# RLinf/RLinf

Measured on NVIDIA H100. Metric: env-steps/sec (rollout+update), higher is better.
Workload: dtype f32

## Files before the change

include/rlinf_b200.h:

```cpp
#ifndef RLINF_B200_H
#define RLINF_B200_H

#include <stdint.h>

#ifdef __cplusplus
extern "C" {
#endif

#define RB200_ABI_VERSION 2

#define RB200_OK 0
#define RB200_E_NULL (-1)
#define RB200_E_SHAPE (-2)
#define RB200_E_ARG (-3)
#define RB200_E_ALIGN (-4)
#define RB200_E_UNSUPPORTED (-5)

typedef void* rb200_stream_t;

int rb200_abi_version(void);
const char* rb200_strerror(int code);
int rb200_device_info(int* sm_count, int* cc_major, int* cc_minor);
uint64_t rb200_launch_count(void);

// ... 164 lines not shown
  float* loss;
  float* metrics;
  float* d_logprobs;
  float* d_entropy;
} rb200_token_loss_args;
int64_t rb200_token_loss_workspace_bytes(int64_t bsz, int64_t L);
int rb200_token_ppo_loss(const rb200_token_loss_args* args, rb200_stream_t stream);

enum {
  RB200_CM_VALUE_LOSS = 0,
  RB200_CM_VALUE_CLIP_RATIO = 1,
  RB200_CM_EV_COUNT = 2,
  RB200_CM_EV_RET_SUM = 3,
  RB200_CM_EV_RET_SQ_SUM = 4,
  RB200_CM_EV_ERR_SUM = 5,
  RB200_CM_EV_ERR_SQ_SUM = 6,
  RB200_CM_FINAL_VALUE_LOSS = 7,
  RB200_CM_NUM = 8
};
typedef struct rb200_token_critic_loss_args {
  int64_t bsz, L;
  const float* values;       int64_t values_stride;
  const float* returns;      int64_t returns_stride;
  const float* prev_values;  int64_t prev_values_stride;
  const uint8_t* loss_mask;  int64_t loss_mask_stride;
  double value_clip, huber_delta;
  void* workspace;
  int64_t workspace_bytes;
  float* loss;
  float* metrics;
  float* d_values;
} rb200_token_critic_loss_args;
int rb200_token_critic_loss(const rb200_token_critic_loss_args* args, rb200_stream_t stream);

enum {
  RB200_RR_SUM_PLEN = 0, RB200_RR_SUM_RLEN = 1, RB200_RR_SUM_REWARDS = 2, RB200_RR_SUM_END = 3,
  RB200_RR_SUM_ADV = 4, RB200_RR_NUM_SEQ = 5, RB200_RR_N_VALID = 6, RB200_RR_SUM_TRAJ_REWARDS = 7,
  RB200_RR_NUM_TRAJ = 8,
  RB200_RR_ADV_NEG_MIN = 9, RB200_RR_ADV_MAX = 10, RB200_RR_MAX_PLEN = 11, RB200_RR_MAX_RLEN = 12,
  RB200_RR_MAX_TOTAL = 13, RB200_RR_VAL_NEG_MIN = 14, RB200_RR_VAL_MAX = 15,
  RB200_RR_VALUES_MEAN = 16,
  RB200_RR_RLEN_SUM = 17, RB200_RR_RLEN_SQ_SUM = 18, RB200_RR_RLEN_MIN = 19, RB200_RR_RLEN_MAX = 20,
  RB200_RR_VERDICT = 21,
  RB200_RR_NUM = 24
};
enum { RB200_RV_EMPTY = 1, RB200_RV_BAD_TRAJ = 2 };
enum {
  RB200_RM_NUM_SEQ = 0, RB200_RM_PROMPT_LENGTH, RB200_RM_RESPONSE_LENGTH, RB200_RM_AVG_RESPONSE_LENGTH,
  RB200_RM_VAR_RESPONSE_LENGTH, RB200_RM_MAX_OF_RESPONSE_LENGTH, RB200_RM_MIN_OF_RESPONSE_LENGTH,
  RB200_RM_TOTAL_LENGTH, RB200_RM_REWARD_SCORES, RB200_RM_PROPERLY_ENDED, RB200_RM_ADV_MEAN, RB200_RM_ADV_MAX,
  RB200_RM_ADV_MIN, RB200_RM_VALUES_MEAN, RB200_RM_VALUES_MAX, RB200_RM_VALUES_MIN, RB200_RM_MAX_PROMPT_LENGTH,
  RB200_RM_MAX_RESPONSE_LENGTH, RB200_RM_MAX_TOTAL_LENGTH, RB200_RM_REWARD_SCORES_TRAJ, RB200_RM_REWARD_SCORES_TURN,
  RB200_RM_AVG_TURNS_PER_TRAJ, RB200_RM_VERDICT, RB200_RM_NUM_LENGTHS_MAX,
  RB200_RM_NUM = 24
};
typedef struct rb200_reasoning_record_args {
  int64_t bsz, L;
  const float* advantages;    int64_t advantages_stride;
  const uint8_t* mask;        int64_t mask_stride;
  const float* values;        int64_t values_stride;
  const int64_t* prompt_lengths;
  const int64_t* response_lengths;
  const float* rewards;
  const uint8_t* is_end;
  const int64_t* idx_to_traj;
  void* workspace;
  int64_t workspace_bytes;
  double* record;
} rb200_reasoning_record_args;
int64_t rb200_reasoning_record_workspace_bytes(int64_t bsz, int64_t L);
int rb200_reasoning_rollout_record(const rb200_reasoning_record_args* args, rb200_stream_t stream);
int rb200_reasoning_rollout_finish(const double* records, int32_t P, const float* values_world_sum,
                                   int32_t world_size, double* metrics, rb200_stream_t stream);

#define RB200_EPI_MAX_KEYS 24
#define RB200_EPI_WS_MIN 64
typedef struct rb200_mb_epilogue_args {
  int32_t n_avg, n_sum;
  int32_t final_slot, ratio_slot;
  const float* src[RB200_EPI_MAX_KEYS];
  const float* loss;
  const uint8_t* mask;  int64_t mask_stride;  int64_t bsz, L;
  const float* global_valid_token;
  int32_t dp, num_microbatches;
  int32_t has_early_stop, mb;
  double early_stop_imp_ratio;
  void* workspace;
  int64_t workspace_bytes;
  float* pack;
  float* scale;
  float* metrics;
  float* step_acc;
  int32_t n_mb, reserved;
} rb200_mb_epilogue_args;
int rb200_mask_count_f32(const uint8_t* mask, int64_t mask_stride, int64_t bsz, int64_t L, void* workspace,
                         int64_t workspace_bytes, float* out, rb200_stream_t stream);
int rb200_mb_epilogue_pack(const rb200_mb_epilogue_args* args, rb200_stream_t stream);
int rb200_mb_epilogue_apply(const rb200_mb_epilogue_args* args, rb200_stream_t stream);
int rb200_step_metrics_finish(const float* step_acc, int32_t n_mb, int32_t n_avg, int32_t n_sum, float* out,
                              rb200_stream_t stream);

int64_t rb200_value_head_workspace_bytes(int64_t n, int64_t H);
int rb200_value_head_fwd(const void* x, int64_t row_stride, const int64_t* rows, int64_t n, int64_t H, const void* w,
                         float* v, rb200_stream_t stream);
int rb200_value_head_bwd(const void* x, int64_t row_stride, const int64_t* rows, int64_t n, int64_t H, const float* g,
                         const void* w, const int64_t* inv_map, int64_t T, void* dx, void* dw, void* workspace,
                         int64_t workspace_bytes, rb200_stream_t stream);

int rb200_scale(float* x, int64_t n, float s, rb200_stream_t stream);
int rb200_scale_by(float* x, int64_t n, const float* s_dev, rb200_stream_t stream);

int rb200_grad_sqnorm(const float* grads, int64_t n, double* out_sq ,
                      rb200_stream_t stream);
int rb200_adamw_step(float* params, const float* grads, float* exp_avg, float* exp_avg_sq,
                     int64_t n, const int64_t* group_end_host, const double* group_lr_host,
                     int n_groups, double beta1, double beta2, double eps, double weight_decay,
                     float max_grad_norm, float grad_scale, const double* grad_sq ,
                     double* state , rb200_stream_t stream);
int rb200_adamw_step_dev(float* params, const float* grads, float* exp_avg, float* exp_avg_sq,
                         int64_t n, const int64_t* group_end_host, const double* group_lr_dev,
                         int n_groups, double beta1, double beta2, double eps, double weight_decay,
                         float max_grad_norm, float grad_scale, const double* grad_sq ,
                         double* state , rb200_stream_t stream);


typedef struct rb200_mlp_layout {
  int32_t obs_dim, act_dim , value_dim, hidden ;
  int64_t logstd;
  int64_t vw0, vb0, vw1, vb1, vw2, vb2, vw3;
  int64_t bw0, bb0, bw1, bb1, bw2, bb2;
  int64_t mw, mb;
  int64_t total;
} rb200_mlp_layout;

int rb200_mlp_layout_init(rb200_mlp_layout* L, int obs_dim, int act_dim, int value_dim, int hidden);

int64_t rb200_mlp_fwd_scratch_floats(const rb200_mlp_layout* L, int64_t n);

int64_t rb200_mlp_wsplit_floats(const rb200_mlp_layout* L);
int rb200_mlp_prepare_weights(const rb200_mlp_layout* L, const float* params, float* wsplit,
                              rb200_stream_t stream);

int rb200_mlp_forward(const rb200_mlp_layout* L, const float* params, const float* wsplit,
                      const float* states, const float* action, const int64_t* idx, int64_t n,
                      float* logprobs, float* entropy, float* values, float* acts, float* work,
                      const float* states_amax, rb200_stream_t stream);
int rb200_absmax(const float* x, int64_t rows, int cols, float* out, rb200_stream_t stream);

int rb200_mlp_backward(const rb200_mlp_layout* L, const float* params, const float* wsplit,
                       const float* states, const float* action, const int64_t* idx, int64_t n,
                       const float* d_logprobs, const float* d_entropy, const float* d_values,
                       const float* acts, float* work, float* grads, rb200_stream_t stream);

int rb200_mlp_sample(const rb200_mlp_layout* L, const float* params, const float* wsplit,
                     const float* states, const float* noise, uint64_t seed, uint64_t offset,
                     const uint64_t* counter_dev, int64_t n, float* action, float* logprobs, float* values,
                     float* work, rb200_stream_t stream);

int rb200_tc_gemm_h(const float* A, const float* B, float* C, int64_t M, int K, int mode, const float* amax,
                    float* work, rb200_stream_t stream);
int rb200_tc_wgrad_h(const float* Z, const float* H, float* dW, int64_t n, int IN, const float* amax,
                     rb200_stream_t stream);
int rb200_tc_dgrad_wgrad_h(const float* Z, const float* W, const float* H, float* dZprev, float* dW, float* colsum,
                           const float* amax_in, float* amax_out, int64_t n, int ngroups, float* work,
                           rb200_stream_t stream);

int rb200_debug_set_flags(int flags);

typedef struct rb200_rollout_args {
  float* states;
  float* actions;
  float* logprobs;
  float* values;
  float* rewards;
  uint8_t* terminations;
  uint8_t* truncations;
  uint8_t* dones;
  float* final_obs;
  float* final_values;
  const float* w_s;
  const float* w_a;
  int32_t* elapsed;
  const float* policy_noise;
  const float* env_noise;
  const uint64_t* counter_policy;
  const uint64_t* counter_env;
  float* episode_return;
  double* episode_acc;
  uint64_t seed_policy, seed_env, offset_policy;
  int32_t T, B;
  int32_t num_action_chunks;
  int32_t max_episode_steps, auto_reset;
  int32_t bootstrap_on_done;
  double gamma, p_term, noise_std, reward_noise_std;
} rb200_rollout_args;

int64_t rb200_rollout_fused_wt_floats(const rb200_mlp_layout* L);
int rb200_rollout_fused_supported(const rb200_mlp_layout* L, int B);
int rb200_rollout_fused_prepare(const rb200_mlp_layout* L, const float* params, float* wt, rb200_stream_t stream);
int rb200_rollout_fused(const rb200_mlp_layout* L, const float* params, const float* wt, const rb200_rollout_args* a,
                        rb200_stream_t stream);

int rb200_rollout_tc_supported(const rb200_mlp_layout* L, int num_action_chunks, int B);
int64_t rb200_rollout_tc_pack_bytes(const rb200_mlp_layout* L);
int rb200_rollout_tc_prepare(const rb200_mlp_layout* L, const float* params, const float* w_s, void* pack,
                             rb200_stream_t stream);
int rb200_rollout_tc(const rb200_mlp_layout* L, const float* params, const void* pack, const rb200_rollout_args* a,
                     rb200_stream_t stream);

int rb200_logits_logprob_entropy_fwd(const void* logits, int dtype, const int64_t* target, int64_t N, int64_t L,
                                     int64_t batch_stride, int64_t row_stride, int V, int v_lo, int v_hi,
                                     double inv_temperature, float* logprob, float* entropy, float* lse,
                                     rb200_stream_t stream);
int rb200_logits_logprob_entropy_bwd(const void* logits, int dtype, const int64_t* target, int64_t N, int64_t L,
                                     int64_t batch_stride, int64_t row_stride, int V, int v_lo, int v_hi,
                                     double inv_temperature, const float* lse, const float* entropy,
                                     const float* grad_logprob, const float* grad_entropy, void* dlogits,
                                     int64_t d_batch_stride, int64_t d_row_stride, rb200_stream_t stream);

int rb200_logits_topk_logprob_entropy_fwd(const void* logits, int dtype, const int64_t* target, int64_t N, int64_t L,
                                          int64_t batch_stride, int64_t row_stride, int V, int v_lo, int v_hi,
                                          double inv_temperature, int top_k, float* logprob, float* entropy, float* lse,
                                          float* threshold, rb200_stream_t stream);
int rb200_logits_topk_logprob_entropy_bwd(const void* logits, int dtype, const int64_t* target, int64_t N, int64_t L,
                                          int64_t batch_stride, int64_t row_stride, int V, int v_lo, int v_hi,
                                          double inv_temperature, const float* threshold, const float* lse,
                                          const float* entropy, const float* grad_logprob, const float* grad_entropy,
                                          void* dlogits, int64_t d_batch_stride, int64_t d_row_stride,
                                          rb200_stream_t stream);

int64_t rb200_lmhead_workspace_bytes(int64_t N, int64_t L, int H, int V, int v_lo, int v_hi, int64_t vocab_chunk);
int rb200_lmhead_logprob_entropy_fwd(const void* hidden, const void* weight, const int64_t* target, int64_t N, int64_t L,
                                     int64_t batch_stride, int64_t row_stride, int H, int V, int v_lo, int v_hi,
                                     double inv_temperature, float* logprob, float* entropy, float* lse,
                                     void* workspace, int64_t workspace_bytes, rb200_stream_t stream);
int rb200_lmhead_logprob_entropy_bwd(const void* hidden, const void* weight, const int64_t* target, int64_t N, int64_t L,
                                     int64_t batch_stride, int64_t row_stride, int H, int V, int v_lo, int v_hi,
                                     double inv_temperature, const float* lse, const float* entropy,
                                     const float* grad_logprob, const float* grad_entropy, void* d_hidden,
                                     void* d_weight, void* workspace, int64_t workspace_bytes, rb200_stream_t stream);

int64_t rb200_lmhead_topk_workspace_bytes(int64_t N, int64_t L, int H, int V, int v_lo, int v_hi, int64_t row_block,
                                          int64_t vocab_chunk);
int rb200_lmhead_topk_logprob_entropy_fwd(const void* hidden, const void* weight, const int64_t* target, int64_t N,
                                          int64_t L, int64_t batch_stride, int64_t row_stride, int H, int V, int v_lo,
                                          int v_hi, double inv_temperature, int top_k, float* logprob, float* entropy,
                                          float* lse, float* threshold, void* workspace, int64_t workspace_bytes,
                                          rb200_stream_t stream);
int rb200_lmhead_topk_logprob_entropy_bwd(const void* hidden, const void* weight, const int64_t* target, int64_t N,
                                          int64_t L, int64_t batch_stride, int64_t row_stride, int H, int V, int v_lo,
                                          int v_hi, double inv_temperature, const float* threshold, const float* lse,
                                          const float* entropy, const float* grad_logprob, const float* grad_entropy,
                                          void* d_hidden, void* d_weight, void* workspace, int64_t workspace_bytes,
                                          rb200_stream_t stream);

typedef struct rb200_action_bins {
  const double* bin_centers;
  const double* low;
  const double* high;
  const uint8_t* mask;
  int64_t vocab_size;
  int32_t n_bins;
  int32_t action_dim;
} rb200_action_bins;
int rb200_logits_sample_tokens(const void* logits, int dtype, int64_t N, int64_t L, int64_t batch_stride,
                               int64_t row_stride, int V, int v_lo, int v_hi, int do_sample, double inv_temperature,
                               int top_k, uint64_t seed, uint64_t offset, const rb200_action_bins* bins, int64_t* token,
                               float* logprob, double* action, rb200_stream_t stream);
int64_t rb200_lmhead_sample_workspace_bytes(int64_t N, int64_t L, int H, int V, int v_lo, int v_hi);
int rb200_lmhead_sample_tokens(const void* hidden, const void* weight, int64_t N, int64_t L, int64_t batch_stride,
                               int64_t row_stride, int H, int V, int v_lo, int v_hi, int do_sample,
                               double inv_temperature, int top_k, uint64_t seed, uint64_t offset,
                               const rb200_action_bins* bins, int64_t* token, float* logprob, double* action,
                               void* workspace, int64_t workspace_bytes, rb200_stream_t stream);

int64_t rb200_lmhead_vp_workspace_bytes(int64_t N, int64_t L, int H, int Vs, int64_t vocab_start, int v_lo, int v_hi,
                                        int64_t vocab_chunk);
int rb200_lmhead_vp_partials_fwd(const void* hidden, const void* weight_shard, const int64_t* target, int64_t N,
                                 int64_t L, int64_t batch_stride, int64_t row_stride, int H, int Vs,
                                 int64_t vocab_start, int v_lo, int v_hi, double inv_temperature, float* record,
                                 void* workspace, int64_t workspace_bytes, rb200_stream_t stream);
int rb200_lmhead_vp_logprob_entropy_bwd(const void* hidden, const void* weight_shard, const int64_t* target,
                                        int64_t N, int64_t L, int64_t batch_stride, int64_t row_stride, int H, int Vs,
                                        int64_t vocab_start, int v_lo, int v_hi, double inv_temperature,
                                        const float* lse, const float* entropy, const float* grad_logprob,
                                        const float* grad_entropy, float* d_hidden_partial, void* d_weight_shard,
                                        void* workspace, int64_t workspace_bytes, rb200_stream_t stream);
int rb200_logits_vp_partials_fwd(const void* logits, int dtype, const int64_t* target, int64_t N, int64_t L,
                                 int64_t batch_stride, int64_t row_stride, int Vs, int64_t vocab_start, int v_lo,
                                 int v_hi, double inv_temperature, float* record, rb200_stream_t stream);
int rb200_vp_combine(const float* records, int n_ranks, int64_t N, const int64_t* target, int vocab_shard, int v_lo,
                     int v_hi, float* logprob, float* entropy, float* lse, rb200_stream_t stream);

enum {
  RB200_RR_RESPONSE = 1,
  RB200_RR_PROMPT = 2,
  RB200_RR_BOUNDS = 4,
  RB200_RR_ORDER = 8,
  RB200_RR_MAX_PROMPT = 16,
  RB200_RR_CAPACITY = 32
};
int rb200_response_rows_plan(int layout, const int64_t* len0, const int64_t* len1, const int64_t* response_lengths,
                             int64_t bsz, int64_t S, int64_t L, int64_t T, int entropy_shift, const int64_t* tokens,
                             int64_t capacity, int64_t* rows, int64_t* targets, int64_t* cell_map,
                             int64_t* hidden_map, int64_t* cells, int64_t* status, rb200_stream_t stream);

enum {
  RB200_RR_SHARD = 64,
  RB200_RR_CP_ALIGN = 128
};
int rb200_response_rows_mp_plan(const int64_t* cu_seqlens_padded, const int64_t* seq_lengths,
                                const int64_t* response_lengths, const int64_t* responses, int64_t bsz, int64_t L,
                                int64_t T_c, int tp_size, int cp_size, int sequence_parallel, int tp_rank, int cp_rank,
                                int64_t capacity_c, int64_t capacity_k, int64_t* rows, int64_t* send, int64_t* unpad,
                                int64_t* slot_map, int64_t* targets, int64_t* cell_map, int64_t* cells,
                                int64_t* hidden_map, int64_t* status, rb200_stream_t stream);
int rb200_response_rows_mp_pack_grad(const float* dx, const int64_t* idx, void* out, int64_t n_out, int64_t H,
                                     rb200_stream_t stream);

int rb200_mlp_value(const rb200_mlp_layout* L, const float* params, const float* wsplit,
// ... 59 lines not shown
```

rlinf_b200/_lib.py:

```python
from __future__ import annotations

import ctypes as C
import os
from typing import Optional

import torch

_PKG_DIR = os.path.dirname(os.path.abspath(__file__))
LIB_PATH = os.path.join(_PKG_DIR, "librlinf_b200.so")

c_void_p, c_int, c_int64, c_float, c_double, c_uint64 = C.c_void_p, C.c_int, C.c_int64, C.c_float, C.c_double, C.c_uint64

NUM_METRICS = 24
LOGPROB_TYPES = {"token_level": 0, "action_level": 1, "chunk_level": 2}

M_KEYS = {
    0: "actor/policy_loss", 1: "actor/policy_loss_abs", 2: "actor/ratio", 3: "actor/ratio_abs",
    4: "actor/clipped_ratio", 5: "actor/dual_cliped_ratio", 6: "actor/approx_kl", 7: "actor/clip_fraction",
    8: "critic/value_loss", 9: "critic/value_clip_ratio",
    10: "__sum__/_critic_explained_variance/count",
    11: "__sum__/_critic_explained_variance/returns_sum",
    12: "__sum__/_critic_explained_variance/returns_sq_sum",
    13: "__sum__/_critic_explained_variance/errors_sum",
    14: "__sum__/_critic_explained_variance/errors_sq_sum",
# ... 32 lines not shown
class DppoScalarVersionArgs(C.Structure):
    _fields_ = [("base", PpoArgs), ("proximal_logprobs", c_void_p), ("version", c_double),
                ("current_version", c_double), ("has_behave_weight_threshold", C.c_int32),
                ("behave_weight_threshold", c_double)]


class RolloutArgs(C.Structure):
    _fields_ = [(n, c_void_p) for n in (
        "states", "actions", "logprobs", "values", "rewards", "terminations", "truncations", "dones", "final_obs",
        "final_values", "w_s", "w_a", "elapsed", "policy_noise", "env_noise", "counter_policy", "counter_env",
        "episode_return", "episode_acc")] + [
        ("seed_policy", c_uint64), ("seed_env", c_uint64), ("offset_policy", c_uint64),
        ("T", C.c_int32), ("B", C.c_int32), ("num_action_chunks", C.c_int32), ("max_episode_steps", C.c_int32),
        ("auto_reset", C.c_int32), ("bootstrap_on_done", C.c_int32),
        ("gamma", c_double), ("p_term", c_double), ("noise_std", c_double), ("reward_noise_std", c_double),
    ]


DM_KEYS = {
    0: "actor/policy_loss", 1: "actor/proximal_ratio", 2: "actor/clipped_proximal_ratio", 3: "actor/clip_fraction",
    4: "actor/dual_clip_fraction", 5: "actor/behav_clip_fraction", 6: "actor/proximal_approx_kl",
    7: "actor/behav_approx_kl", 8: "critic/value_loss", 9: "critic/value_clip_ratio",
    10: "__sum__/_critic_explained_variance/count", 11: "__sum__/_critic_explained_variance/returns_sum",
    12: "__sum__/_critic_explained_variance/returns_sq_sum", 13: "__sum__/_critic_explained_variance/errors_sum",
    14: "__sum__/_critic_explained_variance/errors_sq_sum",
}
DM_ENTROPY = 20


AGG_MODES = {"token-mean": 0, "seq-mean-token-sum": 1, "seq-mean-token-mean": 2}
TM_NUM = 16
TM_KEYS = {
    0: "actor/policy_loss", 1: "actor/policy_loss_abs", 2: "actor/ratio", 3: "actor/ratio_abs",
    4: "actor/clipped_ratio", 5: "actor/dual_cliped_ratio", 6: "actor/approx_kl", 7: "actor/clip_fraction",
    8: "actor/entropy_loss", 9: "actor/kl_loss", 10: "actor/final_loss", 11: "actor/rollout_train_kl",
}


class TokenLossArgs(C.Structure):
    _fields_ = [("bsz", c_int64), ("L", c_int64)] + [
        f for name in ("logprobs", "old_logprobs", "advantages", "loss_mask", "entropy", "ref_logprobs",
                       "rollout_logprobs", "recomputed_logprobs") for f in ((name, c_void_p), (name + "_stride", c_int64))
    ] + [(n, c_double) for n in ("clip_ratio_low", "clip_ratio_high", "clip_ratio_c", "clip_log_ratio_min",
                                  "clip_log_ratio_max", "entropy_bonus", "kl_beta", "importance_sampling_clip")] + [
        (n, C.c_int32) for n in ("has_clip_log_ratio_min", "has_clip_log_ratio_max", "agg", "kl_mode", "kl_order",
                                 "importance_sampling_fix", "fast_path_zero_loss_mask", "reserved")] + [
        ("workspace", c_void_p), ("workspace_bytes", c_int64),
        ("loss", c_void_p), ("metrics", c_void_p), ("d_logprobs", c_void_p), ("d_entropy", c_void_p),
    ]


CM_NUM = 8
CM_KEYS = {
    0: "critic/value_loss", 1: "critic/value_clip_ratio",
    2: "__sum__/_critic_explained_variance/count",
    3: "__sum__/_critic_explained_variance/returns_sum",
    4: "__sum__/_critic_explained_variance/returns_sq_sum",
    5: "__sum__/_critic_explained_variance/errors_sum",
    6: "__sum__/_critic_explained_variance/errors_sq_sum",
    7: "critic/final_value_loss",
}


class TokenCriticLossArgs(C.Structure):
    _fields_ = [("bsz", c_int64), ("L", c_int64)] + [
        f for name in ("values", "returns", "prev_values", "loss_mask")
        for f in ((name, c_void_p), (name + "_stride", c_int64))
    ] + [("value_clip", c_double), ("huber_delta", c_double), ("workspace", c_void_p), ("workspace_bytes", c_int64),
         ("loss", c_void_p), ("metrics", c_void_p), ("d_values", c_void_p)]


RR_NUM = 24
RM_NUM = 24
RM_SLOTS = {
    "total_num_sequence": 0, "prompt_length": 1, "response_length": 2, "average_response_length": 3,
    "variance_of_response_length": 4, "max_of_response_length": 5, "min_of_response_length": 6, "total_length": 7,
    "reward_scores": 8, "fraction_of_samples_properly_ended": 9, "advantages_mean": 10, "advantages_max": 11,
    "advantages_min": 12, "values_mean": 13, "values_max": 14, "values_min": 15, "max_prompt_length": 16,
    "max_response_length": 17, "max_total_length": 18, "reward_scores_traj": 19, "reward_scores_turn": 20,
    "avg_turns_per_traj": 21,
}
RM_VERDICT, RM_NUM_LENGTHS_MAX = 22, 23
RR_VALUES_MEAN = 16
RV_EMPTY, RV_BAD_TRAJ = 1, 2
EPI_MAX_KEYS = 24
EPI_WS_MIN = 64


class ReasoningRecordArgs(C.Structure):
    _fields_ = [("bsz", c_int64), ("L", c_int64)] + [
        f for name in ("advantages", "mask", "values") for f in ((name, c_void_p), (name + "_stride", c_int64))
    ] + [(n, c_void_p) for n in ("prompt_lengths", "response_lengths", "rewards", "is_end", "idx_to_traj",
                                 "workspace")] + [("workspace_bytes", c_int64), ("record", c_void_p)]


class MbEpilogueArgs(C.Structure):
    _fields_ = [(n, C.c_int32) for n in ("n_avg", "n_sum", "final_slot", "ratio_slot")] + [
        ("src", c_void_p * EPI_MAX_KEYS), ("loss", c_void_p), ("mask", c_void_p), ("mask_stride", c_int64),
        ("bsz", c_int64), ("L", c_int64), ("global_valid_token", c_void_p)] + [
        (n, C.c_int32) for n in ("dp", "num_microbatches", "has_early_stop", "mb")] + [
        ("early_stop_imp_ratio", c_double), ("workspace", c_void_p), ("workspace_bytes", c_int64)] + [
        (n, c_void_p) for n in ("pack", "scale", "metrics", "step_acc")] + [("n_mb", C.c_int32), ("reserved", C.c_int32)]


class ActionBins(C.Structure):
    _fields_ = [("bin_centers", c_void_p), ("low", c_void_p), ("high", c_void_p), ("mask", c_void_p),
                ("vocab_size", c_int64), ("n_bins", C.c_int32), ("action_dim", C.c_int32)]


class MlpLayout(C.Structure):
    _fields_ = [
        ("obs_dim", C.c_int32), ("act_dim", C.c_int32), ("value_dim", C.c_int32), ("hidden", C.c_int32),
        ("logstd", c_int64),
        ("vw0", c_int64), ("vb0", c_int64), ("vw1", c_int64), ("vb1", c_int64), ("vw2", c_int64), ("vb2", c_int64),
        ("vw3", c_int64),
        ("bw0", c_int64), ("bb0", c_int64), ("bw1", c_int64), ("bb1", c_int64), ("bw2", c_int64), ("bb2", c_int64),
        ("mw", c_int64), ("mb", c_int64), ("total", c_int64),
    ]


SIGNATURES = {
    "rb200_abi_version": (c_int, []),
    "rb200_strerror": (C.c_char_p, [c_int]),
    "rb200_device_info": (c_int, [C.POINTER(c_int)] * 3),
    "rb200_launch_count": (c_uint64, []),
    "rb200_loss_mask": (c_int, [c_void_p, c_void_p, c_void_p, c_int, c_int, c_int, c_void_p]),
    "rb200_gae": (c_int, [c_void_p] * 7 + [c_int, c_int, c_double, c_double, c_void_p]),
    "rb200_normalize": (c_int, [c_void_p, c_void_p, c_int64, c_float, c_void_p]),
    "rb200_grpo_scores": (c_int, [c_void_p, c_void_p, c_void_p, c_int, c_int, c_void_p]),
    "rb200_grpo_advantages": (c_int, [c_void_p, c_void_p, c_void_p, c_int, c_int, c_int, c_float, c_void_p]),
    "rb200_gather_rows": (c_int, [c_void_p, c_void_p, c_void_p, c_int64, c_int64, c_int64, c_void_p]),
    "rb200_ppo_loss": (c_int, [C.POINTER(PpoArgs), c_void_p]),
    "rb200_decoupled_ppo_loss": (c_int, [C.POINTER(DppoArgs), c_void_p]),
    "rb200_decoupled_ppo_loss_scalar_version": (c_int, [C.POINTER(DppoScalarVersionArgs), c_void_p]),
    "rb200_opd_loss": (c_int, [c_void_p] * 4 + [c_int64, c_int, c_int, c_double] + [c_void_p] * 5),
    "rb200_token_loss_workspace_bytes": (c_int64, [c_int64, c_int64]),
    "rb200_token_ppo_loss": (c_int, [C.POINTER(TokenLossArgs), c_void_p]),
    "rb200_scale": (c_int, [c_void_p, c_int64, c_float, c_void_p]),
    "rb200_scale_by": (c_int, [c_void_p, c_int64, c_void_p, c_void_p]),
    "rb200_grad_sqnorm": (c_int, [c_void_p, c_int64, c_void_p, c_void_p]),
    "rb200_adamw_step": (c_int, [c_void_p] * 4 + [c_int64, C.POINTER(c_int64), C.POINTER(c_double), c_int,
                                                  c_double, c_double, c_double, c_double, c_float, c_float,
                                                  c_void_p, c_void_p, c_void_p]),
    "rb200_adamw_step_dev": (c_int, [c_void_p] * 4 + [c_int64, C.POINTER(c_int64), c_void_p, c_int,
                                                      c_double, c_double, c_double, c_double, c_float, c_float,
                                                      c_void_p, c_void_p, c_void_p]),
    "rb200_mlp_layout_init": (c_int, [C.POINTER(MlpLayout), c_int, c_int, c_int, c_int]),
    "rb200_mlp_fwd_scratch_floats": (c_int64, [C.POINTER(MlpLayout), c_int64]),
    "rb200_mlp_wsplit_floats": (c_int64, [C.POINTER(MlpLayout)]),
    "rb200_mlp_prepare_weights": (c_int, [C.POINTER(MlpLayout), c_void_p, c_void_p, c_void_p]),
    "rb200_mlp_forward": (c_int, [C.POINTER(MlpLayout)] + [c_void_p] * 5 + [c_int64] + [c_void_p] * 7),
    "rb200_absmax": (c_int, [c_void_p, c_int64, c_int, c_void_p, c_void_p]),
    "rb200_mlp_backward": (c_int, [C.POINTER(MlpLayout)] + [c_void_p] * 5 + [c_int64] + [c_void_p] * 7),
    "rb200_mlp_sample": (c_int, [C.POINTER(MlpLayout)] + [c_void_p] * 4 + [c_uint64, c_uint64, c_void_p, c_int64] + [c_void_p] * 5),
    "rb200_tc_gemm_h": (c_int, [c_void_p, c_void_p, c_void_p, c_int64, c_int, c_int, c_void_p, c_void_p, c_void_p]),
    "rb200_tc_wgrad_h": (c_int, [c_void_p, c_void_p, c_void_p, c_int64, c_int, c_void_p, c_void_p]),
    "rb200_tc_dgrad_wgrad_h": (c_int, [c_void_p] * 8 + [c_int64, c_int, c_void_p, c_void_p]),
    "rb200_debug_set_flags": (c_int, [c_int]),
    "rb200_rollout_fused_wt_floats": (c_int64, [C.POINTER(MlpLayout)]),
    "rb200_rollout_fused_supported": (c_int, [C.POINTER(MlpLayout), c_int]),
    "rb200_rollout_fused_prepare": (c_int, [C.POINTER(MlpLayout), c_void_p, c_void_p, c_void_p]),
    "rb200_rollout_fused": (c_int, [C.POINTER(MlpLayout), c_void_p, c_void_p, C.POINTER(RolloutArgs), c_void_p]),
    "rb200_rollout_tc_supported": (c_int, [C.POINTER(MlpLayout), c_int, c_int]),
    "rb200_rollout_tc_pack_bytes": (c_int64, [C.POINTER(MlpLayout)]),
    "rb200_rollout_tc_prepare": (c_int, [C.POINTER(MlpLayout), c_void_p, c_void_p, c_void_p, c_void_p]),
    "rb200_rollout_tc": (c_int, [C.POINTER(MlpLayout), c_void_p, c_void_p, C.POINTER(RolloutArgs), c_void_p]),
    "rb200_logits_logprob_entropy_fwd": (c_int, [c_void_p, c_int, c_void_p, c_int64, c_int64, c_int64, c_int64, c_int,
                                                 c_int, c_int, c_double, c_void_p, c_void_p, c_void_p, c_void_p]),
    "rb200_logits_logprob_entropy_bwd": (c_int, [c_void_p, c_int, c_void_p, c_int64, c_int64, c_int64, c_int64, c_int,
                                                 c_int, c_int, c_double] + [c_void_p] * 5 + [c_int64, c_int64, c_void_p]),
    "rb200_logits_topk_logprob_entropy_fwd": (c_int, [c_void_p, c_int, c_void_p, c_int64, c_int64, c_int64, c_int64,
                                                      c_int, c_int, c_int, c_double, c_int] + [c_void_p] * 5),
    "rb200_logits_topk_logprob_entropy_bwd": (c_int, [c_void_p, c_int, c_void_p, c_int64, c_int64, c_int64, c_int64,
                                                      c_int, c_int, c_int, c_double] + [c_void_p] * 6
                                              + [c_int64, c_int64, c_void_p]),
    "rb200_lmhead_workspace_bytes": (c_int64, [c_int64, c_int64, c_int, c_int, c_int, c_int, c_int64]),
    "rb200_lmhead_logprob_entropy_fwd": (c_int, [c_void_p, c_void_p, c_void_p, c_int64, c_int64, c_int64, c_int64, c_int,
                                                 c_int, c_int, c_int, c_double] + [c_void_p] * 4 + [c_int64, c_void_p]),
    "rb200_lmhead_logprob_entropy_bwd": (c_int, [c_void_p, c_void_p, c_void_p, c_int64, c_int64, c_int64, c_int64, c_int,
                                                 c_int, c_int, c_int, c_double] + [c_void_p] * 7 + [c_int64, c_void_p]),
    "rb200_lmhead_topk_workspace_bytes": (c_int64, [c_int64, c_int64, c_int, c_int, c_int, c_int, c_int64, c_int64]),
    "rb200_lmhead_topk_logprob_entropy_fwd": (c_int, [c_void_p, c_void_p, c_void_p, c_int64, c_int64, c_int64, c_int64,
                                                      c_int, c_int, c_int, c_int, c_double, c_int] + [c_void_p] * 5
                                              + [c_int64, c_void_p]),
    "rb200_lmhead_topk_logprob_entropy_bwd": (c_int, [c_void_p, c_void_p, c_void_p, c_int64, c_int64, c_int64, c_int64,
                                                      c_int, c_int, c_int, c_int, c_double] + [c_void_p] * 8
                                              + [c_int64, c_void_p]),
    "rb200_logits_sample_tokens": (c_int, [c_void_p, c_int, c_int64, c_int64, c_int64, c_int64, c_int, c_int, c_int,
                                           c_int, c_double, c_int, c_uint64, c_uint64, C.POINTER(ActionBins)]
                                   + [c_void_p] * 4),
    "rb200_lmhead_sample_workspace_bytes": (c_int64, [c_int64, c_int64, c_int, c_int, c_int, c_int]),
    "rb200_lmhead_sample_tokens": (c_int, [c_void_p, c_void_p, c_int64, c_int64, c_int64, c_int64, c_int, c_int, c_int,
                                           c_int, c_int, c_double, c_int, c_uint64, c_uint64, C.POINTER(ActionBins)]
                                   + [c_void_p] * 4 + [c_int64, c_void_p]),
    "rb200_lmhead_vp_workspace_bytes": (c_int64, [c_int64, c_int64, c_int, c_int, c_int64, c_int, c_int, c_int64]),
    "rb200_lmhead_vp_partials_fwd": (c_int, [c_void_p, c_void_p, c_void_p, c_int64, c_int64, c_int64, c_int64, c_int,
                                             c_int, c_int64, c_int, c_int, c_double, c_void_p, c_void_p, c_int64,
                                             c_void_p]),
    "rb200_lmhead_vp_logprob_entropy_bwd": (c_int, [c_void_p, c_void_p, c_void_p, c_int64, c_int64, c_int64, c_int64,
                                                    c_int, c_int, c_int64, c_int, c_int, c_double] + [c_void_p] * 7
                                            + [c_int64, c_void_p]),
    "rb200_logits_vp_partials_fwd": (c_int, [c_void_p, c_int, c_void_p, c_int64, c_int64, c_int64, c_int64, c_int,
                                             c_int64, c_int, c_int, c_double, c_void_p, c_void_p]),
    "rb200_vp_combine": (c_int, [c_void_p, c_int, c_int64, c_void_p, c_int, c_int, c_int] + [c_void_p] * 4),
    "rb200_response_rows_plan": (c_int, [c_int, c_void_p, c_void_p, c_void_p, c_int64, c_int64, c_int64, c_int64,
                                         c_int, c_void_p, c_int64] + [c_void_p] * 6 + [c_void_p]),
    "rb200_response_rows_mp_plan": (c_int, [c_void_p] * 4 + [c_int64] * 3 + [c_int] * 5 + [c_int64] * 2
                                    + [c_void_p] * 9 + [c_void_p]),
    "rb200_response_rows_mp_pack_grad": (c_int, [c_void_p, c_void_p, c_void_p, c_int64, c_int64, c_void_p]),
    "rb200_token_critic_loss": (c_int, [C.POINTER(TokenCriticLossArgs), c_void_p]),
    "rb200_reasoning_record_workspace_bytes": (c_int64, [c_int64, c_int64]),
    "rb200_reasoning_rollout_record": (c_int, [C.POINTER(ReasoningRecordArgs), c_void_p]),
    "rb200_reasoning_rollout_finish": (c_int, [c_void_p, C.c_int32, c_void_p, C.c_int32, c_void_p, c_void_p]),
    "rb200_mask_count_f32": (c_int, [c_void_p, c_int64, c_int64, c_int64, c_void_p, c_int64, c_void_p, c_void_p]),
    "rb200_mb_epilogue_pack": (c_int, [C.POINTER(MbEpilogueArgs), c_void_p]),
    "rb200_mb_epilogue_apply": (c_int, [C.POINTER(MbEpilogueArgs), c_void_p]),
    "rb200_step_metrics_finish": (c_int, [c_void_p, C.c_int32, C.c_int32, C.c_int32, c_void_p, c_void_p]),
    "rb200_value_head_workspace_bytes": (c_int64, [c_int64, c_int64]),
    "rb200_value_head_fwd": (c_int, [c_void_p, c_int64, c_void_p, c_int64, c_int64, c_void_p, c_void_p, c_void_p]),
    "rb200_value_head_bwd": (c_int, [c_void_p, c_int64, c_void_p, c_int64, c_int64, c_void_p, c_void_p, c_void_p,
                                     c_int64, c_void_p, c_void_p, c_void_p, c_int64, c_void_p]),
    "rb200_mlp_value":(c_int, [C.POINTER(MlpLayout), c_void_p, c_void_p, c_void_p, c_int64, c_void_p, c_void_p, c_void_p]),
    "rb200_synth_env_step": (c_int, [c_void_p] * 13 + [c_int] * 5 + [c_float] * 3 + [c_uint64, c_void_p, c_void_p]),
    "rb200_synth_env_chunk_step": (c_int, [c_void_p] * 13 + [c_int] * 6 + [c_float] * 3 + [c_uint64, c_void_p, c_void_p]),
    "rb200_bootstrap_rewards_ld": (c_int, [c_void_p, c_int, c_void_p, c_int, c_void_p, c_int, c_int, c_double, c_void_p]),
    "rb200_bootstrap_rewards": (c_int, [c_void_p, c_void_p, c_void_p, c_int, c_int, c_double, c_void_p]),
    "rb200_reward_filter": (c_int, [c_void_p] * 4 + [c_int] * 4 + [c_float, c_float, c_void_p]),
    "rb200_kl_penalty": (c_int, [c_void_p] * 4 + [c_int64, c_int, c_void_p]),
    "rb200_masked_stats": (c_int, [c_void_p, c_void_p, c_int64, c_int64, c_void_p, c_void_p]),
    "rb200_counter_add": (c_int, [c_void_p, c_uint64, c_void_p]),
    "rb200_masked_moments": (c_int, [c_void_p, c_void_p, c_int64, c_void_p, c_void_p]),
    "rb200_masked_normalize": (c_int, [c_void_p, c_void_p, c_void_p, c_int64, c_void_p, c_int, c_double, c_int, c_void_p]),
    "rb200_raw_advantages": (c_int, [c_void_p, c_void_p, c_void_p, c_int, c_int, c_void_p, c_void_p]),
    "rb200_reinpp_returns": (c_int, [c_void_p] * 5 + [c_int, c_int, c_double, c_int, c_void_p, c_void_p]),
    "rb200_grpo_video_advantages": (c_int, [c_void_p] * 4 + [c_int, c_int, c_int, c_int, c_float, c_void_p]),
    "rb200_grpo_dynamic_turn_advantages": (c_int, [c_void_p] * 3 + [c_int, c_int, c_int, c_int, c_float, c_void_p]),
    "rb200_sub": (c_int, [c_void_p, c_void_p, c_void_p, c_int64, c_void_p]),
    "rb200_mlp_mean": (c_int, [C.POINTER(MlpLayout), c_void_p, c_void_p, c_void_p, c_int64] + [c_void_p] * 5),
    "rb200_episode_stats_step": (c_int, [c_void_p, c_void_p, c_int, c_int, c_int] + [c_void_p] * 6),
    "rb200_episode_stats_reduce": (c_int, [c_void_p, c_int, c_void_p, c_void_p]),
    "rb200_train_episode_stats_step": (c_int, [c_void_p, c_void_p] + [c_int] * 4 + [c_void_p] * 4),
}

_LIB: Optional[C.CDLL] = None


class Rb200Error(RuntimeError):
    pass


def load() -> C.CDLL:
    global _LIB
    if _LIB is not None:
        return _LIB
    if not os.path.exists(LIB_PATH):
        raise Rb200Error(
            f"{LIB_PATH} not found: build it with `python -m rlinf_b200.build` "
            "(nvcc, sm_90a). rlinf_b200 has no CPU or PyTorch fallback.")
    lib = C.CDLL(LIB_PATH)
    for name, (res, args) in SIGNATURES.items():
        fn = getattr(lib, name)
        fn.restype = res
        fn.argtypes = args
    _LIB = lib
    return lib


def check(code: int, what: str = "") -> None:
    if code == 0:
        return
    msg = load().rb200_strerror(code).decode()
    if code < 0:
        raise ValueError(f"rlinf_b200 {what}: {msg} (code {code})")
    raise Rb200Error(f"rlinf_b200 {what}: CUDA error {code}: {msg}")


def ptr(t: Optional[torch.Tensor]):
    if t is None:
        return None
    if not t.is_cuda:
        raise Rb200Error("rlinf_b200 kernels take CUDA tensors; move inputs with to_device() first")
    if not t.is_contiguous():
        raise Rb200Error("rlinf_b200 kernels take contiguous tensors")
    return c_void_p(t.data_ptr())


def stream_ptr(device=None):
    return c_void_p(torch.cuda.current_stream(device).cuda_stream)


def default_device() -> torch.device:
    if not torch.cuda.is_available():
        raise Rb200Error("rlinf_b200 needs a CUDA device (H100, sm_90a); there is no CPU fallback")
    return torch.device("cuda", torch.cuda.current_device())


def to_device(t: Optional[torch.Tensor], device=None, dtype=None) -> Optional[torch.Tensor]:
    if t is None:
        return None
    device = device or default_device()
    if t.device != device:
        t = t.to(device, non_blocking=True)
    if dtype is not None and t.dtype != dtype:
        t = t.to(dtype)
    return t.contiguous()


def as_u8(t: Optional[torch.Tensor]) -> Optional[torch.Tensor]:
    if t is None:
        return None
    if t.dtype == torch.bool:
# ... 5 lines not shown
```

rlinf_b200/actor.py:

```python
from __future__ import annotations

from typing import Optional

import numpy as np
import torch
import torch.distributed as dist

from . import _lib as L
from . import dist_utils as D
from . import ops
from .algorithms import calculate_adv_and_returns
from .config import wrap
from .lr_scheduler import LRSchedule
from .policy import FlatAdamW, MLPPolicy

EV_KEY = "critic/explained_variance"
_T_PLUS_ONE_KEYS = ("dones", "terminations", "truncations", "prev_values")


def process_nested_dict_for_adv(nested, rollout_epoch):
    out = {}
    for k, v in nested.items():
        if isinstance(v, dict):
            out[k] = process_nested_dict_for_adv(v, rollout_epoch)
        elif isinstance(v, torch.Tensor):
            x = v.reshape(rollout_epoch, -1, *v.shape[1:]).transpose(0, 1)
            out[k] = x.reshape(x.shape[0], -1, *x.shape[3:])
    return out


def process_nested_dict_for_train(nested, shuffle_id):
    out = {}
    for k, v in nested.items():
        if v is None:
            out[k] = None
        elif isinstance(v, dict):
            out[k] = process_nested_dict_for_train(v, shuffle_id)
        elif isinstance(v, torch.Tensor):
            if k in _T_PLUS_ONE_KEYS:
                v = v[:-1]
            flat = v.reshape(-1, *v.shape[2:])
            if any(s == 0 for s in flat.stride()) and flat.numel() > 1:
                flat = flat.contiguous()
            as_bool = flat.dtype == torch.bool
            src = flat.contiguous()
            res = ops.gather_rows(src.view(torch.uint8) if as_bool else src, shuffle_id)
            out[k] = res.view(torch.bool) if as_bool else res
    return out


class EmbodiedActor:
    def __init__(self, cfg, policy: Optional[MLPPolicy] = None, rank: Optional[int] = None,
                 world_size: Optional[int] = None, process_group=None):
        self.cfg = wrap(cfg)
        self.pg = process_group
        self._dist = dist.is_available() and dist.is_initialized()
        self._rank = rank if rank is not None else (dist.get_rank() if self._dist else 0)
        self._world_size = world_size if world_size is not None else (dist.get_world_size() if self._dist else 1)
        m = self.cfg.actor.model
        self.device = L.default_device()
        self.model = policy or MLPPolicy(m.obs_dim, m.action_dim, m.get("num_action_chunks", 1),
                                         add_value_head=m.get("add_value_head", True), device=self.device,
                                         seed=self.cfg.actor.seed)
        o = self.cfg.actor.optim
        self.optimizer = FlatAdamW(self.model, lr=o.lr, value_lr=o.get("value_lr", o.lr),
                                   betas=(o.get("adam_beta1", 0.9), o.get("adam_beta2", 0.999)),
                                   eps=o.get("adam_eps", 1e-8), weight_decay=o.get("weight_decay", 1e-2),
                                   clip_grad=o.get("clip_grad", 1.0))
        self.optimizer_steps = 0
        self.critic_warmup_steps = int(o.get("critic_warmup_steps", 0) or 0) if self.model.value_dim > 0 else 0
        self._with_critic = self.cfg.algorithm.adv_type == "gae"
        self._set_frozen_groups()
        self.lr_schedule = LRSchedule(o, base_lr=o.lr)
        self.optimizer.lr_scale = self.lr_schedule.multiplier()
        self.rollout_batch: dict = {}
        self._perm_cache: dict = {}
        self.version = 0
        self._graph_update = self.cfg.actor.get("cuda_graph_update", False)
        self._graph_multi_rank = bool(self.cfg.actor.get("cuda_graph_multi_rank", False))
        self._capture_nccl = bool(self.cfg.actor.get("cuda_graph_capture_nccl", True))
        self._static_batch: dict = {}
        self._step_graphs: dict = {}
        self._train_calls = 0
        self._states_amax = torch.zeros(4 + m.obs_dim if m.obs_dim <= 256 else 1, dtype=torch.float32,
                                        device=self.device) if m.obs_dim % 32 == 0 else None

    def recv_rollout_trajectories(self, batch: dict) -> None:
        def to_dev(d):
            return {k: (to_dev(v) if isinstance(v, dict) else L.to_device(v, self.device)) for k, v in d.items()
                    if v is not None}

        self.rollout_batch = self._process_received_rollout_batch(to_dev(batch))

    def _process_received_rollout_batch(self, rollout_batch: dict) -> dict:
        cfg = self.cfg
        rollout_epoch = cfg.env.train.get("rollout_epoch", 1)
        if rollout_epoch != 1:
            rollout_batch = process_nested_dict_for_adv(rollout_batch, rollout_epoch)
        if not cfg.env.train.auto_reset and not cfg.env.train.get("ignore_terminations", False):
            loss_mask, loss_mask_sum = ops.loss_mask(rollout_batch["dones"])
            if cfg.algorithm.reward_type == "chunk_level":
                loss_mask = loss_mask.any(dim=-1, keepdim=True)
                loss_mask_sum = loss_mask_sum[..., -1:]
            rollout_batch["loss_mask"] = loss_mask
            rollout_batch["loss_mask_sum"] = loss_mask_sum
        if cfg.algorithm.get("filter_rewards", False):
            rollout_batch["loss_mask"] = ops.reward_filter(
                rollout_batch["rewards"], rollout_batch.get("loss_mask", None), cfg.algorithm.group_size,
                cfg.algorithm.rewards_lower_bound, cfg.algorithm.rewards_upper_bound)
        return rollout_batch

    def compute_advantages_and_returns(self) -> dict:
        cfg, rb = self.cfg, self.rollout_batch
        kwargs = {
            "task_type": cfg.runner.task_type, "adv_type": cfg.algorithm.adv_type, "rewards": rb["rewards"],
            "dones": rb["dones"], "values": rb.get("prev_values", None), "prev_logprobs": rb.get("prev_logprobs", None),
            "teacher_logprobs": None, "num_action_chunks": cfg.actor.model.get("num_action_chunks", 1),
            "gamma": cfg.algorithm.get("gamma", 1), "gae_lambda": cfg.algorithm.get("gae_lambda", 1),
            "group_size": cfg.algorithm.get("group_size", 8), "reward_type": cfg.algorithm.reward_type,
            "loss_mask": rb.get("loss_mask", None), "loss_mask_sum": rb.get("loss_mask_sum", None),
            "advantage_mode": cfg.algorithm.get("advantage_mode", None),
        }
        rb.update(calculate_adv_and_returns(**kwargs))
        if not cfg.runner.get("rollout_metrics", True):
            return {}
        from .metric_utils import compute_rollout_metrics

        return compute_rollout_metrics(rb, self._world_size, self.pg)

    def _shuffle_id(self, n: int) -> torch.Tensor:
        key = (n, self.cfg.actor.seed + self._rank)
        if key not in self._perm_cache:
            g = torch.Generator()
            g.manual_seed(D.shuffle_seed(self.cfg.actor.seed, self._rank))
            self._perm_cache[key] = torch.randperm(n, generator=g).to(self.device)
        return self._perm_cache[key]

    def run_training(self) -> dict:
        cfg = self.cfg
        rb = self.rollout_batch
        rollout_size = rb["prev_logprobs"].shape[0] * rb["prev_logprobs"].shape[1]
        shuffle_id = self._shuffle_id(rollout_size)
        batch = process_nested_dict_for_train(rb, shuffle_id)
        self.rollout_batch = batch
        mbs = cfg.actor.micro_batch_size
        batch_size_per_rank, self.gradient_accumulation, n_global = D.per_rank_batch(
            cfg.actor.global_batch_size, self._world_size, mbs, rollout_size)
        update_epoch = cfg.algorithm.get("update_epoch", 1)
        n_steps = update_epoch * n_global
        n_micro = n_steps * self.gradient_accumulation
        metric_rows = torch.zeros(n_micro, L.NUM_METRICS, dtype=torch.float32, device=self.device)
        step_rows = torch.zeros(n_steps, 4, dtype=torch.float64, device=self.device)
        lr_rows = []
        mi = si = 0
        use_graph = self._graph_update
        if use_graph == "auto":
            use_graph = batch_size_per_rank <= 65536
        if self._world_size > 1 and not self._graph_multi_rank:
            use_graph = False
        graphed = bool(use_graph) and self._train_calls > 0
        self._train_calls += 1
        if graphed:
            batch = self._persist_batch(batch)
            self.rollout_batch = batch
        if self._states_amax is not None:
            ops.absmax(batch["forward_inputs"]["states"], out=self._states_amax)
        for _ in range(update_epoch):
            for gb in range(n_global):
                if graphed:
                    lr_rows.append(self._graphed_step(batch, gb, batch_size_per_rank, mbs,
                                                      metric_rows[mi: mi + self.gradient_accumulation], step_rows[si]))
                    mi += self.gradient_accumulation
                    si += 1
                    continue
                self.optimizer.zero_grad()
                for k in range(self.gradient_accumulation):
                    lo = gb * batch_size_per_rank + k * mbs
                    self.train_micro_batch(batch, lo, lo + mbs, metric_rows[mi])
                    mi += 1
                grad_norm_state, lr_list = self.optimizer_step()
                step_rows[si].copy_(grad_norm_state)
                lr_rows.append(lr_list)
                si += 1
        self.optimizer.lr_scale = self.lr_schedule.step()
        self.optimizer.zero_grad()
        return self._reduce_metrics(metric_rows, step_rows, lr_rows)

    def _persist_batch(self, batch: dict, prefix: str = "") -> dict:
        out = {}
        for k, v in batch.items():
            key = prefix + k
            if isinstance(v, dict):
                out[k] = self._persist_batch(v, key + "/")
            elif isinstance(v, torch.Tensor):
                buf = self._static_batch.get(key)
                if buf is None or buf.shape != v.shape or buf.dtype != v.dtype:
                    buf = torch.empty_like(v)
                    self._static_batch[key] = buf
                    self._step_graphs.clear()
                buf.copy_(v)
                out[k] = buf
            else:
                out[k] = v
        return out

    def _graphed_step(self, batch, gb, batch_size_per_rank, mbs, metric_out, state_out):
        warm = self.optimizer_steps < self.critic_warmup_steps
        accum = self.gradient_accumulation
        key = (gb, warm, accum, mbs, batch_size_per_rank, self._world_size)
        self.optimizer.sync_lr_table()
        entry = self._step_graphs.get(key)
        if entry is None:
            stage_m = torch.zeros(accum, L.NUM_METRICS, dtype=torch.float32, device=self.device)
            stage_s = torch.zeros(4, dtype=torch.float64, device=self.device)
            scale = 1.0 / self._world_size

            def fwd_bwd():
                self.optimizer.zero_grad()
                for k in range(accum):
                    lo = gb * batch_size_per_rank + k * mbs
                    self.train_micro_batch(batch, lo, lo + mbs, stage_m[k])

            def opt():
                self.optimizer.step(grad_scale=scale)
                stage_s.copy_(self.optimizer.state)

            graphs = None
            if self._world_size > 1 and self._capture_nccl:
                try:
                    torch.cuda.synchronize()
                    self.model.mark_params_changed()
                    g_all = torch.cuda.CUDAGraph()
                    with torch.cuda.graph(g_all):
                        fwd_bwd()
                        dist.all_reduce(self.model.flat_grads, op=dist.ReduceOp.SUM, group=self.pg)
                        opt()
                    graphs = (g_all, None)
                except Exception as e:
                    self._capture_nccl = False
                    self._capture_nccl_error = repr(e)
                    torch.cuda.synchronize()
            if graphs is None:
                torch.cuda.synchronize()
                self.model.mark_params_changed()
                g_a = torch.cuda.CUDAGraph()
                with torch.cuda.graph(g_a):
                    fwd_bwd()
                g_b = torch.cuda.CUDAGraph()
                with torch.cuda.graph(g_b, pool=g_a.pool()):
                    opt()
                graphs = (g_a, g_b)
            entry = (graphs, stage_m, stage_s)
            self._step_graphs[key] = entry
        (g_a, g_b), stage_m, stage_s = entry
        g_a.replay()
        self.optimizer_steps += 1
        if g_b is not None:
            D.allreduce_flat_grads(self.model.flat_grads, self._world_size, self.pg)
            g_b.replay()
        self.model.mark_params_changed()
        metric_out.copy_(stage_m)
        state_out.copy_(stage_s)
        return self._after_optimizer_step()

    def train_micro_batch(self, batch, lo, hi, metric_out) -> None:
        cfg = self.cfg
        fi = batch["forward_inputs"]
        with_critic = self._with_critic
        ent_bonus = float(cfg.algorithm.get("entropy_bonus", 0) or 0)
        warm = self.optimizer_steps < self.critic_warmup_steps
        out = self.model.forward_train(fi["states"][lo:hi], fi["action"][lo:hi], compute_entropy=ent_bonus > 0,
                                       compute_values=with_critic, states_amax=self._states_amax)
        A = cfg.actor.model.get("action_dim", 7)
        Cc = out["logprobs"].shape[1] // A
        U = 1 if cfg.algorithm.logprob_type == "chunk_level" else Cc
        n = hi - lo

        def unit(key):
            t = batch.get(key)
            return None if t is None else t[lo:hi].reshape(n, U)

        loss, metrics, d_lp, d_v, d_e = ops.ppo_loss(
            logprobs=out["logprobs"], values=out.get("values") if with_critic else None,
            entropy=out.get("entropy"), old_logprobs=batch["prev_logprobs"][lo:hi].reshape(n, Cc * A),
            advantages=unit("advantages"), returns=unit("returns") if with_critic else None,
            prev_values=unit("prev_values") if with_critic else None, loss_mask=unit("loss_mask"),
            loss_mask_sum=unit("loss_mask_sum"), C_chunks=Cc, A_dim=A, logprob_type=cfg.algorithm.logprob_type,
            clip_ratio_low=cfg.algorithm.clip_ratio_low, clip_ratio_high=cfg.algorithm.clip_ratio_high,
            value_clip=cfg.algorithm.get("value_clip", None), huber_delta=cfg.algorithm.get("huber_delta", None),
            max_episode_steps=cfg.env.train.max_episode_steps if batch.get("loss_mask_sum") is not None else None,
            critic_warmup=warm, entropy_bonus=ent_bonus, loss_scale=1.0 / self.gradient_accumulation)
        metric_out.copy_(metrics)
        self.model.backward(d_lp, d_v if with_critic else None, d_e)

    def _set_frozen_groups(self):
        frozen = set()
        if self.critic_warmup_steps > 0:
            frozen.add("actor")
        if not self._with_critic:
            frozen.add("critic")
        self.optimizer.frozen = frozen

    def _after_optimizer_step(self):
        if self.critic_warmup_steps > 0:
            lr_list = [0.0 for _ in self.optimizer.lr_list()]
            if self.optimizer_steps >= self.critic_warmup_steps:
                self.critic_warmup_steps = 0
                self._set_frozen_groups()
                self.optimizer.reset_state(carry_grads=True)
                self.lr_schedule = LRSchedule(self.cfg.actor.optim, base_lr=self.cfg.actor.optim.lr)
                self.optimizer.lr_scale = self.lr_schedule.multiplier()
            return lr_list
        return self.optimizer.lr_list()

    def state_dict(self) -> dict:
        return {"optimizer": self.optimizer.state_dict(), "optimizer_steps": int(self.optimizer_steps),
                "critic_warmup_steps": int(self.critic_warmup_steps),
                "lr_last_epoch": int(self.lr_schedule.last_epoch), "lr_scale": float(self.optimizer.lr_scale)}

    def load_state_dict(self, sd: dict) -> None:
        self.optimizer.load_state_dict(sd["optimizer"])
        self.optimizer_steps = int(sd["optimizer_steps"])
        self.critic_warmup_steps = int(sd["critic_warmup_steps"])
        self._set_frozen_groups()
        self.lr_schedule.last_epoch = int(sd["lr_last_epoch"])
        self.optimizer.lr_scale = float(sd["lr_scale"])
        self.model.mark_params_changed()

    def optimizer_step(self):
        self.optimizer_steps += 1
        scale = D.allreduce_flat_grads(self.model.flat_grads, self._world_size, self.pg)
        self.optimizer.step(grad_scale=scale)
        state = self.optimizer.state.clone()
        return state, self._after_optimizer_step()

    def _reduce_metrics(self, metric_rows, step_rows, lr_rows) -> dict:
        with_critic = self.cfg.algorithm.adv_type == "gae"
        mean_vec = metric_rows.mean(dim=0)
        ev_sum = metric_rows[:, 10:15].sum(dim=0)
        grad_norm = step_rows[:, 1].mean().to(torch.float32)
        packed = D.reduce_metric_pack(mean_vec, ev_sum, grad_norm, self._world_size, self.pg)
        host = packed.tolist()
        out = {}
        slots = L.ACTOR_SLOTS + ((8, 9) if with_critic else ()) + (15, 16)
        for s in slots:
            out[L.M_KEYS[s]] = host[s]
        out["actor/grad_norm"] = host[-1]
        out["actor/lr"] = float(np.mean([r[0] for r in lr_rows]))
        second = [r[1] for r in lr_rows if len(r) > 1]
        if second:
            out["critic/lr"] = float(np.mean(second))
        if with_critic:
            cnt, rs, rss, es, ess = host[L.NUM_METRICS: L.NUM_METRICS + 5]
            ev = float("nan")
            if cnt >= 2:
                rc = rss - rs * rs / cnt
                ec = ess - es * es / cnt
                if rc == rc and rc != 0 and ec == ec:
                    ev = 1 - ec / rc
            out[EV_KEY] = ev
        return out

    def sync_model_to_rollout(self, rollout_params: Optional[torch.Tensor] = None, src: int = 0):
        if rollout_params is not None and rollout_params.data_ptr() != self.model.flat_params.data_ptr():
            rollout_params.copy_(self.model.flat_params)
        if self.cfg.runner.get("broadcast_params", True):
            from .weight_sync import broadcast_flat

            self.rollout_version = broadcast_flat(self.model, self.version, src, self.pg)
        self.model.mark_params_changed()
```

rlinf_b200/csrc/mlp.cu:

```cuda
#include <curand_kernel.h>

#include "common.cuh"
#include "sgemm.cuh"
#include "tc_gemm.cuh"

namespace {

using namespace rb::gemm;

__global__ void __launch_bounds__(256) absmax_kernel(const float4* __restrict__ x, int64_t n4, int cols4, int cols,
                                                     float* __restrict__ out) {
  __shared__ unsigned int s_col[256];
  __shared__ unsigned int s_all;
  for (int c = threadIdx.x; c < 256; c += blockDim.x) s_col[c] = 0u;
  if (threadIdx.x == 0) s_all = 0u;
  __syncthreads();
  float4 m = make_float4(0.f, 0.f, 0.f, 0.f);
  for (int64_t i = (int64_t)blockIdx.x * blockDim.x + threadIdx.x; i < n4; i += (int64_t)gridDim.x * blockDim.x) {
    const float4 v = __ldg(x + i);
    m.x = fmaxf(m.x, fabsf(v.x)); m.y = fmaxf(m.y, fabsf(v.y)); m.z = fmaxf(m.z, fabsf(v.z)); m.w = fmaxf(m.w, fabsf(v.w));
  }
  atomicMax(&s_all, __float_as_uint(fmaxf(fmaxf(m.x, m.y), fmaxf(m.z, m.w))));
  if (cols) {
    const int c0 = 4 * (threadIdx.x % cols4);
    atomicMax(&s_col[c0], __float_as_uint(m.x)); atomicMax(&s_col[c0 + 1], __float_as_uint(m.y));
    atomicMax(&s_col[c0 + 2], __float_as_uint(m.z)); atomicMax(&s_col[c0 + 3], __float_as_uint(m.w));
  }
  __syncthreads();
  if (threadIdx.x == 0 && s_all) atomicMax(reinterpret_cast<unsigned int*>(out), s_all);
  for (int c = threadIdx.x; c < cols; c += blockDim.x)
    if (s_col[c]) atomicMax(reinterpret_cast<unsigned int*>(out + 4 + c), s_col[c]);
}

constexpr int kH = 256;
constexpr int kMaxAct = 32;
constexpr int kMaxVal = 8;
constexpr float kHalfLog2Pi = 0.91893853320467274178f;

struct HeadFwdArgs {
  const float* h3;
  const float* g3;
  const float* mw;
  const float* mb;
  const float* logstd;
  const float* vw3;
  const float* action;
  const int64_t* idx;
  const float* noise;
  uint64_t seed, offset;
  const uint64_t* counter;
  int sample_mode;
  float* mean_out;
  float* action_out;
  float* logprobs;
  float* entropy;
  float* values;
  int64_t n;
  int act, vdim;
};

__global__ void __launch_bounds__(256) head_fwd_kernel(HeadFwdArgs p) {
  extern __shared__ float sm[];
  float* s_mw = sm;
  float* s_vw = sm + p.act * kH;
  for (int i = threadIdx.x; i < p.act * kH; i += blockDim.x) s_mw[i] = p.mw[i];
  if (p.g3 && p.values)
    for (int i = threadIdx.x; i < p.vdim * kH; i += blockDim.x) s_vw[i] = p.vw3[i];
  __syncthreads();
  const int lane = threadIdx.x & 31, warp = threadIdx.x >> 5, nwarp = blockDim.x >> 5;
  const bool want_v = p.g3 && p.values;
  const int64_t row_stride = (int64_t)gridDim.x * nwarp;
  float4 nh0 = make_float4(0.f, 0.f, 0.f, 0.f), nh1 = nh0, ng0 = nh0, ng1 = nh0;
  auto fetch = [&](int64_t r) {
    if (r < p.n) {
      nh0 = __ldg(reinterpret_cast<const float4*>(p.h3 + r * kH + lane * 4));
      nh1 = __ldg(reinterpret_cast<const float4*>(p.h3 + r * kH + 128 + lane * 4));
      if (want_v) {
        ng0 = __ldg(reinterpret_cast<const float4*>(p.g3 + r * kH + lane * 4));
        ng1 = __ldg(reinterpret_cast<const float4*>(p.g3 + r * kH + 128 + lane * 4));
      }
    }
  };
  fetch((int64_t)blockIdx.x * nwarp + warp);
  for (int64_t row = (int64_t)blockIdx.x * nwarp + warp; row < p.n; row += row_stride) {
    const float4 h0 = nh0, h1 = nh1, pg0 = ng0, pg1 = ng1;
    fetch(row + row_stride);
    float my_mean = 0.f;
    for (int a = 0; a < p.act; ++a) {
      const float4 w0 = *reinterpret_cast<const float4*>(s_mw + a * kH + lane * 4);
      const float4 w1 = *reinterpret_cast<const float4*>(s_mw + a * kH + 128 + lane * 4);
      float s = h0.x * w0.x + h0.y * w0.y + h0.z * w0.z + h0.w * w0.w + h1.x * w1.x + h1.y * w1.y + h1.z * w1.z +
                h1.w * w1.w;
      s = rb::warp_sum(s);
      if (lane == a) my_mean = s + p.mb[a];
    }
    if (lane < p.act) {
      const float ls = p.logstd[lane];
      const float sd = expf(ls);
      float x;
      if (p.sample_mode == 2) {
        x = my_mean;
        p.action_out[row * p.act + lane] = x;
      } else if (p.sample_mode) {
        float z;
        if (p.noise) {
          z = p.noise[row * p.act + lane];
        } else {
          curandStatePhilox4_32_10_t st;
          curand_init(p.seed, (unsigned long long)(row * p.act + lane), p.offset + 4ull * (p.counter ? p.counter[0] : 0ull), &st);
          z = curand_normal(&st);
        }
        x = my_mean + sd * z;
        p.action_out[row * p.act + lane] = x;
      } else {
        const int64_t src = p.idx ? p.idx[row] : row;
        x = p.action[src * p.act + lane];
      }
      const float d = x - my_mean;
      const float var = sd * sd;
      if (p.logprobs) p.logprobs[row * p.act + lane] = -(d * d) / (2.0f * var) - logf(sd) - kHalfLog2Pi;
      if (p.entropy) p.entropy[row * p.act + lane] = 0.5f + kHalfLog2Pi + logf(sd);
      if (p.mean_out) p.mean_out[row * p.act + lane] = my_mean;
    }
    if (want_v) {
      const float4 g0 = pg0, g1 = pg1;
      for (int c = 0; c < p.vdim; ++c) {
        const float4 w0 = *reinterpret_cast<const float4*>(s_vw + c * kH + lane * 4);
        const float4 w1 = *reinterpret_cast<const float4*>(s_vw + c * kH + 128 + lane * 4);
        float s = g0.x * w0.x + g0.y * w0.y + g0.z * w0.z + g0.w * w0.w + g1.x * w1.x + g1.y * w1.y + g1.z * w1.z +
                  g1.w * w1.w;
        s = rb::warp_sum(s);
        if (lane == 0) p.values[row * p.vdim + c] = s;
      }
    }
  }
}

struct HeadBwdArgs {
  const float* h3;
  const float* g3;
  const float* mean;
  const float* mw;
  const float* logstd;
  const float* vw3;
  const float* action;
  const int64_t* idx;
  const float* d_logprobs;
  const float* d_entropy;
  const float* d_values;
  float* dz3;
  float* dy3;
  float* g_mw;
  float* g_mb;
  float* g_logstd;
  float* g_vw3;
  float* g_b2;
  float* g_vb2;
  float* amax_dz3;
  float* amax_dy3;
  float* part;
  int64_t n;
  int act, vdim;
};

template <bool REG>
__global__ void __launch_bounds__(256) head_bwd_kernel(HeadBwdArgs p) {
  extern __shared__ float sm[];
  const int lane = threadIdx.x & 31, warp = threadIdx.x >> 5, nwarp = blockDim.x >> 5;
  const int acc_len = (p.act + p.vdim) * kH + 64 + 2 * kH;
  float* s_mw = sm;
  float* s_vw = s_mw + p.act * kH;
  float* acc0 = s_vw + p.vdim * kH;
  float* a_mw = acc0 + warp * acc_len;
  float* a_vw = a_mw + p.act * kH;
  float* a_mb = a_vw + p.vdim * kH;
  float* a_ls = a_mb + 32;
  float* a_b2 = a_ls + 32;
  float* a_vb2 = a_b2 + kH;
  const bool has_v = p.d_values != nullptr;
  for (int i = threadIdx.x; i < p.act * kH; i += blockDim.x) s_mw[i] = p.mw[i];
  for (int i = threadIdx.x; i < p.vdim * kH; i += blockDim.x) s_vw[i] = has_v ? p.vw3[i] : 0.f;
  for (int i = threadIdx.x; i < nwarp * acc_len; i += blockDim.x) acc0[i] = 0.f;
  __syncthreads();
  float cb[8] = {0.f, 0.f, 0.f, 0.f, 0.f, 0.f, 0.f, 0.f}, cv[8] = {0.f, 0.f, 0.f, 0.f, 0.f, 0.f, 0.f, 0.f};
  float mz = 0.f, my = 0.f;
  float rm[REG ? 8 : 1][8], rv[REG ? 2 : 1][8];
#pragma unroll
  for (int a = 0; a < (REG ? 8 : 1); ++a)
#pragma unroll
    for (int j = 0; j < 8; ++j) rm[a][j] = 0.f;
#pragma unroll
  for (int c = 0; c < (REG ? 2 : 1); ++c)
#pragma unroll
    for (int j = 0; j < 8; ++j) rv[c][j] = 0.f;
  struct RowIn {
    float4 h0, h1, g0, g1;
    float x, mu, dlp, den, dv0, dv1;
  };
  auto load_row = [&](int64_t row) -> RowIn {
    RowIn r;
    r.h0 = r.h1 = r.g0 = r.g1 = make_float4(0.f, 0.f, 0.f, 0.f);
    r.x = r.mu = r.dlp = r.den = r.dv0 = r.dv1 = 0.f;
    if (row < p.n) {
      r.h0 = __ldg(reinterpret_cast<const float4*>(p.h3 + row * kH + lane * 4));
      r.h1 = __ldg(reinterpret_cast<const float4*>(p.h3 + row * kH + 128 + lane * 4));
      if (has_v) {
        r.g0 = __ldg(reinterpret_cast<const float4*>(p.g3 + row * kH + lane * 4));
        r.g1 = __ldg(reinterpret_cast<const float4*>(p.g3 + row * kH + 128 + lane * 4));
        if (REG) {
          r.dv0 = __ldg(p.d_values + row * p.vdim);
          if (p.vdim > 1) r.dv1 = __ldg(p.d_values + row * p.vdim + 1);
        }
      }
      if (lane < p.act) {
        const int64_t src = p.idx ? p.idx[row] : row;
        r.x = __ldg(p.action + src * p.act + lane);
        r.mu = __ldg(p.mean + row * p.act + lane);
        r.dlp = __ldg(p.d_logprobs + row * p.act + lane);
        if (p.d_entropy) r.den = __ldg(p.d_entropy + row * p.act + lane);
      }
    }
    return r;
  };
  const int64_t row_stride = (int64_t)gridDim.x * nwarp;
  const int64_t row_first = (int64_t)blockIdx.x * nwarp + warp;
  const float sd_l = lane < p.act ? expf(p.logstd[lane]) : 1.f;
  const float var_l = sd_l * sd_l;
  RowIn nxt0 = load_row(row_first), nxt1 = load_row(row_first + row_stride);
  for (int64_t row = row_first; row < p.n; row += row_stride) {
    const RowIn cur = nxt0;
    nxt0 = nxt1;
    nxt1 = load_row(row + 2 * row_stride);
    const float4 h0 = cur.h0, h1 = cur.h1;
    float dmu = 0.f;
    if (lane < p.act) {
      const float d = cur.x - cur.mu;
      dmu = cur.dlp * d / var_l;
      const float dls = cur.dlp * (d * d / var_l - 1.0f) + cur.den;
      atomicAdd(&a_mb[lane], dmu);
      atomicAdd(&a_ls[lane], dls);
    }
    float4 dh0 = make_float4(0.f, 0.f, 0.f, 0.f), dh1 = dh0;
#pragma unroll
    for (int a = 0; a < (REG ? 8 : kMaxAct); ++a) {
      if (a >= p.act) break;
      const float g = __shfl_sync(0xffffffffu, dmu, a);
      const float4 w0 = *reinterpret_cast<const float4*>(s_mw + a * kH + lane * 4);
      const float4 w1 = *reinterpret_cast<const float4*>(s_mw + a * kH + 128 + lane * 4);
      dh0.x += g * w0.x; dh0.y += g * w0.y; dh0.z += g * w0.z; dh0.w += g * w0.w;
      dh1.x += g * w1.x; dh1.y += g * w1.y; dh1.z += g * w1.z; dh1.w += g * w1.w;
      if (REG) {
        const int ar = a < 8 ? a : 0;
        rm[ar][0] += g * h0.x; rm[ar][1] += g * h0.y; rm[ar][2] += g * h0.z; rm[ar][3] += g * h0.w;
        rm[ar][4] += g * h1.x; rm[ar][5] += g * h1.y; rm[ar][6] += g * h1.z; rm[ar][7] += g * h1.w;
        continue;
      }
      float* am = a_mw + a * kH;
      atomicAdd(&am[lane * 4 + 0], g * h0.x); atomicAdd(&am[lane * 4 + 1], g * h0.y);
      atomicAdd(&am[lane * 4 + 2], g * h0.z); atomicAdd(&am[lane * 4 + 3], g * h0.w);
      atomicAdd(&am[128 + lane * 4 + 0], g * h1.x); atomicAdd(&am[128 + lane * 4 + 1], g * h1.y);
      atomicAdd(&am[128 + lane * 4 + 2], g * h1.z); atomicAdd(&am[128 + lane * 4 + 3], g * h1.w);
    }
    float4 o0, o1;
    o0.x = dh0.x * (1.f - h0.x * h0.x); o0.y = dh0.y * (1.f - h0.y * h0.y);
    o0.z = dh0.z * (1.f - h0.z * h0.z); o0.w = dh0.w * (1.f - h0.w * h0.w);
    o1.x = dh1.x * (1.f - h1.x * h1.x); o1.y = dh1.y * (1.f - h1.y * h1.y);
    o1.z = dh1.z * (1.f - h1.z * h1.z); o1.w = dh1.w * (1.f - h1.w * h1.w);
    *reinterpret_cast<float4*>(p.dz3 + row * kH + lane * 4) = o0;
    *reinterpret_cast<float4*>(p.dz3 + row * kH + 128 + lane * 4) = o1;
    cb[0] += o0.x; cb[1] += o0.y; cb[2] += o0.z; cb[3] += o0.w;
    cb[4] += o1.x; cb[5] += o1.y; cb[6] += o1.z; cb[7] += o1.w;
    mz = fmaxf(mz, fmaxf(fmaxf(fmaxf(fabsf(o0.x), fabsf(o0.y)), fmaxf(fabsf(o0.z), fabsf(o0.w))),
                         fmaxf(fmaxf(fabsf(o1.x), fabsf(o1.y)), fmaxf(fabsf(o1.z), fabsf(o1.w)))));

    if (has_v) {
      const float4 g0 = cur.g0, g1 = cur.g1;
      float4 dg0 = make_float4(0.f, 0.f, 0.f, 0.f), dg1 = dg0;
#pragma unroll
      for (int c = 0; c < (REG ? 2 : kMaxVal); ++c) {
        if (c >= p.vdim) break;
        const float g = REG ? (c == 0 ? cur.dv0 : cur.dv1) : p.d_values[row * p.vdim + c];
        const float4 w0 = *reinterpret_cast<const float4*>(s_vw + c * kH + lane * 4);
        const float4 w1 = *reinterpret_cast<const float4*>(s_vw + c * kH + 128 + lane * 4);
        dg0.x += g * w0.x; dg0.y += g * w0.y; dg0.z += g * w0.z; dg0.w += g * w0.w;
        dg1.x += g * w1.x; dg1.y += g * w1.y; dg1.z += g * w1.z; dg1.w += g * w1.w;
        if (REG) {
          const int cr = c < 2 ? c : 0;
          rv[cr][0] += g * g0.x; rv[cr][1] += g * g0.y; rv[cr][2] += g * g0.z; rv[cr][3] += g * g0.w;
          rv[cr][4] += g * g1.x; rv[cr][5] += g * g1.y; rv[cr][6] += g * g1.z; rv[cr][7] += g * g1.w;
          continue;
        }
        float* av = a_vw + c * kH;
        atomicAdd(&av[lane * 4 + 0], g * g0.x); atomicAdd(&av[lane * 4 + 1], g * g0.y);
        atomicAdd(&av[lane * 4 + 2], g * g0.z); atomicAdd(&av[lane * 4 + 3], g * g0.w);
        atomicAdd(&av[128 + lane * 4 + 0], g * g1.x); atomicAdd(&av[128 + lane * 4 + 1], g * g1.y);
        atomicAdd(&av[128 + lane * 4 + 2], g * g1.z); atomicAdd(&av[128 + lane * 4 + 3], g * g1.w);
      }
      float4 q0, q1;
      q0.x = dg0.x * (1.f - g0.x * g0.x); q0.y = dg0.y * (1.f - g0.y * g0.y);
      q0.z = dg0.z * (1.f - g0.z * g0.z); q0.w = dg0.w * (1.f - g0.w * g0.w);
      q1.x = dg1.x * (1.f - g1.x * g1.x); q1.y = dg1.y * (1.f - g1.y * g1.y);
      q1.z = dg1.z * (1.f - g1.z * g1.z); q1.w = dg1.w * (1.f - g1.w * g1.w);
      *reinterpret_cast<float4*>(p.dy3 + row * kH + lane * 4) = q0;
      *reinterpret_cast<float4*>(p.dy3 + row * kH + 128 + lane * 4) = q1;
      cv[0] += q0.x; cv[1] += q0.y; cv[2] += q0.z; cv[3] += q0.w;
      cv[4] += q1.x; cv[5] += q1.y; cv[6] += q1.z; cv[7] += q1.w;
      my = fmaxf(my, fmaxf(fmaxf(fmaxf(fabsf(q0.x), fabsf(q0.y)), fmaxf(fabsf(q0.z), fabsf(q0.w))),
                           fmaxf(fmaxf(fabsf(q1.x), fabsf(q1.y)), fmaxf(fabsf(q1.z), fabsf(q1.w)))));
    }
  }
  if (p.amax_dz3 != nullptr) {
#pragma unroll
    for (int o = 16; o > 0; o >>= 1) {
      mz = fmaxf(mz, __shfl_xor_sync(0xffffffffu, mz, o));
      my = fmaxf(my, __shfl_xor_sync(0xffffffffu, my, o));
    }
    if (lane == 0) {
      if (mz > 0.f) atomicMax(reinterpret_cast<unsigned int*>(p.amax_dz3), __float_as_uint(mz));
      if (has_v && my > 0.f && p.amax_dy3) atomicMax(reinterpret_cast<unsigned int*>(p.amax_dy3), __float_as_uint(my));
    }
  }
#pragma unroll
  for (int j = 0; j < 4; ++j) {
    atomicAdd(&a_b2[lane * 4 + j], cb[j]);
    atomicAdd(&a_b2[128 + lane * 4 + j], cb[4 + j]);
    if (has_v) {
      atomicAdd(&a_vb2[lane * 4 + j], cv[j]);
      atomicAdd(&a_vb2[128 + lane * 4 + j], cv[4 + j]);
    }
  }
  if (REG) {
#pragma unroll
    for (int a = 0; a < 8; ++a) {
      if (a >= p.act) break;
      float* am = a_mw + a * kH;
#pragma unroll
      for (int j = 0; j < 4; ++j) {
        atomicAdd(&am[lane * 4 + j], rm[a][j]);
        atomicAdd(&am[128 + lane * 4 + j], rm[a][4 + j]);
      }
    }
    if (has_v) {
#pragma unroll
      for (int c = 0; c < 2; ++c) {
        if (c >= p.vdim) break;
        float* av = a_vw + c * kH;
#pragma unroll
        for (int j = 0; j < 4; ++j) {
          atomicAdd(&av[lane * 4 + j], rv[c][j]);
          atomicAdd(&av[128 + lane * 4 + j], rv[c][4 + j]);
        }
      }
    }
  }
  __syncthreads();
  for (int i = threadIdx.x; i < acc_len; i += blockDim.x) {
    float s = 0.f;
    for (int w = 0; w < nwarp; ++w) s += acc0[w * acc_len + i];
    p.part[(size_t)blockIdx.x * acc_len + i] = s;
  }
}

int head_grid(int64_t n) {
  int64_t blocks = (n + 7) / 8;
  const int64_t cap = (int64_t)rb::sm_count() * 4;
  if (blocks > cap) blocks = cap;
  return (int)(blocks < 1 ? 1 : blocks);
}

struct TowerW {
  const float *w0, *b0, *w1, *b1, *w2, *b2;
};
int layer_forward(const float* in, const int64_t* idx, int64_t n, int in_dim, const float* w, const float* b,
                  float* out, cudaStream_t st) {
  GemmArgs g{};
  g.M = n; g.N = kH; g.ldc = kH; g.k_per_split = 1 << 30;
  g.A = in; g.lda = in_dim; g.a_rows = idx; g.B = w; g.ldb = in_dim; g.K = in_dim; g.bias = b; g.C = out;
  return launch_gemm<A_KCONTIG, B_KCONTIG, EPI_BIAS_TANH>(g, 1, st);
}


struct TowerWH {
  const float *w0f, *w1f, *w2f;
  const float *w1d, *w2d;
};

struct TowerIO {
  TowerW w;
  TowerWH wh;
  float *H1, *H2, *H3;
  float *g_w0, *g_b0, *g_w1, *g_b1, *g_w2, *g_b2;
  const float* dZ3;
  float *tA, *tB;
  float* amax;
};

bool layer0_on_tc(const int64_t* idx, int in_dim) { return idx == nullptr && in_dim % rb::tc::BK == 0; }

float* x_amax_slot(const rb200_mlp_layout* L, float* buf, int64_t n) { return buf + 6 * n * kH + n * L->act_dim; }
int64_t x_amax_floats(int cols) { return cols <= 256 ? 4 + cols : 1; }

int publish_absmax(const float* X, int64_t rows, int cols, float* out, cudaStream_t st) {
  if (reinterpret_cast<uintptr_t>(X) & 15) return RB200_E_ALIGN;
  if (cols % 4 != 0) return RB200_E_SHAPE;
  cudaError_t ce = cudaMemsetAsync(out, 0, sizeof(float) * x_amax_floats(cols), st);
  if (ce != cudaSuccess) return (int)ce;
  const int cols4 = cols / 4, col_out = cols <= 256 ? cols : 0;
  const int threads = col_out ? cols4 * (256 / cols4) : 256;
  const int64_t n4 = rows * cols4;
  int64_t blocks = (n4 + threads - 1) / threads;
  const int64_t cap = (int64_t)rb::sm_count() * 4;
  if (blocks > cap) blocks = cap;
  absmax_kernel<<<(int)(blocks < 1 ? 1 : blocks), threads, 0, st>>>(reinterpret_cast<const float4*>(X), n4,
                                                                    col_out ? cols4 : 1, col_out, out);
  rb::count_launch();
  ce = cudaPeekAtLastError();
  return ce == cudaSuccess ? 0 : (int)ce;
}

int towers_forward_h(const float* X, const int64_t* idx, int64_t n, int in_dim, TowerIO* t, int nt, float* x_amax,
                     const float* x_amax_in, cudaStream_t st) {
  int e;
  const bool l0_tc = layer0_on_tc(idx, in_dim);
  rb::tch::GemmLaunch g[2];
  auto gemm = [&](int K) {
    return K <= rb::tc::BN ? rb::tch::forward(g, nt, n, K, rb::tc::EPI_BIAS_TANH, st)
                           : rb::tch::launch(g, nt, n, K, rb::tc::EPI_BIAS_TANH, 0, st);
  };
  if (l0_tc) {
    if (x_amax_in) {
      cudaError_t ce = cudaMemcpyAsync(x_amax, x_amax_in, sizeof(float) * x_amax_floats(in_dim), cudaMemcpyDeviceToDevice, st);
      if (ce != cudaSuccess) return (int)ce;
    } else if ((e = publish_absmax(X, n, in_dim, x_amax, st))) {
      return e;
    }
    for (int i = 0; i < nt; ++i) g[i] = rb::tch::GemmLaunch{X, t[i].wh.w0f, t[i].H1, t[i].w.b0, nullptr, nullptr, nullptr, nullptr, x_amax};
    if ((e = gemm(in_dim))) return e;
  } else {
    for (int i = 0; i < nt; ++i)
      if ((e = layer_forward(X, idx, n, in_dim, t[i].w.w0, t[i].w.b0, t[i].H1, st))) return e;
  }
  for (int i = 0; i < nt; ++i) g[i] = rb::tch::GemmLaunch{t[i].H1, t[i].wh.w1f, t[i].H2, t[i].w.b1, nullptr, nullptr, nullptr, nullptr};
  if ((e = gemm(kH))) return e;
  for (int i = 0; i < nt; ++i) g[i] = rb::tch::GemmLaunch{t[i].H2, t[i].wh.w2f, t[i].H3, t[i].w.b2, nullptr, nullptr, nullptr, nullptr};
  return gemm(kH);
}

int simt_wgrad_chunks(int64_t n, int64_t* rows_per_chunk) {
  int64_t chunks = (n + 255) / 256;
  const int64_t cap = rb::sm_count() / 2 > 1 ? rb::sm_count() / 2 : 1;
  if (chunks > cap) chunks = cap;
  const int64_t rows = (n + chunks - 1) / chunks;
  *rows_per_chunk = rows;
  return (int)((n + rows - 1) / rows);
}

int towers_backward_h(const float* X, const int64_t* idx, int64_t n, int in_dim, TowerIO* t, int nt,
                      const float* x_amax, cudaStream_t st) {
  int e;
  rb::tch::WgradLaunch w[2];
  rb::tch::BackwardLaunch b[2];
  for (int i = 0; i < nt; ++i)
    b[i] = rb::tch::BackwardLaunch{t[i].dZ3, t[i].wh.w2d, t[i].H2, t[i].tA, t[i].g_w2, t[i].g_b1, t[i].amax, t[i].amax + 1,
                                   t[i].tB};
  if ((e = rb::tch::dgrad_wgrad(b, nt, n, st))) return e;
  for (int i = 0; i < nt; ++i)
    b[i] = rb::tch::BackwardLaunch{t[i].tA, t[i].wh.w1d, t[i].H1, t[i].tB, t[i].g_w1, t[i].g_b0, t[i].amax + 1, t[i].amax + 2,
                                   const_cast<float*>(t[i].dZ3)};
  if ((e = rb::tch::dgrad_wgrad(b, nt, n, st))) return e;
  if (layer0_on_tc(idx, in_dim) && in_dim <= 256) {
    for (int i = 0; i < nt; ++i) w[i] = rb::tch::WgradLaunch{t[i].tB, X, t[i].g_w0, t[i].amax + 2, x_amax + 4};
    return rb::tch::wgrad(w, nt, n, in_dim, st);
  }
  int64_t rows = 0;
  const int chunks = simt_wgrad_chunks(n, &rows);
  const int64_t slab = (int64_t)kH * in_dim;
  float* part = rb::partials_scratch(chunks * slab);
  if (!part) return RB200_E_UNSUPPORTED;
  for (int i = 0; i < nt; ++i) {
    GemmArgs a{};
    a.A = t[i].tB; a.lda = kH; a.B = X; a.ldb = in_dim; a.b_rows = idx; a.C = part; a.c_split_stride = slab;
    a.ldc = in_dim; a.M = kH; a.N = in_dim; a.K = n; a.k_per_split = rows;
    if ((e = launch_gemm<A_MCONTIG, B_NCONTIG, EPI_STORE>(a, chunks, st))) return e;
    rb::tch::SlotSums ss{};
    ss.count = 1;
    ss.nslab = chunks;
    ss.stride = slab;
    ss.part[0] = part;
    ss.out[0] = t[i].g_w0;
    ss.len[0] = (int)slab;
    if ((e = rb::tch::sum_slots(ss, st))) return e;
  }
  return 0;
}

}

extern "C" int rb200_mlp_layout_init(rb200_mlp_layout* L, int obs_dim, int act_dim, int value_dim, int hidden) {
  if (!L) return RB200_E_NULL;
  if (obs_dim <= 0 || act_dim <= 0 || value_dim < 0) return RB200_E_SHAPE;
  if (hidden != kH || act_dim > kMaxAct || value_dim > kMaxVal) return RB200_E_UNSUPPORTED;
  L->obs_dim = obs_dim; L->act_dim = act_dim; L->value_dim = value_dim; L->hidden = hidden;
  int64_t o = 0;
  auto take = [&](int64_t n) { o = (o + 3) & ~int64_t(3); const int64_t at = o; o += n; return at; };
  L->logstd = take(act_dim);
  L->vw0 = take((int64_t)hidden * obs_dim); L->vb0 = take(hidden);
  L->vw1 = take((int64_t)hidden * hidden); L->vb1 = take(hidden);
  L->vw2 = take((int64_t)hidden * hidden); L->vb2 = take(hidden);
  L->vw3 = take((int64_t)value_dim * hidden);
  L->bw0 = take((int64_t)hidden * obs_dim); L->bb0 = take(hidden);
  L->bw1 = take((int64_t)hidden * hidden); L->bb1 = take(hidden);
  L->bw2 = take((int64_t)hidden * hidden); L->bb2 = take(hidden);
  L->mw = take((int64_t)act_dim * hidden); L->mb = take(act_dim);
  L->total = (o + 3) & ~int64_t(3);
  const int64_t sms = rb::sm_count(), head = 4 * sms * ((act_dim + value_dim) * hidden + 64 + 2 * hidden);
  const int64_t wg = sms / 2 * hidden * (obs_dim > hidden ? obs_dim : hidden) + sms * hidden;
  if (!rb::partials_scratch(head > wg ? head : wg)) (void)cudaGetLastError();
  return RB200_OK;
}

static inline int64_t act_floats(int64_t n) { return n * kH; }

extern "C" int64_t rb200_mlp_fwd_scratch_floats(const rb200_mlp_layout* L, int64_t n) {
  if (!L || n <= 0) return 0;
  return 6 * act_floats(n) + n * L->act_dim + 64 + 256;
}

static inline int64_t wsplit_tower_floats(int obs) { return (int64_t)kH * obs + 4ll * kH * kH; }

extern "C" int64_t rb200_mlp_wsplit_floats(const rb200_mlp_layout* L) {
  if (!L) return 0;
  return 2 * wsplit_tower_floats(L->obs_dim);
}

static int check_layout(const rb200_mlp_layout* L) {
  if (!L) return RB200_E_NULL;
  if (L->hidden != kH || L->act_dim <= 0 || L->act_dim > kMaxAct || L->value_dim < 0 || L->value_dim > kMaxVal)
    return RB200_E_UNSUPPORTED;
  return RB200_OK;
}

namespace {
TowerW tower_w(const rb200_mlp_layout* L, const float* P, bool value) {
  TowerW w;
  if (value) {
    w.w0 = P + L->vw0; w.b0 = P + L->vb0; w.w1 = P + L->vw1; w.b1 = P + L->vb1; w.w2 = P + L->vw2; w.b2 = P + L->vb2;
  } else {
    w.w0 = P + L->bw0; w.b0 = P + L->bb0; w.w1 = P + L->bw1; w.b1 = P + L->bb1; w.w2 = P + L->bw2; w.b2 = P + L->bb2;
  }
  return w;
}
TowerWH tower_wh(const rb200_mlp_layout* L, const float* ws, bool value) {
  const int64_t n0 = (int64_t)kH * L->obs_dim, nn = (int64_t)kH * kH;
  const float* b = ws + (value ? 0 : wsplit_tower_floats(L->obs_dim));
  TowerWH t;
  t.w0f = b;
  t.w1f = b + n0;
  t.w2f = b + n0 + nn;
  t.w1d = b + n0 + 2 * nn;
  t.w2d = b + n0 + 3 * nn;
  return t;
}

TowerIO tower_io(const rb200_mlp_layout* L, const float* P, const float* wsplit, bool value, float* h, int64_t n) {
  TowerIO t{};
  t.w = tower_w(L, P, value);
  t.wh = tower_wh(L, wsplit, value);
  t.H1 = h;
  t.H2 = h + act_floats(n);
  t.H3 = h + 2 * act_floats(n);
  return t;
}

int forward_towers(const rb200_mlp_layout* L, const float* P, const float* wsplit, const float* states,
                   const int64_t* idx, int64_t n, bool policy, bool value, float* buf, const float* x_amax_in,
                   cudaStream_t st) {
  TowerIO t[2];
  int nt = 0;
  if (policy) t[nt++] = tower_io(L, P, wsplit, false, buf, n);
  if (value) t[nt++] = tower_io(L, P, wsplit, true, buf + 3 * act_floats(n), n);
  return towers_forward_h(states, idx, n, L->obs_dim, t, nt, x_amax_slot(L, buf, n), x_amax_in, st);
}

int head_forward(const rb200_mlp_layout* L, const float* P, const float* buf, int64_t n, float* values, HeadFwdArgs h,
                 cudaStream_t st) {
  h.h3 = buf + 2 * act_floats(n); h.g3 = values ? buf + 5 * act_floats(n) : nullptr;
  h.mw = P + L->mw; h.mb = P + L->mb; h.logstd = P + L->logstd; h.vw3 = P + L->vw3;
  h.values = values; h.n = n; h.act = L->act_dim; h.vdim = L->value_dim;
  const size_t smem = sizeof(float) * (size_t)(L->act_dim + (values ? L->value_dim : 0)) * kH;
  head_fwd_kernel<<<head_grid(n), 256, smem, st>>>(h);
  rb::count_launch();
  RB_RETURN_LAUNCH();
}
}

extern "C" int rb200_mlp_prepare_weights(const rb200_mlp_layout* L, const float* params, float* wsplit,
                                         rb200_stream_t stream) {
  int e = check_layout(L);
  if (e) return e;
  if (!params || !wsplit) return RB200_E_NULL;
  rb::tch::SplitSpec sp[6];
  int cnt = 0;
  for (int v = 0; v < 2; ++v) {
    if (v == 0 && L->value_dim == 0) continue;
    const TowerW w = tower_w(L, params, v == 0);
    const TowerWH t = tower_wh(L, wsplit, v == 0);
    const int64_t n0 = (int64_t)kH * L->obs_dim, nn = (int64_t)kH * kH;
    if (L->obs_dim % rb::tc::BK == 0)
      sp[cnt++] = rb::tch::SplitSpec{w.w0, const_cast<float*>(t.w0f), nullptr, n0};
    sp[cnt++] = rb::tch::SplitSpec{w.w1, const_cast<float*>(t.w1f), const_cast<float*>(t.w1d), nn};
    sp[cnt++] = rb::tch::SplitSpec{w.w2, const_cast<float*>(t.w2f), const_cast<float*>(t.w2d), nn};
  }
  return rb::tch::split_weights(sp, cnt, rb::as_stream(stream));
}

extern "C" int rb200_mlp_forward(const rb200_mlp_layout* L, const float* params, const float* wsplit,
                                 const float* states, const float* action, const int64_t* idx, int64_t n,
                                 float* logprobs, float* entropy, float* values, float* acts, float* work,
                                 const float* states_amax, rb200_stream_t stream) {
  int e = check_layout(L);
  if (e) return e;
  if (!params || !wsplit || !states || !action || !logprobs || !acts || !work) return RB200_E_NULL;
  if (n <= 0) return RB200_E_SHAPE;
  if (values && L->value_dim == 0) return RB200_E_SHAPE;
  cudaStream_t st = rb::as_stream(stream);
  if ((e = forward_towers(L, params, wsplit, states, idx, n, true, values != nullptr, acts, states_amax, st))) return e;
  HeadFwdArgs h{};
  h.action = action; h.idx = idx; h.sample_mode = 0; h.mean_out = acts + 6 * act_floats(n); h.logprobs = logprobs;
  h.entropy = entropy;
  return head_forward(L, params, acts, n, values, h, st);
}

extern "C" int rb200_mlp_backward(const rb200_mlp_layout* L, const float* params, const float* wsplit,
                                  const float* states, const float* action, const int64_t* idx, int64_t n,
                                  const float* d_logprobs, const float* d_entropy, const float* d_values,
                                  const float* acts, float* work, float* grads, rb200_stream_t stream) {
  int e = check_layout(L);
  if (e) return e;
  if (!params || !wsplit || !states || !action || !d_logprobs || !acts || !work || !grads) return RB200_E_NULL;
  if (n <= 0) return RB200_E_SHAPE;
  cudaStream_t st = rb::as_stream(stream);
  const int64_t PF = act_floats(n);
  const float *H3 = acts + 2 * PF, *G3 = acts + 5 * PF, *mean = acts + 6 * PF;
  float *dZ3 = work, *tA = dZ3 + PF, *tB = tA + PF, *dY3 = tB + PF, *uA = dY3 + PF, *uB = uA + PF;
  const float* P = params;
  float* G = grads;
  HeadBwdArgs h{};
  h.h3 = H3; h.g3 = G3; h.mean = mean; h.mw = P + L->mw;
  h.logstd = P + L->logstd; h.vw3 = P + L->vw3; h.action = action; h.idx = idx; h.d_logprobs = d_logprobs;
  h.d_entropy = d_entropy; h.d_values = d_values; h.dz3 = dZ3; h.dy3 = dY3;
  h.g_mw = G + L->mw; h.g_mb = G + L->mb; h.g_logstd = G + L->logstd; h.g_vw3 = G + L->vw3;
  h.g_b2 = G + L->bb2; h.g_vb2 = G + L->vb2;
  h.n = n; h.act = L->act_dim; h.vdim = L->value_dim;
  float* amax = work + 6 * PF;
  {
    cudaError_t ce = cudaMemsetAsync(amax, 0, 8 * sizeof(float), st);
    if (ce != cudaSuccess) return (int)ce;
  }
  h.amax_dz3 = amax;
  h.amax_dy3 = amax + 3;
  const int acc_len = (L->act_dim + L->value_dim) * kH + 64 + 2 * kH, w_len = (L->act_dim + L->value_dim) * kH;
  int nw = (232448 / 4 - w_len) / acc_len;
  nw = nw > 8 ? 8 : nw;
  const size_t smem = sizeof(float) * ((size_t)w_len + (size_t)nw * acc_len);
  const bool reg = L->act_dim <= 8 && L->value_dim <= 2;
  const int grid = head_grid(n);
  if (!(h.part = rb::partials_scratch((int64_t)grid * acc_len))) return RB200_E_UNSUPPORTED;
  {
    cudaError_t ce = cudaFuncSetAttribute(head_bwd_kernel<false>, cudaFuncAttributeMaxDynamicSharedMemorySize, (int)smem);
    if (ce == cudaSuccess)
      ce = cudaFuncSetAttribute(head_bwd_kernel<true>, cudaFuncAttributeMaxDynamicSharedMemorySize, (int)smem);
    if (ce != cudaSuccess) return (int)ce;
  }
  if (reg)
    head_bwd_kernel<true><<<grid, 32 * nw, smem, st>>>(h);
  else
    head_bwd_kernel<false><<<grid, 32 * nw, smem, st>>>(h);
  rb::count_launch();
  {
    cudaError_t ce = cudaPeekAtLastError();
    if (ce != cudaSuccess) return (int)ce;
  }
  {
    rb::tch::SlotSums ss{};
    ss.nslab = grid;
    ss.stride = acc_len;
    const int A = L->act_dim, V = L->value_dim;
    auto seg = [&](int off, float* out, int len) {
      ss.part[ss.count] = h.part + off; ss.out[ss.count] = out; ss.len[ss.count++] = len;
    };
    seg(0, h.g_mw, A * kH);
    seg((A + V) * kH, h.g_mb, A);
    seg((A + V) * kH + 32, h.g_logstd, A);
    seg((A + V) * kH + 64, h.g_b2, kH);
    if (d_values) {
      seg(A * kH, h.g_vw3, V * kH);
      seg((A + V) * kH + 64 + kH, h.g_vb2, kH);
    }
    if ((e = rb::tch::sum_slots(ss, st))) return e;
  }
  float* act_buf = const_cast<float*>(acts);
  TowerIO t[2] = {tower_io(L, P, wsplit, false, act_buf, n), tower_io(L, P, wsplit, true, act_buf + 3 * PF, n)};
  t[0].dZ3 = dZ3; t[0].tA = tA; t[0].tB = tB; t[0].amax = amax;
  t[0].g_w0 = G + L->bw0; t[0].g_b0 = G + L->bb0; t[0].g_w1 = G + L->bw1; t[0].g_b1 = G + L->bb1;
  t[0].g_w2 = G + L->bw2; t[0].g_b2 = G + L->bb2;
  t[1].dZ3 = dY3; t[1].tA = uA; t[1].tB = uB; t[1].amax = amax + 3;
  t[1].g_w0 = G + L->vw0; t[1].g_b0 = G + L->vb0; t[1].g_w1 = G + L->vw1; t[1].g_b1 = G + L->vb1;
  t[1].g_w2 = G + L->vw2; t[1].g_b2 = G + L->vb2;
  return towers_backward_h(states, idx, n, L->obs_dim, t, d_values ? 2 : 1, x_amax_slot(L, act_buf, n), st);
}

extern "C" int rb200_mlp_sample(const rb200_mlp_layout* L, const float* params, const float* wsplit,
                                const float* states, const float* noise, uint64_t seed, uint64_t offset,
                                const uint64_t* counter_dev, int64_t n, float* action, float* logprobs, float* values,
                                float* work, rb200_stream_t stream) {
  int e = check_layout(L);
  if (e) return e;
  if (!params || !wsplit || !states || !action || !logprobs || !work) return RB200_E_NULL;
  if (n <= 0) return RB200_E_SHAPE;
  cudaStream_t st = rb::as_stream(stream);
  if ((e = forward_towers(L, params, wsplit, states, nullptr, n, true, values != nullptr, work, nullptr, st))) return e;
  HeadFwdArgs h{};
  h.noise = noise; h.seed = seed; h.offset = offset; h.counter = counter_dev; h.sample_mode = 1; h.action_out = action;
  h.logprobs = logprobs;
  return head_forward(L, params, work, n, values, h, st);
}

namespace rb {
int mlp_mean_forward(const rb200_mlp_layout* L, const float* params, const float* wsplit, const float* states,
                     int64_t n, float* action, float* logprobs, float* values, float* work, cudaStream_t st) {
  int e = check_layout(L);
  if (e) return e;
  if ((e = forward_towers(L, params, wsplit, states, nullptr, n, true, values != nullptr, work, nullptr, st))) return e;
  HeadFwdArgs h{};
  h.sample_mode = 2; h.action_out = action; h.logprobs = logprobs;
  return head_forward(L, params, work, n, values, h, st);
}
}

extern "C" int rb200_absmax(const float* x, int64_t rows, int cols, float* out, rb200_stream_t stream) {
  if (!x || !out) return RB200_E_NULL;
  if (rows <= 0 || cols <= 0 || cols % 4 != 0) return RB200_E_SHAPE;
  return publish_absmax(x, rows, cols, out, rb::as_stream(stream));
}

namespace {
__global__ void __launch_bounds__(256) value_head_kernel(const float* __restrict__ g3, const float* __restrict__ vw3, float* __restrict__ values,
                                                         int64_t n, int vdim) {
  const int lane = threadIdx.x & 31, warp = threadIdx.x >> 5, nwarp = blockDim.x >> 5;
  for (int64_t row = (int64_t)blockIdx.x * nwarp + warp; row < n; row += (int64_t)gridDim.x * nwarp) {
    const float4 g0 = *reinterpret_cast<const float4*>(g3 + row * kH + lane * 4);
    const float4 g1 = *reinterpret_cast<const float4*>(g3 + row * kH + 128 + lane * 4);
    for (int c = 0; c < vdim; ++c) {
      const float4 w0 = *reinterpret_cast<const float4*>(vw3 + c * kH + lane * 4);
      const float4 w1 = *reinterpret_cast<const float4*>(vw3 + c * kH + 128 + lane * 4);
      float s = g0.x * w0.x + g0.y * w0.y + g0.z * w0.z + g0.w * w0.w + g1.x * w1.x + g1.y * w1.y + g1.z * w1.z +
                g1.w * w1.w;
      s = rb::warp_sum(s);
      if (lane == 0) values[row * vdim + c] = s;
    }
  }
}
}

extern "C" int rb200_mlp_value(const rb200_mlp_layout* L, const float* params, const float* wsplit,
                               const float* states, int64_t n, float* values, float* work, rb200_stream_t stream) {
  int e = check_layout(L);
  if (e) return e;
  if (!params || !wsplit || !states || !values || !work) return RB200_E_NULL;
  if (n <= 0 || L->value_dim <= 0) return RB200_E_SHAPE;
  cudaStream_t st = rb::as_stream(stream);
  if ((e = forward_towers(L, params, wsplit, states, nullptr, n, false, true, work, nullptr, st))) return e;
  value_head_kernel<<<head_grid(n), 256, 0, st>>>(work + 5 * act_floats(n), params + L->vw3, values, n, L->value_dim);
  rb::count_launch();
  RB_RETURN_LAUNCH();
}
```

rlinf_b200/csrc/tc_gemm_h.cu:

```cuda
#include <cuda_fp16.h>

#include "common.cuh"
#include "tc_gemm.cuh"
#include "tc_half.cuh"
#include "tma.cuh"
#include "wgmma.cuh"

namespace rb {
namespace tch {

using rb::tc::BK;
using rb::tc::BM;
using rb::tc::BN;

constexpr int kStages = 4;
constexpr int kA32 = BM * BK * 4;
constexpr int kB16 = BN * BK * 2;
constexpr int kWBytes = 2 * kB16;
constexpr int kStageBytes = kA32 + kWBytes;
constexpr int kRingBytes = kStages * kStageBytes;
constexpr int kThreads = 384;
constexpr int kProducerRegs = 40, kConsumerRegs = 232;
static_assert(128 * kProducerRegs + 256 * kConsumerRegs <= 65536, "register file");

// ... 390 lines not shown
  }
}

int encode_f32_sw128(CUtensorMap* out, const float* base, uint64_t rows, uint64_t cols, uint32_t box_rows);

int launch(const GemmLaunch* L, int ngroups, int64_t M, int K, int epi, int b_mn, cudaStream_t st) {
  if (ngroups < 1 || ngroups > 2 || K % BK != 0 || K <= 0 || M <= 0) return RB200_E_SHAPE;
  GemmParams P{};
  P.M = M; P.K = K; P.epi = epi; P.ngroups = ngroups;
  for (int g = 0; g < ngroups; ++g) {
    const GemmLaunch& l = L[g];
    const uintptr_t al = reinterpret_cast<uintptr_t>(l.a) | reinterpret_cast<uintptr_t>(l.b_hi) |
                         reinterpret_cast<uintptr_t>(l.c) | reinterpret_cast<uintptr_t>(l.h);
    if (al & 15) return RB200_E_ALIGN;
    if (encode_f32_sw128(&P.a[g], l.a, (uint64_t)M, (uint64_t)K, BM)) return RB200_E_UNSUPPORTED;
    P.wpack[g] = reinterpret_cast<const uint8_t*>(l.b_hi);
    P.g[g] = Group{l.bias, l.h, l.colsum, l.amax_in, l.amax_x, l.amax_out, l.c};
  }
  static bool attr_done = false;
  constexpr int kSmem = kRingBytes + 1024 + (int)sizeof(Barriers);
  static_assert(kSmem <= 232448, "tc_h_gemm_kernel shared memory");
  if (!attr_done) {
    cudaError_t ce = cudaFuncSetAttribute(tc_h_gemm_kernel<0>, cudaFuncAttributeMaxDynamicSharedMemorySize, kSmem);
    if (ce == cudaSuccess) ce = cudaFuncSetAttribute(tc_h_gemm_kernel<1>, cudaFuncAttributeMaxDynamicSharedMemorySize, kSmem);
    if (ce != cudaSuccess) return (int)ce;
    attr_done = true;
  }
  const int64_t n_tiles = (M + BM - 1) / BM;
  int per_group = rb::sm_count() / ngroups;
  if (per_group > n_tiles) per_group = (int)n_tiles;
  if (per_group < 1) per_group = 1;
  rb::tch::SlotSums ss{};
  ss.nslab = per_group;
  ss.stride = (int64_t)ngroups * BN;
  if (epi == rb::tc::EPI_TANHGRAD)
    for (int g = 0; g < ngroups; ++g)
      if (L[g].colsum) {
        if (!P.part && !(P.part = rb::partials_scratch((int64_t)per_group * ngroups * BN))) return RB200_E_UNSUPPORTED;
        ss.part[ss.count] = P.part + g * BN;
        ss.out[ss.count] = L[g].colsum;
        ss.len[ss.count++] = BN;
      }
  if (b_mn) tc_h_gemm_kernel<1><<<per_group * ngroups, kThreads, kSmem, st>>>(P);
  else tc_h_gemm_kernel<0><<<per_group * ngroups, kThreads, kSmem, st>>>(P);
  rb::count_launch();
  cudaError_t ce = cudaPeekAtLastError();
  if (ce != cudaSuccess) return (int)ce;
  return ss.count ? rb::tch::sum_slots(ss, st) : 0;
}

int wgrad(const WgradLaunch* L, int ngroups, int64_t n, int IN, cudaStream_t st) {
  if (ngroups < 1 || ngroups > 2 || n <= 0 || IN <= 0 || IN > 256 || IN % 32 != 0) return RB200_E_SHAPE;
  WgradParams P{};
  P.n = n; P.IN = IN; P.ngroups = ngroups;
  for (int g = 0; g < ngroups; ++g) {
    const uintptr_t al = reinterpret_cast<uintptr_t>(L[g].z) | reinterpret_cast<uintptr_t>(L[g].h) |
                         reinterpret_cast<uintptr_t>(L[g].dW);
    if (al & 15) return RB200_E_ALIGN;
    int e = encode_f32_sw128(&P.z[g], L[g].z, (uint64_t)n, 256, 32);
    if (!e) e = encode_f32_sw128(&P.h[g], L[g].h, (uint64_t)n, (uint64_t)IN, 32);
    if (e) return RB200_E_UNSUPPORTED;
    P.dW[g] = L[g].dW;
    P.amax_z[g] = L[g].amax_z;
    P.amax_h[g] = L[g].amax_h;
  }
  static bool attr_done = false;
  constexpr int kSmem = kWgRingBytes + 1024 + (int)sizeof(WgBarriers);
  static_assert(kSmem <= 232448, "tc_h_wgrad_kernel shared memory");
  if (!attr_done) {
    cudaError_t ce = cudaFuncSetAttribute(tc_h_wgrad_kernel<128>, cudaFuncAttributeMaxDynamicSharedMemorySize, kSmem);
    if (ce == cudaSuccess) ce = cudaFuncSetAttribute(tc_h_wgrad_kernel<256>, cudaFuncAttributeMaxDynamicSharedMemorySize, kSmem);
    if (ce != cudaSuccess) return (int)ce;
    attr_done = true;
  }
  const int n_kb = (int)((n + BK - 1) / BK);
  int chunks = rb::sm_count() / (2 * ngroups);
  if (chunks < 1) chunks = 1;
  if (chunks > n_kb) chunks = n_kb;
  P.kb_per_chunk = (n_kb + chunks - 1) / chunks;
  chunks = (n_kb + P.kb_per_chunk - 1) / P.kb_per_chunk;
  const int64_t slab = 256 * (int64_t)IN;
  if (!(P.part = rb::partials_scratch(chunks * ngroups * slab))) return RB200_E_UNSUPPORTED;
  const dim3 grid(ngroups * 2 * chunks);
  if (IN <= 128) tc_h_wgrad_kernel<128><<<grid, kThreads, kSmem, st>>>(P);
  else tc_h_wgrad_kernel<256><<<grid, kThreads, kSmem, st>>>(P);
  rb::count_launch();
  cudaError_t ce = cudaPeekAtLastError();
  if (ce != cudaSuccess) return (int)ce;
  rb::tch::SlotSums ss{};
  ss.count = ngroups;
  ss.nslab = chunks;
  ss.stride = ngroups * slab;
  for (int g = 0; g < ngroups; ++g) {
    ss.part[g] = P.part + g * slab;
    ss.out[g] = L[g].dW;
    ss.len[g] = (int)slab;
  }
  return rb::tch::sum_slots(ss, st);
}

__global__ void __launch_bounds__(256) sum_slots_kernel(const SlotSums s) {
  const int q = blockIdx.y;
  for (int i = blockIdx.x * blockDim.x + threadIdx.x; i < s.len[q]; i += gridDim.x * blockDim.x) {
    float acc = 0.f;
    for (int k = 0; k < s.nslab; ++k) acc += s.part[q][k * s.stride + i];
    s.out[q][i] += acc;
  }
}

int sum_slots(const SlotSums& s, cudaStream_t st) {
  if (s.count < 1 || s.count > 8 || s.nslab < 1) return RB200_E_SHAPE;
  int len = 0;
  for (int q = 0; q < s.count; ++q) len = s.len[q] > len ? s.len[q] : len;
  int blocks = (len + 255) / 256;
  if (blocks > 4 * rb::sm_count()) blocks = 4 * rb::sm_count();
  sum_slots_kernel<<<dim3(blocks, s.count), 256, 0, st>>>(s);
  rb::count_launch();
  cudaError_t ce = cudaPeekAtLastError();
  return ce == cudaSuccess ? 0 : (int)ce;
}

int split_weights(const SplitSpec* specs, int count, cudaStream_t st) {
  if (count < 1 || count > 8) return RB200_E_SHAPE;
  SplitJobs jobs{};
  jobs.count = count;
  int64_t total = 0;
  for (int i = 0; i < count; ++i) {
    const int64_t K = specs[i].n / BN;
    if (K * BN != specs[i].n || K % BK != 0 || (specs[i].lo != nullptr && K != BN)) return RB200_E_SHAPE;
    jobs.j[i] = SplitJob{specs[i].src, reinterpret_cast<uint8_t*>(specs[i].hi), reinterpret_cast<uint8_t*>(specs[i].lo), (int)K};
    total = specs[i].n / 8 > total ? specs[i].n / 8 : total;
  }
  int64_t blocks = (total + 255) / 256;
  const int64_t cap = (int64_t)rb::sm_count() * 4;
  if (blocks > cap) blocks = cap;
  split_half_kernel<<<(int)blocks, 256, 0, st>>>(jobs);
  rb::count_launch();
  cudaError_t ce = cudaPeekAtLastError();
  return ce == cudaSuccess ? 0 : (int)ce;
}

}

namespace tc {
int g_debug_flags = 0;

}
}

extern "C" int rb200_debug_set_flags(int flags) {
  rb::tc::g_debug_flags = flags;
  return RB200_OK;
}

extern "C" int rb200_tc_gemm_h(const float* A, const float* B, float* C, int64_t M, int K, int mode, const float* amax,
                               float* work, rb200_stream_t stream) {
  if (!A || !B || !C || !work) return RB200_E_NULL;
  if (M <= 0 || K <= 0 || K % rb::tc::BK != 0 || mode < 0 || mode > 2) return RB200_E_SHAPE;
  cudaStream_t st = rb::as_stream(stream);
  const int64_t nb = (int64_t)rb::tc::BN * K;
  const bool dgrad = mode == 1;
  if (dgrad && K != rb::tc::BN) return RB200_E_SHAPE;
  rb::tch::SplitSpec sp{B, work, dgrad ? work + nb : nullptr, nb};
  int e = rb::tch::split_weights(&sp, 1, st);
  if (e) return e;
  rb::tch::GemmLaunch l{};
  l.a = A; l.b_hi = dgrad ? sp.lo : sp.hi; l.c = C; l.amax_in = amax;
  if (mode == 0 && K <= rb::tc::BN) return rb::tch::forward(&l, 1, M, K, rb::tc::EPI_STORE, st);
  return rb::tch::launch(&l, 1, M, K, rb::tc::EPI_STORE, dgrad ? 1 : 0, st);
}

extern "C" int rb200_tc_wgrad_h(const float* Z, const float* H, float* dW, int64_t n, int IN, const float* amax,
                                rb200_stream_t stream) {
  if (!Z || !H || !dW) return RB200_E_NULL;
  rb::tch::WgradLaunch l{Z, H, dW, amax};
  return rb::tch::wgrad(&l, 1, n, IN, rb::as_stream(stream));
}
```

rlinf_b200/ops.py:

```python
from __future__ import annotations

import ctypes as C
import operator
from typing import Optional

import torch

from . import _lib as L


def loss_mask(dones: torch.Tensor):
    lib = L.load()
    if dones.dim() != 3:
        raise ValueError(f"dones must be [n_chunk_steps+1, bsz, num_action_chunks], got {tuple(dones.shape)}")
    d = L.as_u8(L.to_device(dones))
    ncp1, B, Cc = d.shape
    mask = torch.empty((ncp1 - 1, B, Cc), dtype=torch.uint8, device=d.device)
    msum = torch.empty((B,), dtype=torch.int64, device=d.device)
    L.check(lib.rb200_loss_mask(L.ptr(d), L.ptr(mask), L.ptr(msum), ncp1 - 1, B, Cc, L.stream_ptr()), "loss_mask")
    return mask.view(torch.bool), msum.view(1, B, 1).expand(ncp1 - 1, B, Cc)


def gae(rewards, values, dones, gamma, gae_lambda, loss_mask=None, want_stats=False):
    lib = L.load()
    r = L.to_device(rewards, dtype=torch.float32)
    dev = r.device
    v = L.to_device(values, dev, torch.float32)
    d = L.as_u8(L.to_device(dones, dev))
    m = L.as_u8(L.to_device(loss_mask, dev))
    T, B = r.shape
    if d.shape != (T + 1, B):
        raise ValueError(f"dones must be [T+1,B]=({T + 1},{B}), got {tuple(d.shape)}")
    if v is not None and v.shape != (T + 1, B):
        raise ValueError(f"values must be [T+1,B]=({T + 1},{B}), got {tuple(v.shape)}")
    if m is not None and m.shape != (T, B):
        raise ValueError(f"loss_mask must be [T,B]=({T},{B}), got {tuple(m.shape)}")
    adv = torch.empty_like(r)
    ret = torch.empty_like(r)
    stats = torch.empty(6, dtype=torch.float64, device=dev) if want_stats else None
    L.check(lib.rb200_gae(L.ptr(r), L.ptr(v), L.ptr(d), L.ptr(m), L.ptr(adv), L.ptr(ret), L.ptr(stats), T, B,
                          float(gamma), float(gae_lambda), L.stream_ptr()), "gae")
    return adv, ret, stats


def normalize_(x: torch.Tensor, stats: torch.Tensor, eps: float = 1e-5) -> torch.Tensor:
    lib = L.load()
    L.check(lib.rb200_normalize(L.ptr(x), L.ptr(stats), x.numel(), float(eps), L.stream_ptr()), "normalize")
    return x


def grpo_scores(rewards, dones) -> torch.Tensor:
    lib = L.load()
    r = L.to_device(rewards, dtype=torch.float32)
    d = L.as_u8(L.to_device(dones, r.device))
    T, B = r.shape
    s = torch.empty((B,), dtype=torch.float32, device=r.device)
    L.check(lib.rb200_grpo_scores(L.ptr(r), L.ptr(d), L.ptr(s), T, B, L.stream_ptr()), "grpo_scores")
    return s


def grpo_advantages(scores, loss_mask, T, group_size, eps=1e-6) -> torch.Tensor:
    lib = L.load()
    s = L.to_device(scores, dtype=torch.float32).reshape(-1)
    m = L.as_u8(L.to_device(loss_mask, s.device))
    B = s.numel()
    adv = torch.empty((T, B), dtype=torch.float32, device=s.device)
    L.check(lib.rb200_grpo_advantages(L.ptr(s), L.ptr(m), L.ptr(adv), T, B, int(group_size), float(eps),
                                      L.stream_ptr()), "grpo_advantages")
    return adv


def absmax(x: torch.Tensor, out: Optional[torch.Tensor] = None) -> torch.Tensor:
    lib = L.load()
    rows, cols = x.shape[0], x[0].numel()
    out = out if out is not None else torch.empty(4 + cols if cols <= 256 else 1, dtype=torch.float32, device=x.device)
    L.check(lib.rb200_absmax(L.ptr(x), rows, cols, L.ptr(out), L.stream_ptr()), "absmax")
    return out


def gather_rows(src: torch.Tensor, idx: torch.Tensor) -> torch.Tensor:
    lib = L.load()
    s = L.to_device(src)
    i = L.to_device(idx, s.device, torch.int64)
    n_src = s.shape[0]
    row_bytes = s[0].numel() * s.element_size() if n_src > 0 else 0
    out = torch.empty((i.numel(), *s.shape[1:]), dtype=s.dtype, device=s.device)
    if i.numel() == 0 or row_bytes == 0:
        return out
    L.check(lib.rb200_gather_rows(L.ptr(s), L.ptr(i), L.ptr(out), i.numel(), n_src, row_bytes, L.stream_ptr()),
            "gather_rows")
    return out


def ppo_loss(*, logprobs, old_logprobs, advantages, C_chunks, A_dim, logprob_type, values=None, returns=None,
             prev_values=None, loss_mask=None, loss_mask_sum=None, mask_sum_row_mod=0, idx=None, entropy=None,
             adv_stats=None, adv_norm_eps=1e-5, clip_ratio_low=0.2, clip_ratio_high=0.2, clip_ratio_c=None,
             clip_log_ratio_min=None, clip_log_ratio_max=None, value_clip=0.0, huber_delta=0.0,
             max_episode_steps=None, critic_warmup=False, entropy_bonus=0.0, loss_scale=1.0, want_grads=True,
             _decoupled=None):
    lib = L.load()
    dev = logprobs.device
    bsz = logprobs.shape[0]
    with_critic = values is not None
    lp = logprobs.contiguous()
    a = L.PpoArgs()
    a.bsz, a.C, a.A = bsz, int(C_chunks), int(A_dim)
    a.logprob_type = L.LOGPROB_TYPES[logprob_type] if isinstance(logprob_type, str) else int(logprob_type)
    a.with_critic = 1 if with_critic else 0
    keep = [lp]

    def P(t, dtype=None):
        if t is None:
            return None
        t = L.to_device(t, dev, dtype)
        keep.append(t)
        return L.ptr(t)

    a.logprobs = L.ptr(lp)
    a.values = P(values, torch.float32)
    a.entropy = P(entropy, torch.float32)
    a.idx = P(idx, torch.int64)
    a.old_logprobs = P(old_logprobs, torch.float32)
    a.advantages = P(advantages, torch.float32)
    a.returns = P(returns, torch.float32)
    a.prev_values = P(prev_values, torch.float32)
    a.loss_mask = P(L.as_u8(loss_mask) if loss_mask is not None else None)
    a.loss_mask_sum = P(loss_mask_sum, torch.int64)
    a.mask_sum_row_mod = int(mask_sum_row_mod)
    a.adv_stats = P(adv_stats, torch.float64)
    a.adv_norm_eps = float(adv_norm_eps)
    a.clip_ratio_low, a.clip_ratio_high = float(clip_ratio_low), float(clip_ratio_high)
    a.clip_ratio_c = float(clip_ratio_c) if clip_ratio_c is not None else 0.0
    if clip_ratio_c is not None and not clip_ratio_c > 1.0:
        raise AssertionError("clip_ratio_c must be greater than 1.0")
    a.has_clip_log_ratio_min = int(clip_log_ratio_min is not None)
    a.has_clip_log_ratio_max = int(clip_log_ratio_max is not None)
    a.clip_log_ratio_min = float(clip_log_ratio_min or 0.0)
    a.clip_log_ratio_max = float(clip_log_ratio_max or 0.0)
    a.value_clip = float(value_clip or 0.0)
    a.huber_delta = float(huber_delta or 0.0)
    a.max_episode_steps = int(max_episode_steps) if max_episode_steps else 0
    a.critic_warmup = int(bool(critic_warmup))
    a.entropy_bonus = float(entropy_bonus)
    a.loss_scale = float(loss_scale)
    ws = _loss_workspace(dev)
    loss = torch.empty(1, dtype=torch.float32, device=dev)
    metrics = torch.empty(L.NUM_METRICS, dtype=torch.float32, device=dev)
    d_lp = torch.empty_like(lp) if want_grads else None
    d_v = torch.empty((values.numel(),), dtype=torch.float32, device=dev).view(values.shape) if (want_grads and with_critic) else None
    d_e = torch.empty_like(keep[0]) if (want_grads and entropy is not None) else None
    a.workspace, a.loss, a.metrics = L.ptr(ws), L.ptr(loss), L.ptr(metrics)
    a.d_logprobs, a.d_values, a.d_entropy = L.ptr(d_lp), L.ptr(d_v), L.ptr(d_e)
    if _decoupled is not None and _decoupled.get("version") is not None:
        if _decoupled.get("versions") is not None or _decoupled.get("current_version") is None:
            raise ValueError("a scalar `version` needs `current_version` and excludes the `versions` tensor")
        d = L.DppoScalarVersionArgs()
        d.base = a
        d.proximal_logprobs = P(_decoupled.get("proximal_logprobs"), torch.float32)
        d.version, d.current_version = float(_decoupled["version"]), float(_decoupled["current_version"])
        thr = _decoupled.get("behave_weight_threshold")
        d.has_behave_weight_threshold, d.behave_weight_threshold = int(thr is not None), float(thr or 0.0)
        L.check(lib.rb200_decoupled_ppo_loss_scalar_version(C.byref(d), L.stream_ptr()), "decoupled_ppo_loss")
        return loss, metrics, d_lp, d_v, d_e
    if _decoupled is not None:
        d = L.DppoArgs()
        d.base = a
        d.proximal_logprobs = P(_decoupled.get("proximal_logprobs"), torch.float32)
        d.versions = P(_decoupled.get("versions"), torch.float32)
        cv, thr = _decoupled.get("current_version"), _decoupled.get("behave_weight_threshold")
        d.has_current_version, d.current_version = int(cv is not None), float(cv or 0.0)
        d.has_behave_weight_threshold, d.behave_weight_threshold = int(thr is not None), float(thr or 0.0)
        L.check(lib.rb200_decoupled_ppo_loss(C.byref(d), L.stream_ptr()), "decoupled_ppo_loss")
        return loss, metrics, d_lp, d_v, d_e
    L.check(lib.rb200_ppo_loss(C.byref(a), L.stream_ptr()), "ppo_loss")
    return loss, metrics, d_lp, d_v, d_e


def opd_loss(*, logprobs, advantages, loss_mask, loss_mask_sum, max_episode_steps=None, loss_scale=1.0, want_grads=True):
    lib = L.load()
    lp = logprobs.contiguous()
    dev = lp.device
    n_units, g = lp.shape
    adv = L.to_device(advantages, dev, torch.float32).reshape(n_units, g)
    m = L.as_u8(L.to_device(loss_mask, dev)).reshape(n_units).contiguous()
    ms = L.to_device(loss_mask_sum, dev, torch.int64).reshape(n_units).contiguous()
    loss = torch.empty(1, dtype=torch.float32, device=dev)
    metrics = torch.empty(L.NUM_METRICS, dtype=torch.float32, device=dev)
    d_lp = torch.empty_like(lp) if want_grads else None
    L.check(lib.rb200_opd_loss(L.ptr(lp), L.ptr(adv), L.ptr(m), L.ptr(ms), n_units, g, int(max_episode_steps or 0),
                               float(loss_scale), L.ptr(_loss_workspace(dev)), L.ptr(loss), L.ptr(metrics), L.ptr(d_lp),
                               L.stream_ptr()), "opd_loss")
    return loss, metrics, d_lp


_WS: dict = {}


def _loss_workspace(dev) -> torch.Tensor:
    key = dev.index
    ws = _WS.get(key)
    if ws is None:
        ws = torch.zeros(32, dtype=torch.float64, device=dev)
        _WS[key] = ws
    return ws


def scale_(x: torch.Tensor, s: float) -> torch.Tensor:
    lib = L.load()
    L.check(lib.rb200_scale(L.ptr(x), x.numel(), float(s), L.stream_ptr()), "scale")
    return x


def scale_by_(x: torch.Tensor, s_dev: torch.Tensor) -> torch.Tensor:
    lib = L.load()
    s = s_dev.reshape(1).to(torch.float32)
    L.check(lib.rb200_scale_by(L.ptr(x), x.numel(), L.ptr(s), L.stream_ptr()), "scale_by")
    return x


def reward_filter(rewards, loss_mask, group_size, lower, upper):
    lib = L.load()
    r = L.to_device(rewards, dtype=torch.float32)
    m = L.as_u8(L.to_device(loss_mask, r.device))
    nc, B, Cc = r.shape
    if B % group_size != 0:
        raise AssertionError(f"batch {B} not divisible by group_size {group_size}")
    out = torch.empty((nc, B, Cc if m is not None else 1), dtype=torch.uint8, device=r.device)
    keep = torch.empty((B,), dtype=torch.uint8, device=r.device)
    L.check(lib.rb200_reward_filter(L.ptr(r), L.ptr(m), L.ptr(out), L.ptr(keep), nc, B, Cc, int(group_size),
                                    float(lower), float(upper), L.stream_ptr()), "reward_filter")
    return out.view(torch.bool)


_KL_MODES = {"kl": 0, "k1": 0, "abs": 1, "mse": 2, "k2": 2, "low_var_kl": 3, "k3": 3}


def kl_penalty_raw(logprob, ref_logprob, kind, want_grad=False):
    lib = L.load()
    if kind not in _KL_MODES:
        raise NotImplementedError(kind)
    a = L.to_device(logprob, dtype=torch.float32)
    b = L.to_device(ref_logprob, a.device, torch.float32)
    out = torch.empty_like(a)
    g = torch.empty_like(a) if want_grad else None
    L.check(lib.rb200_kl_penalty(L.ptr(a), L.ptr(b), L.ptr(out), L.ptr(g), a.numel(), _KL_MODES[kind],
                                 L.stream_ptr()), "kl_penalty")
    return out, g


_KL_ORDERS = {"megatron": 0, "fsdp": 1}


def _rows(t, name, shape, dev, dtype=torch.float32):
    if t is None:
        return None, 0
    if tuple(t.shape) != shape:
        raise ValueError(f"token_policy_loss: {name} has shape {tuple(t.shape)}, expected {shape} (that of logprobs)")
    if t.dtype != dtype:
        raise ValueError(f"token_policy_loss: {name} must be {dtype}, got {t.dtype}")
    if t.device != dev:
        raise ValueError(f"token_policy_loss: {name} is on {t.device}, logprobs on {dev}")
    if t.stride(1) != 1 or t.stride(0) < shape[1]:
        t = t.contiguous()
    return t, t.stride(0)


def _token_loss_cfg(logprobs, old_logprobs, advantages, loss_mask, entropy, ref_logprobs, rollout_logprobs,
                    recomputed_logprobs, loss_agg, clip_ratio_low, clip_ratio_high, clip_ratio_c, clip_log_ratio_min,
                    clip_log_ratio_max, entropy_bonus, kl_beta, kl_penalty, kl_order, importance_sampling_fix,
                    importance_sampling_clip, fast_path_zero_loss_mask):
    for name, t in (("logprobs", logprobs), ("old_logprobs", old_logprobs), ("advantages", advantages)):
        assert t.dtype == torch.float32, f"{name} must be float32 to keep numerical stability"
    if logprobs.dim() != 2:
        raise ValueError(f"token_policy_loss: logprobs must be [bsz, L], got {tuple(logprobs.shape)}")
    if loss_agg not in L.AGG_MODES:
        raise ValueError(f"Unsupported loss aggregation method: {loss_agg}; supported: {sorted(L.AGG_MODES)}")
    if clip_ratio_c is not None:
        assert clip_ratio_c > 1.0, "clip_ratio_c must be greater than 1.0"
    if kl_penalty == "full":
        raise NotImplementedError("kl_penalty 'full' needs the whole vocabulary's log-probs (utils.py:60-62)")
    if kl_penalty not in _KL_MODES:
        raise ValueError(f"unknown kl_penalty {kl_penalty!r}; supported: {sorted(_KL_MODES)}")
    if kl_order not in _KL_ORDERS:
        raise ValueError(f"kl_order must be one of {sorted(_KL_ORDERS)}, got {kl_order!r}")
    if importance_sampling_fix:
        if rollout_logprobs is None or recomputed_logprobs is None:
            raise ValueError("importance_sampling_fix requires both rollout_logprobs and recomputed_logprobs")
        if importance_sampling_clip is None:
            raise ValueError("importance_sampling_fix requires importance_sampling_clip")
    shape, dev = tuple(logprobs.shape), logprobs.device
    if loss_mask is None or tuple(loss_mask.shape) != shape:
        raise ValueError(f"token_policy_loss: loss_mask has shape {None if loss_mask is None else tuple(loss_mask.shape)}"
                         f", expected {shape} (that of logprobs)")
    if loss_mask.dtype not in (torch.bool, torch.uint8):
        raise ValueError(f"token_policy_loss: loss_mask must be bool or uint8, got {loss_mask.dtype}")
    if 0 in shape:
        raise ValueError(f"token_policy_loss: empty logprobs {shape}")
    named = dict(logprobs=logprobs, old_logprobs=old_logprobs, advantages=advantages,
                 loss_mask=loss_mask.view(torch.uint8) if loss_mask.dtype == torch.bool else loss_mask,
                 entropy=entropy, ref_logprobs=ref_logprobs, rollout_logprobs=rollout_logprobs,
                 recomputed_logprobs=recomputed_logprobs)
    ins = {k: _rows(t, k, shape, dev, torch.uint8 if k == "loss_mask" else torch.float32) for k, t in named.items()}
    hp = dict(clip_ratio_low=float(clip_ratio_low), clip_ratio_high=float(clip_ratio_high),
              clip_ratio_c=float(clip_ratio_c) if clip_ratio_c is not None else 0.0,
              has_clip_log_ratio_min=int(clip_log_ratio_min is not None),
              has_clip_log_ratio_max=int(clip_log_ratio_max is not None),
              clip_log_ratio_min=float(clip_log_ratio_min or 0.0), clip_log_ratio_max=float(clip_log_ratio_max or 0.0),
              entropy_bonus=float(entropy_bonus or 0.0), kl_beta=float(kl_beta or 0.0),
              importance_sampling_clip=float(importance_sampling_clip or 0.0), agg=L.AGG_MODES[loss_agg],
              kl_mode=_KL_MODES[kl_penalty], kl_order=_KL_ORDERS[kl_order],
              importance_sampling_fix=int(bool(importance_sampling_fix)),
              fast_path_zero_loss_mask=int(bool(fast_path_zero_loss_mask)))
    return ins, hp


def _token_loss_launch(lp, ent, ins, hp, want_d_lp, want_d_ent):
    if not lp.is_cuda:
        raise L.Rb200Error("token_policy_loss takes CUDA tensors; there is no CPU path")
    lib = L.load()
    dev = lp.device
    bsz, Ln = lp.shape
    a = L.TokenLossArgs()
    a.bsz, a.L = bsz, Ln
    keep = []
    for name, (t, stride) in ins.items():
        if name == "logprobs":
            t, stride = lp, lp.stride(0)
        elif name == "entropy":
# ... 1301 lines not shown
```

rlinf_b200/policy.py:

```python
from __future__ import annotations

import ctypes as C
import math
from typing import Optional

import torch

from . import _lib as L

HIDDEN = 256


class MLPPolicy:
    def __init__(self, obs_dim: int, action_dim: int, num_action_chunks: int = 1, add_value_head: bool = True,
                 value_granularity: str = "action_level", device=None, seed: Optional[int] = None):
        self.obs_dim, self.action_dim, self.num_action_chunks = int(obs_dim), int(action_dim), int(num_action_chunks)
        self.act_dim = self.action_dim * self.num_action_chunks
        self.value_dim = 0 if not add_value_head else (1 if value_granularity == "chunk_level" else self.num_action_chunks)
        self.device = device or L.default_device()
        lib = L.load()
        self.layout = L.MlpLayout()
        L.check(lib.rb200_mlp_layout_init(C.byref(self.layout), self.obs_dim, self.act_dim, self.value_dim, HIDDEN),
                "mlp_layout_init")
        n = self.layout.total
        self._param_store = torch.zeros(n + 4, dtype=torch.float32, device=self.device)
        self.flat_params = self._param_store[:n]
        self.flat_grads = torch.zeros(n, dtype=torch.float32, device=self.device)
        self._spec = self._build_spec()
        self._scratch: dict[tuple, torch.Tensor] = {}
        self.wsplit = torch.zeros(int(lib.rb200_mlp_wsplit_floats(C.byref(self.layout))), dtype=torch.float32,
                                  device=self.device)
        self._wsplit_fresh = False
        self.reset_parameters(seed)

    def _build_spec(self):
        Lo, H, O, A, V = self.layout, HIDDEN, self.obs_dim, self.act_dim, self.value_dim
        spec = [("actor_logstd", Lo.logstd, (1, A)),
                ("value_head.mlp.0.weight", Lo.vw0, (H, O)), ("value_head.mlp.0.bias", Lo.vb0, (H,)),
                ("value_head.mlp.2.weight", Lo.vw1, (H, H)), ("value_head.mlp.2.bias", Lo.vb1, (H,)),
                ("value_head.mlp.4.weight", Lo.vw2, (H, H)), ("value_head.mlp.4.bias", Lo.vb2, (H,)),
                ("value_head.mlp.6.weight", Lo.vw3, (V, H)),
                ("backbone.0.weight", Lo.bw0, (H, O)), ("backbone.0.bias", Lo.bb0, (H,)),
                ("backbone.2.weight", Lo.bw1, (H, H)), ("backbone.2.bias", Lo.bb1, (H,)),
                ("backbone.4.weight", Lo.bw2, (H, H)), ("backbone.4.bias", Lo.bb2, (H,)),
                ("actor_mean.weight", Lo.mw, (A, H)), ("actor_mean.bias", Lo.mb, (A,))]
        if V == 0:
            spec = [s for s in spec if not s[0].startswith("value_head")]
        return spec

    def named_parameters(self):
        for name, off, shape in self._spec:
            yield name, self.flat_params[off: off + math.prod(shape)].view(shape)

    def named_grads(self):
        for name, off, shape in self._spec:
            yield name, self.flat_grads[off: off + math.prod(shape)].view(shape)

    def state_dict(self):
        return {k: v.clone() for k, v in self.named_parameters()}

    def sync_buffer(self) -> torch.Tensor:
        return self._param_store[: self.flat_params.numel() + 1]

    def mark_params_changed(self):
        self._wsplit_fresh = False

    def _ws(self):
        if not self._wsplit_fresh:
            L.check(L.load().rb200_mlp_prepare_weights(C.byref(self.layout), L.ptr(self.flat_params),
                                                       L.ptr(self.wsplit), L.stream_ptr()), "mlp_prepare_weights")
            self._wsplit_fresh = True
        return L.ptr(self.wsplit)

    def load_state_dict(self, sd: dict, strict: bool = False):
        views = dict(self.named_parameters())
        if strict:
            unexpected = [k for k in sd if k not in views]
            shapes = [f"{k}: {tuple(sd[k].shape)} vs {tuple(v.shape)}" for k, v in views.items()
                      if k in sd and tuple(sd[k].shape) != tuple(v.shape)]
            if unexpected or shapes:
                raise ValueError(f"state dict does not match the policy: unexpected keys {unexpected}, "
                                 f"shape mismatches {shapes}")
        missing = [k for k in views if k not in sd]
        if missing:
            raise KeyError(f"missing parameters: {missing}")
        for k, v in views.items():
            v.copy_(sd[k].to(self.device, torch.float32).reshape(v.shape))
        self.mark_params_changed()

    def lr_group_ends(self):
        segs = []
        for name, off, shape in self._spec:
            kind = "critic" if "value_head" in name else "actor"
            end = off + math.prod(shape)
            if segs and segs[-1][0] == kind:
                segs[-1][1] = end
            else:
                segs.append([kind, end])
        segs[-1][1] = int(self.layout.total)
        return segs

    def reset_parameters(self, seed: Optional[int] = None):
        g = torch.Generator().manual_seed(0 if seed is None else int(seed))
        for name, p in self.named_parameters():
            if name == "actor_logstd":
                p.fill_(-0.5)
            elif name.endswith("bias"):
                p.zero_()
            elif name == "value_head.mlp.6.weight":
                p.copy_(torch.randn(p.shape, generator=g) * 0.02)
            elif name.startswith("value_head"):
                p.copy_(torch.randn(p.shape, generator=g) * ((5.0 / 3.0) / math.sqrt(p.shape[0])))
            else:
                w = torch.empty(p.shape)
                gain = 0.01 * math.sqrt(2) if name.startswith("actor_mean") else math.sqrt(2)
                torch.nn.init.orthogonal_(w, gain=gain, generator=g)
                p.copy_(w)
        self.mark_params_changed()

    def _buf(self, key, numel):
        t = self._scratch.get(key)
        if t is None or t.numel() < numel:
            t = torch.empty(numel, dtype=torch.float32, device=self.device)
            self._scratch[key] = t
        return t

    def forward_train(self, states, action, idx=None, n=None, compute_entropy=True, compute_values=True,
                      states_amax=None):
        lib = L.load()
        n = int(n if n is not None else (idx.numel() if idx is not None else states.shape[0]))
        nscr = lib.rb200_mlp_fwd_scratch_floats(C.byref(self.layout), n)
        acts = self._buf("acts", nscr)
        work = self._buf("work", nscr)
        logp = torch.empty((n, self.act_dim), dtype=torch.float32, device=self.device)
        ent = torch.empty_like(logp) if compute_entropy else None
        vals = torch.empty((n, self.value_dim), dtype=torch.float32, device=self.device) if (
            compute_values and self.value_dim > 0) else None
        L.check(lib.rb200_mlp_forward(C.byref(self.layout), L.ptr(self.flat_params), self._ws(), L.ptr(states),
                                      L.ptr(action), L.ptr(idx), n, L.ptr(logp), L.ptr(ent), L.ptr(vals), L.ptr(acts),
                                      L.ptr(work), L.ptr(states_amax), L.stream_ptr()), "mlp_forward")
        self._last = (states, action, idx, n, acts)
        out = {"logprobs": logp}
        if ent is not None:
            out["entropy"] = ent
        if vals is not None:
            out["values"] = vals
        return out

    def backward(self, d_logprobs, d_values=None, d_entropy=None):
        lib = L.load()
        states, action, idx, n, acts = self._last
        work = self._buf("work", acts.numel())
        L.check(lib.rb200_mlp_backward(C.byref(self.layout), L.ptr(self.flat_params), self._ws(), L.ptr(states),
                                       L.ptr(action), L.ptr(idx), n, L.ptr(d_logprobs), L.ptr(d_entropy), L.ptr(d_values),
                                       L.ptr(acts), L.ptr(work), L.ptr(self.flat_grads), L.stream_ptr()),
                "mlp_backward")

    def sample(self, states, noise=None, seed=0, offset=0, calculate_values=True, counter=None, out=None):
        lib = L.load()
        n = states.shape[0]
        work = self._buf("sample", lib.rb200_mlp_fwd_scratch_floats(C.byref(self.layout), n))
        if out is not None:
            action, logp, vals = out
        else:
            action = torch.empty((n, self.act_dim), dtype=torch.float32, device=self.device)
            logp = torch.empty_like(action)
            vals = torch.empty((n, self.value_dim), dtype=torch.float32, device=self.device) if (
                calculate_values and self.value_dim > 0) else None
        L.check(lib.rb200_mlp_sample(C.byref(self.layout), L.ptr(self.flat_params), self._ws(), L.ptr(states), L.ptr(noise),
                                     int(seed), int(offset), L.ptr(counter), n, L.ptr(action), L.ptr(logp),
                                     L.ptr(vals), L.ptr(work), L.stream_ptr()), "mlp_sample")
        return action, logp, vals

    def value(self, states, out=None):
        lib = L.load()
        n = states.shape[0]
        work = self._buf("value", lib.rb200_mlp_fwd_scratch_floats(C.byref(self.layout), n))
        vals = out if out is not None else torch.empty((n, self.value_dim), dtype=torch.float32, device=self.device)
        L.check(lib.rb200_mlp_value(C.byref(self.layout), L.ptr(self.flat_params), self._ws(), L.ptr(states), n, L.ptr(vals),
                                    L.ptr(work), L.stream_ptr()), "mlp_value")
        return vals

    def mean(self, states, calculate_logprobs=True, calculate_values=True, out=None, work_key="mean"):
        lib = L.load()
        n = states.shape[0]
        work = self._buf(work_key, lib.rb200_mlp_fwd_scratch_floats(C.byref(self.layout), n))
        action = out if out is not None else torch.empty((n, self.act_dim), dtype=torch.float32, device=self.device)
        logp = torch.empty_like(action) if calculate_logprobs else None
        vals = torch.empty((n, self.value_dim), dtype=torch.float32, device=self.device) if (
            calculate_values and self.value_dim > 0) else None
        L.check(lib.rb200_mlp_mean(C.byref(self.layout), L.ptr(self.flat_params), self._ws(), L.ptr(states), n,
                                   L.ptr(action), L.ptr(logp), L.ptr(vals), L.ptr(work), L.stream_ptr()), "mlp_mean")
        return action, logp, vals

    def predict_action_batch(self, env_obs, calculate_values=True, noise=None, seed=0, offset=0, mode="train",
                             **kwargs):
        states = env_obs["states"]
        if mode == "train":
            action, logp, vals = self.sample(states, noise=noise, seed=seed, offset=offset,
                                             calculate_values=calculate_values)
        elif mode == "eval":
            action, logp, vals = self.mean(states, calculate_values=calculate_values)
        else:
            raise NotImplementedError(f"mode={mode!r}")
        if vals is None:
            vals = torch.zeros((states.shape[0], 1), dtype=torch.float32, device=self.device)
        result = {"prev_logprobs": logp, "prev_values": vals,
                  "forward_inputs": {"action": action, "model_action": action, "states": states}}
        return action.reshape(-1, self.num_action_chunks, self.action_dim), result


class FlatAdamW:

    def __init__(self, policy: MLPPolicy, lr=3e-4, value_lr=3e-4, betas=(0.9, 0.999), eps=1e-8, weight_decay=1e-2,
                 clip_grad=0.5):
        self.policy = policy
        self.lr, self.value_lr, self.betas, self.eps, self.weight_decay = lr, value_lr, betas, eps, weight_decay
        self.clip_grad = float(clip_grad)
        n = policy.flat_params.numel()
        dev = policy.device
        self.exp_avg = torch.zeros(n, dtype=torch.float32, device=dev)
        self.exp_avg_sq = torch.zeros(n, dtype=torch.float32, device=dev)
        self.grad_sq = torch.zeros(1, dtype=torch.float64, device=dev)
        self.state = torch.zeros(4, dtype=torch.float64, device=dev)
        segs = policy.lr_group_ends()
        self._ends = (C.c_int64 * len(segs))(*[e for _, e in segs])
        self._kinds = [k for k, _ in segs]
        self.lr_scale = 1.0
        self.frozen: set = set()
        self._lr_dev = torch.zeros(8, dtype=torch.float64, device=dev)
        self._lr_key = None

    def zero_grad(self):
        self.policy.flat_grads.zero_()

    def _segment_lrs(self):
        return [-1.0 if k in self.frozen else (self.value_lr if k == "critic" else self.lr) * self.lr_scale
                for k in self._kinds]

    def sync_lr_table(self):
        lrs = self._segment_lrs()
        key = tuple(lrs)
        if key != self._lr_key:
            host = torch.zeros(8, dtype=torch.float64)
            host[: len(lrs)] = torch.tensor(lrs, dtype=torch.float64)
            self._lr_dev.copy_(host)
            self._lr_key = key

    def step(self, grad_scale: float = 1.0):
        lib = L.load()
        p = self.policy
        n = p.flat_params.numel()
        st = L.stream_ptr()
        if not torch.cuda.is_current_stream_capturing():
            self.sync_lr_table()
        L.check(lib.rb200_grad_sqnorm(L.ptr(p.flat_grads), n, L.ptr(self.grad_sq), st), "grad_sqnorm")
        L.check(lib.rb200_adamw_step_dev(L.ptr(p.flat_params), L.ptr(p.flat_grads), L.ptr(self.exp_avg),
                                         L.ptr(self.exp_avg_sq), n, self._ends, L.ptr(self._lr_dev), len(self._kinds),
                                         self.betas[0], self.betas[1], self.eps, self.weight_decay, self.clip_grad,
                                         float(grad_scale), L.ptr(self.grad_sq), L.ptr(self.state), st), "adamw_step")
        self._last_grad_scale = float(grad_scale)
        p.mark_params_changed()

    def state_dict(self) -> dict:
        return {"exp_avg": self.exp_avg, "exp_avg_sq": self.exp_avg_sq, "state": self.state,
                "last_grad_scale": float(getattr(self, "_last_grad_scale", 1.0))}

    def load_state_dict(self, sd: dict):
        self.exp_avg.copy_(sd["exp_avg"])
        self.exp_avg_sq.copy_(sd["exp_avg_sq"])
        self.state.copy_(sd["state"])
        self._last_grad_scale = float(sd["last_grad_scale"])

    def reset_state(self, carry_grads: bool = False):
        self.state[0].zero_()
        if not carry_grads:
            self.exp_avg.zero_()
            self.exp_avg_sq.zero_()
            return
        gmul = self.state[2].to(torch.float32) * getattr(self, "_last_grad_scale", 1.0)
        g = self.policy.flat_grads * gmul
        g = torch.where(self.state[3] != 0, torch.zeros_like(g), g)
        torch.mul(g, 1.0 - self.betas[0], out=self.exp_avg)
        torch.mul(g * g, 1.0 - self.betas[1], out=self.exp_avg_sq)

    def last_grad_norm(self) -> torch.Tensor:
        return self.state[1]

    def lr_list(self):
        lrs = []
        if "actor" not in self.frozen:
            lrs.append(self.lr * self.lr_scale)
        if "critic" in self._kinds and "critic" not in self.frozen:
            lrs.append(self.value_lr * self.lr_scale)
        return lrs
```

Measured before the change: 6.615 million.

## Fuse policy/value heads with PPO loss and head backward into one kernel

```diff
diff --git a/include/rlinf_b200.h b/include/rlinf_b200.h
--- a/include/rlinf_b200.h
+++ b/include/rlinf_b200.h
@@ -340,6 +340,10 @@
                        const float* d_logprobs, const float* d_entropy, const float* d_values,
                        const float* acts, float* work, float* grads, rb200_stream_t stream);
 
+int rb200_mlp_ppo_train(const rb200_mlp_layout* L, const float* params, const float* wsplit, const float* states,
+                        const float* action, int64_t n, const rb200_ppo_args* args, const float* states_amax,
+                        float* acts, float* work, float* grads, rb200_stream_t stream);
+
 int rb200_mlp_sample(const rb200_mlp_layout* L, const float* params, const float* wsplit,
                      const float* states, const float* noise, uint64_t seed, uint64_t offset,
                      const uint64_t* counter_dev, int64_t n, float* action, float* logprobs, float* values,
@@ -354,6 +358,7 @@
                            rb200_stream_t stream);
 
 int rb200_debug_set_flags(int flags);
+int rb200_debug_get_flags(void);
 
 typedef struct rb200_rollout_args {
   float* states;
diff --git a/rlinf_b200/_lib.py b/rlinf_b200/_lib.py
--- a/rlinf_b200/_lib.py
+++ b/rlinf_b200/_lib.py
@@ -208,11 +208,14 @@
     "rb200_mlp_forward": (c_int, [C.POINTER(MlpLayout)] + [c_void_p] * 5 + [c_int64] + [c_void_p] * 7),
     "rb200_absmax": (c_int, [c_void_p, c_int64, c_int, c_void_p, c_void_p]),
     "rb200_mlp_backward": (c_int, [C.POINTER(MlpLayout)] + [c_void_p] * 5 + [c_int64] + [c_void_p] * 7),
+    "rb200_mlp_ppo_train": (c_int, [C.POINTER(MlpLayout)] + [c_void_p] * 4 + [c_int64, C.POINTER(PpoArgs)] +
+                            [c_void_p] * 5),
     "rb200_mlp_sample": (c_int, [C.POINTER(MlpLayout)] + [c_void_p] * 4 + [c_uint64, c_uint64, c_void_p, c_int64] + [c_void_p] * 5),
     "rb200_tc_gemm_h": (c_int, [c_void_p, c_void_p, c_void_p, c_int64, c_int, c_int, c_void_p, c_void_p, c_void_p]),
     "rb200_tc_wgrad_h": (c_int, [c_void_p, c_void_p, c_void_p, c_int64, c_int, c_void_p, c_void_p]),
     "rb200_tc_dgrad_wgrad_h": (c_int, [c_void_p] * 8 + [c_int64, c_int, c_void_p, c_void_p]),
     "rb200_debug_set_flags": (c_int, [c_int]),
+    "rb200_debug_get_flags": (c_int, []),
     "rb200_rollout_fused_wt_floats": (c_int64, [C.POINTER(MlpLayout)]),
     "rb200_rollout_fused_supported": (c_int, [C.POINTER(MlpLayout), c_int]),
     "rb200_rollout_fused_prepare": (c_int, [C.POINTER(MlpLayout), c_void_p, c_void_p, c_void_p]),
diff --git a/rlinf_b200/actor.py b/rlinf_b200/actor.py
--- a/rlinf_b200/actor.py
+++ b/rlinf_b200/actor.py
@@ -70,6 +70,7 @@
         self.optimizer_steps = 0
         self.critic_warmup_steps = int(o.get("critic_warmup_steps", 0) or 0) if self.model.value_dim > 0 else 0
         self._with_critic = self.cfg.algorithm.adv_type == "gae"
+        self._heads_ppo = ops.heads_ppo_supported(self.cfg, self.model.layout)
         self._set_frozen_groups()
         self.lr_schedule = LRSchedule(o, base_lr=o.lr)
         self.optimizer.lr_scale = self.lr_schedule.multiplier()
@@ -269,12 +270,29 @@
         with_critic = self._with_critic
         ent_bonus = float(cfg.algorithm.get("entropy_bonus", 0) or 0)
         warm = self.optimizer_steps < self.critic_warmup_steps
+        n = hi - lo
+        if self._heads_ppo and not (L.load().rb200_debug_get_flags() & ops.HEADS_PPO_OFF):
+            def rows(key):
+                t = batch.get(key)
+                return None if t is None else t[lo:hi].reshape(n)
+
+            _, metrics = self.model.ppo_train(
+                fi["states"][lo:hi], fi["action"][lo:hi], states_amax=self._states_amax, with_critic=with_critic,
+                old_logprobs=batch["prev_logprobs"][lo:hi].reshape(n, -1), advantages=rows("advantages"),
+                returns=rows("returns") if with_critic else None,
+                prev_values=rows("prev_values") if with_critic else None, loss_mask=rows("loss_mask"),
+                loss_mask_sum=rows("loss_mask_sum"), logprob_type=cfg.algorithm.logprob_type,
+                clip_ratio_low=cfg.algorithm.clip_ratio_low, clip_ratio_high=cfg.algorithm.clip_ratio_high,
+                value_clip=cfg.algorithm.get("value_clip", None), huber_delta=cfg.algorithm.get("huber_delta", None),
+                max_episode_steps=cfg.env.train.max_episode_steps if batch.get("loss_mask_sum") is not None else None,
+                critic_warmup=warm, entropy_bonus=ent_bonus, loss_scale=1.0 / self.gradient_accumulation)
+            metric_out.copy_(metrics)
+            return
         out = self.model.forward_train(fi["states"][lo:hi], fi["action"][lo:hi], compute_entropy=ent_bonus > 0,
                                        compute_values=with_critic, states_amax=self._states_amax)
         A = cfg.actor.model.get("action_dim", 7)
         Cc = out["logprobs"].shape[1] // A
         U = 1 if cfg.algorithm.logprob_type == "chunk_level" else Cc
-        n = hi - lo
 
         def unit(key):
             t = batch.get(key)
diff --git a/rlinf_b200/csrc/heads.cuh b/rlinf_b200/csrc/heads.cuh
--- /dev/null
+++ b/rlinf_b200/csrc/heads.cuh
@@ -0,0 +1,64 @@
+#pragma once
+#include "common.cuh"
+
+namespace rb {
+namespace heads {
+
+constexpr int kH = 256;
+constexpr int kMaxAct = 32;
+constexpr int kMaxVal = 8;
+constexpr float kHalfLog2Pi = 0.91893853320467274178f;
+
+__device__ __forceinline__ float row_dot(const float4& h0, const float4& h1, const float* w, int lane) {
+  const float4 w0 = *reinterpret_cast<const float4*>(w + lane * 4);
+  const float4 w1 = *reinterpret_cast<const float4*>(w + 128 + lane * 4);
+  const float s = h0.x * w0.x + h0.y * w0.y + h0.z * w0.z + h0.w * w0.w + h1.x * w1.x + h1.y * w1.y + h1.z * w1.z +
+                  h1.w * w1.w;
+  return rb::warp_sum(s);
+}
+
+__device__ __forceinline__ float normal_logprob(float d, float sd) {
+  const float var = sd * sd;
+  return -(d * d) / (2.0f * var) - logf(sd) - kHalfLog2Pi;
+}
+__device__ __forceinline__ float normal_entropy(float sd) { return 0.5f + kHalfLog2Pi + logf(sd); }
+
+struct HeadBwdArgs {
+  const float* h3;
+  const float* g3;
+  const float* mean;
+  const float* mw;
+  const float* logstd;
+  const float* vw3;
+  const float* action;
+  const int64_t* idx;
+  const float* d_logprobs;
+  const float* d_entropy;
+  const float* d_values;
+  float* dz3;
+  float* dy3;
+  float* g_mw;
+  float* g_mb;
+  float* g_logstd;
+  float* g_vw3;
+  float* g_b2;
+  float* g_vb2;
+  float* amax_dz3;
+  float* amax_dy3;
+  float* part;
+  int64_t n;
+  int act, vdim;
+};
+
+int head_grid(int64_t n);
+
+}
+
+int mlp_train_forward(const rb200_mlp_layout* L, const float* params, const float* wsplit, const float* states, int64_t n,
+                      bool values, float* acts, const float* states_amax, cudaStream_t st);
+void head_bwd_shape(const rb200_mlp_layout* L, int* warps, size_t* smem, int* acc_len);
+int head_bwd_finish(const rb200_mlp_layout* L, const float* params, const float* wsplit, const float* states,
+                    const int64_t* idx, int64_t n, const float* part, int grid, bool values, const float* acts,
+                    float* work, float* grads, cudaStream_t st);
+
+}
diff --git a/rlinf_b200/csrc/heads_ppo.cu b/rlinf_b200/csrc/heads_ppo.cu
--- /dev/null
+++ b/rlinf_b200/csrc/heads_ppo.cu
@@ -0,0 +1,517 @@
+#include "common.cuh"
+#include "critic_unit.cuh"
+#include "heads.cuh"
+#include "ppo_unit.cuh"
+#include "tc_gemm.cuh"
+
+namespace {
+
+using rb::heads::HeadBwdArgs;
+using rb::heads::kH;
+
+enum SumSlot {
+  S_CNT = 0,
+  S_L,
+  S_LABS,
+  S_RATIO,
+  S_RABS,
+  S_CLIPPED,
+  S_DUAL,
+  S_KL,
+  S_CLIPFRAC,
+  S_VL,
+  S_VCLIP,
+  S_EV_N,
+  S_EV_R,
+  S_EV_R2,
+  S_EV_E,
+  S_EV_E2,
+  S_ENT,
+  S_NUM
+};
+
+struct Hyper {
+  float clip_lo_bound, clip_hi_bound;
+  float dual_c;
+  int has_lr_min, has_lr_max;
+  float lr_min, lr_max;
+  float value_clip, huber_delta, half_huber_delta;
+  float max_episode_steps;
+  int critic_warmup;
+  float entropy_bonus, loss_scale;
+  float adv_eps;
+};
+
+struct RowPassArgs {
+  HeadBwdArgs p;
+  const float* mb;
+  const float* old_logprobs;
+  const float* advantages;
+  const float* returns;
+  const float* prev_values;
+  const uint8_t* loss_mask;
+  const int64_t* loss_mask_sum;
+  int64_t mask_sum_row_mod;
+  const double* adv_stats;
+  Hyper h;
+  int critic;
+  int token;
+  int entropy;
+  double* sums;
+  float* loss;
+  float* metrics;
+};
+
+__global__ void __launch_bounds__(256) mask_count_kernel(const uint8_t* __restrict__ mask, int64_t n,
+                                                         double* __restrict__ sums) {
+  __shared__ double red[32];
+  double v[1] = {0.0};
+  for (int64_t i = (int64_t)blockIdx.x * blockDim.x + threadIdx.x; i < n; i += (int64_t)gridDim.x * blockDim.x)
+    v[0] += mask[i] ? 1.0 : 0.0;
+  rb::block_sum<1>(v, red);
+  if (threadIdx.x == 0 && v[0] != 0.0) atomicAdd(&sums[S_CNT], v[0]);
+}
+
+__device__ void finalize(const RowPassArgs& q, const double* sums) {
+  const Hyper& h = q.h;
+  const double n_units = (double)q.p.n;
+  const double n_elems = n_units * (q.token ? q.p.act : 1);
+  const bool has_mask = q.loss_mask != nullptr;
+  const bool ratio_agg = has_mask && q.loss_mask_sum != nullptr && h.max_episode_steps > 0.0f;
+  const double mcnt = has_mask ? sums[S_CNT] : 0.0;
+  const bool all_masked = has_mask && mcnt == 0.0;
+  const double cnt = has_mask ? (mcnt > 0.0 ? mcnt : 1.0) : n_elems;
+  const double d_loss = ratio_agg ? n_elems : (has_mask ? (all_masked ? 1.0 : mcnt) : n_elems);
+  const double d_metric = has_mask ? (all_masked ? 1.0 : mcnt * (q.token ? q.p.act : 1)) : n_elems;
+  const double d_unit = ratio_agg ? n_units : (has_mask ? (all_masked ? 1.0 : mcnt) : n_units);
+  const double d_ent = has_mask ? (all_masked ? 1.0 : mcnt) : n_units;
+
+  float* M = q.metrics;
+  for (int k = 0; k < RB200_NUM_METRICS; ++k) M[k] = 0.0f;
+  double policy_loss = sums[S_L] / d_loss;
+  if (h.critic_warmup) policy_loss = 0.0;
+  M[RB200_M_POLICY_LOSS] = (float)policy_loss;
+  M[RB200_M_POLICY_LOSS_ABS] = (float)(sums[S_LABS] / d_loss);
+  M[RB200_M_RATIO] = (float)(sums[S_RATIO] / d_metric);
+  M[RB200_M_RATIO_ABS] = (float)(sums[S_RABS] / d_metric);
+  M[RB200_M_CLIPPED_RATIO] = (float)(sums[S_CLIPPED] / d_metric);
+  M[RB200_M_DUAL_CLIPPED_RATIO] = (float)(sums[S_DUAL] / d_metric);
+  M[RB200_M_APPROX_KL] = (float)(-sums[S_KL] / cnt);
+  M[RB200_M_CLIP_FRACTION] = (float)(sums[S_CLIPFRAC] / cnt);
+  M[RB200_M_TOKEN_NUM] = (float)(has_mask ? mcnt : n_elems);
+  double total = policy_loss;
+  if (q.critic) {
+    const double vl = sums[S_VL] / d_unit;
+    M[RB200_M_VALUE_LOSS] = (float)vl;
+    M[RB200_M_VALUE_CLIP_RATIO] = (float)(sums[S_VCLIP] / n_units);
+    M[RB200_M_EV_COUNT] = (float)sums[S_EV_N];
+    M[RB200_M_EV_RET_SUM] = (float)sums[S_EV_R];
+    M[RB200_M_EV_RET_SQ_SUM] = (float)sums[S_EV_R2];
+    M[RB200_M_EV_ERR_SUM] = (float)sums[S_EV_E];
+    M[RB200_M_EV_ERR_SQ_SUM] = (float)sums[S_EV_E2];
+    total += vl;
+  }
+  if (q.entropy && h.entropy_bonus > 0.0f && !h.critic_warmup) {
+    const double ent = sums[S_ENT] / d_ent;
+    M[RB200_M_ENTROPY] = (float)ent;
+    total -= (double)h.entropy_bonus * ent;
+  }
+  total *= (double)h.loss_scale;
+  M[RB200_M_TOTAL_LOSS] = (float)total;
+  if (q.loss) q.loss[0] = (float)total;
+}
+
+template <int ACT, bool CRITIC, bool TOKEN>
+__global__ void __launch_bounds__(256) heads_ppo_kernel(RowPassArgs q) {
+  extern __shared__ float sm[];
+  __shared__ double red[S_NUM * 32];
+  const HeadBwdArgs& p = q.p;
+  const int act = ACT ? ACT : p.act;
+  const Hyper& h = q.h;
+  const int lane = threadIdx.x & 31, warp = threadIdx.x >> 5, nwarp = blockDim.x >> 5;
+  const int acc_len = (act + p.vdim) * kH + 64 + 2 * kH;
+  float* s_mw = sm;
+  float* s_vw = s_mw + act * kH;
+  float* acc0 = s_vw + p.vdim * kH;
+  float* a_mw = acc0 + warp * acc_len;
+  float* a_vw = a_mw + act * kH;
+  float* a_mb = a_vw + p.vdim * kH;
+  float* a_ls = a_mb + 32;
+  float* a_b2 = a_ls + 32;
+  float* a_vb2 = a_b2 + kH;
+  constexpr bool has_v = CRITIC;
+  for (int i = threadIdx.x; i < act * kH; i += blockDim.x) s_mw[i] = p.mw[i];
+  for (int i = threadIdx.x; i < p.vdim * kH; i += blockDim.x) s_vw[i] = has_v ? p.vw3[i] : 0.f;
+  for (int i = threadIdx.x; i < nwarp * acc_len; i += blockDim.x) acc0[i] = 0.f;
+  __syncthreads();
+
+  const bool has_mask = q.loss_mask != nullptr;
+  const bool ratio_agg = has_mask && q.loss_mask_sum != nullptr && h.max_episode_steps > 0.0f;
+  const double n_units = (double)p.n;
+  const double n_elems = n_units * (TOKEN ? act : 1);
+  const double mask_cnt = has_mask ? q.sums[S_CNT] : 0.0;
+  float coef_actor, coef_unit;
+  if (ratio_agg) {
+    coef_actor = (float)(1.0 / n_elems);
+    coef_unit = (float)(1.0 / n_units);
+  } else if (has_mask) {
+    const double d = mask_cnt > 0.0 ? mask_cnt : 1.0;
+    coef_actor = (float)(1.0 / d);
+    coef_unit = coef_actor;
+  } else {
+    coef_actor = (float)(1.0 / n_elems);
+    coef_unit = (float)(1.0 / n_units);
+  }
+  bool norm_adv = false;
+  float adv_mean = 0.0f, adv_den = 1.0f;
+  if (q.adv_stats != nullptr && q.adv_stats[0] > 0.0) {
+    const double cnt = q.adv_stats[0];
+    const double mean_d = q.adv_stats[1] / cnt;
+    const double var_d = (q.adv_stats[2] - q.adv_stats[1] * mean_d) / (cnt - 1.0);
+    adv_mean = (float)mean_d;
+    adv_den = __fadd_rn((float)sqrt(var_d > 0.0 || !(var_d == var_d) ? var_d : 0.0), h.adv_eps);
+    norm_adv = true;
+  }
+  const float scale = h.loss_scale;
+  const float sd_l = lane < act ? expf(p.logstd[lane]) : 1.f;
+  const float var_l = sd_l * sd_l;
+  const float mb_l = lane < act ? q.mb[lane] : 0.f;
+  float ent_sum = 0.0f;
+  if (q.entropy) {
+    const float e_l = rb::heads::normal_entropy(sd_l);
+    for (int k = 0; k < act; ++k) ent_sum = __fadd_rn(ent_sum, __shfl_sync(0xffffffffu, e_l, k));
+  }
+  const bool want_den = q.entropy && h.entropy_bonus > 0.0f && !h.critic_warmup;
+
+  float acc[S_NUM];
+#pragma unroll
+  for (int k = 0; k < S_NUM; ++k) acc[k] = 0.0f;
+  float cb[8] = {0.f, 0.f, 0.f, 0.f, 0.f, 0.f, 0.f, 0.f}, cv[8] = {0.f, 0.f, 0.f, 0.f, 0.f, 0.f, 0.f, 0.f};
+  float mz = 0.f, my = 0.f;
+  float rm[8][8], rv[8];
+#pragma unroll
+  for (int a = 0; a < 8; ++a)
+#pragma unroll
+    for (int j = 0; j < 8; ++j) rm[a][j] = 0.f;
+#pragma unroll
+  for (int j = 0; j < 8; ++j) rv[j] = 0.f;
+
+  struct RowIn {
+    float4 h0, h1, g0, g1;
+    float x, olp, adv, rt, pv, msum;
+    bool m;
+  };
+  auto load_row = [&](int64_t row) -> RowIn {
+    RowIn r;
+    r.h0 = r.h1 = r.g0 = r.g1 = make_float4(0.f, 0.f, 0.f, 0.f);
+    r.x = r.olp = r.adv = r.rt = r.pv = r.msum = 0.f;
+    r.m = true;
+    if (row < p.n) {
+      r.h0 = __ldg(reinterpret_cast<const float4*>(p.h3 + row * kH + lane * 4));
+      r.h1 = __ldg(reinterpret_cast<const float4*>(p.h3 + row * kH + 128 + lane * 4));
+      if (has_v) {
+        r.g0 = __ldg(reinterpret_cast<const float4*>(p.g3 + row * kH + lane * 4));
+        r.g1 = __ldg(reinterpret_cast<const float4*>(p.g3 + row * kH + 128 + lane * 4));
+        r.rt = __ldg(q.returns + row);
+        r.pv = __ldg(q.prev_values + row);
+      }
+      if (lane < act) {
+        r.x = __ldg(p.action + row * act + lane);
+        r.olp = __ldg(q.old_logprobs + row * act + lane);
+      }
+      r.adv = __ldg(q.advantages + row);
+      if (has_mask) r.m = q.loss_mask[row] != 0;
+      if (ratio_agg) r.msum = (float)q.loss_mask_sum[q.mask_sum_row_mod > 0 ? row % q.mask_sum_row_mod : row];
+    }
+    return r;
+  };
+  const int64_t row_stride = (int64_t)gridDim.x * nwarp;
+  const int64_t row_first = (int64_t)blockIdx.x * nwarp + warp;
+  RowIn nxt0 = load_row(row_first), nxt1 = load_row(row_first + row_stride);
+  for (int64_t row = row_first; row < p.n; row += row_stride) {
+    const RowIn cur = nxt0;
+    nxt0 = nxt1;
+    nxt1 = load_row(row + 2 * row_stride);
+    const float4 h0 = cur.h0, h1 = cur.h1;
+
+    float mu = 0.f;
+#pragma unroll
+    for (int a = 0; a < 8; ++a) {
+      const float s = rb::heads::row_dot(h0, h1, s_mw + (a < act ? a : 0) * kH, lane);
+      if (lane == a) mu = s + mb_l;
+    }
+    const float v = rb::heads::row_dot(cur.g0, cur.g1, s_vw, lane);
+    const float lp = lane < act ? rb::heads::normal_logprob(cur.x - mu, sd_l) : 0.f;
+
+    const bool m = cur.m;
+    const float mf = m ? 1.0f : 0.0f;
+    float adv = cur.adv;
+    if (norm_adv) adv = __fdiv_rn(__fsub_rn(adv, adv_mean), adv_den);
+    float w = 1.0f;
+    if (ratio_agg) w = __fdiv_rn(cur.msum, h.max_episode_steps);
+    float lp_r = lp, old_r = cur.olp;
+    if (!TOKEN) {
+      float lp_k[8], old_k[8];
+#pragma unroll
+      for (int k = 0; k < 8; ++k) {
+        lp_k[k] = __shfl_sync(0xffffffffu, lp, k);
+        old_k[k] = __shfl_sync(0xffffffffu, cur.olp, k);
+      }
+      lp_r = 0.0f;
+      old_r = 0.0f;
+#pragma unroll
+      for (int k = 0; k < 8; ++k) {
+        if (k < act) {
+          lp_r = __fadd_rn(lp_r, lp_k[k]);
+          old_r = __fadd_rn(old_r, old_k[k]);
+        }
+      }
+    }
+    const rb::RatioOut o = rb::ratio_terms(lp_r, old_r, adv, m, h);
+    if (TOKEN ? lane < act : lane == 0) {
+      acc[S_L] += ratio_agg ? __fmul_rn(__fdiv_rn(o.loss_e, w), mf) : __fmul_rn(o.loss_e, mf);
+      acc[S_LABS] += ratio_agg ? __fmul_rn(__fdiv_rn(fabsf(o.loss_e), w), mf) : __fmul_rn(fabsf(o.loss_e), mf);
+      acc[S_RATIO] += (o.ratio * mf);
+      acc[S_RABS] += (fabsf(__fsub_rn(o.ratio, 1.0f)) * mf);
+      acc[S_CLIPPED] += (o.clipped * mf);
+      acc[S_DUAL] += (o.dual_ratio * mf);
+      acc[S_KL] += o.lr_kl;
+      acc[S_CLIPFRAC] += (o.clip_hit * mf);
+    }
+    const float cw_a = ratio_agg ? coef_actor / w : coef_actor;
+    const float dlp = h.critic_warmup ? 0.0f : scale * cw_a * o.dL_dlp;
+    float dv0 = 0.f;
+    if (has_v) {
+      const rb::CriticOut c = rb::critic_terms(v, cur.pv, cur.rt, h.value_clip, h.huber_delta, h.half_huber_delta);
+      if (lane == 0) {
+        acc[S_VL] += has_mask ? (ratio_agg ? __fmul_rn(__fdiv_rn(c.vl, w), mf) : __fmul_rn(c.vl, mf)) : c.vl;
+        acc[S_VCLIP] += rb::critic_clip_hit(c, cur.pv, h.value_clip) ? 1.0f : 0.0f;
+        if (m) {
+          acc[S_EV_N] += 1.0f;
+          acc[S_EV_R] += cur.rt;
+          acc[S_EV_R2] += __fmul_rn(cur.rt, cur.rt);
+          acc[S_EV_E] += c.e1;
+          acc[S_EV_E2] += __fmul_rn(c.e1, c.e1);
+        }
+      }
+      const float dvl = rb::critic_dvl(c, h.value_clip, h.huber_delta);
+      const float cw = has_mask ? (ratio_agg ? coef_unit / w : coef_unit) * mf : coef_unit;
+      dv0 = scale * cw * dvl;
+    }
+    float den = 0.f;
+    if (q.entropy) {
+      if (lane == 0) acc[S_ENT] += (has_mask ? __fmul_rn(ent_sum, mf) : ent_sum);
+      const float cw = (has_mask ? coef_unit * mf : (float)(1.0 / n_units));
+      den = want_den ? __fmul_rn(-scale * h.entropy_bonus, cw) : 0.0f;
+    }
+
+    float dmu = 0.f;
+    if (lane < act) {
+      const float d = cur.x - mu;
+      dmu = dlp * d / var_l;
+      const float dls = dlp * (d * d / var_l - 1.0f) + den;
+      atomicAdd(&a_mb[lane], dmu);
+      atomicAdd(&a_ls[lane], dls);
+    }
+    float4 dh0 = make_float4(0.f, 0.f, 0.f, 0.f), dh1 = dh0;
+#pragma unroll
+    for (int a = 0; a < 8; ++a) {
+      if (a >= act) break;
+      const float g = __shfl_sync(0xffffffffu, dmu, a);
+      const float4 w0 = *reinterpret_cast<const float4*>(s_mw + a * kH + lane * 4);
+      const float4 w1 = *reinterpret_cast<const float4*>(s_mw + a * kH + 128 + lane * 4);
+      dh0.x += g * w0.x; dh0.y += g * w0.y; dh0.z += g * w0.z; dh0.w += g * w0.w;
+      dh1.x += g * w1.x; dh1.y += g * w1.y; dh1.z += g * w1.z; dh1.w += g * w1.w;
+      rm[a][0] += g * h0.x; rm[a][1] += g * h0.y; rm[a][2] += g * h0.z; rm[a][3] += g * h0.w;
+      rm[a][4] += g * h1.x; rm[a][5] += g * h1.y; rm[a][6] += g * h1.z; rm[a][7] += g * h1.w;
+    }
+    float4 o0, o1;
+    o0.x = dh0.x * (1.f - h0.x * h0.x); o0.y = dh0.y * (1.f - h0.y * h0.y);
+    o0.z = dh0.z * (1.f - h0.z * h0.z); o0.w = dh0.w * (1.f - h0.w * h0.w);
+    o1.x = dh1.x * (1.f - h1.x * h1.x); o1.y = dh1.y * (1.f - h1.y * h1.y);
+    o1.z = dh1.z * (1.f - h1.z * h1.z); o1.w = dh1.w * (1.f - h1.w * h1.w);
+    *reinterpret_cast<float4*>(p.dz3 + row * kH + lane * 4) = o0;
+    *reinterpret_cast<float4*>(p.dz3 + row * kH + 128 + lane * 4) = o1;
+    cb[0] += o0.x; cb[1] += o0.y; cb[2] += o0.z; cb[3] += o0.w;
+    cb[4] += o1.x; cb[5] += o1.y; cb[6] += o1.z; cb[7] += o1.w;
+    mz = fmaxf(mz, fmaxf(fmaxf(fmaxf(fabsf(o0.x), fabsf(o0.y)), fmaxf(fabsf(o0.z), fabsf(o0.w))),
+                         fmaxf(fmaxf(fabsf(o1.x), fabsf(o1.y)), fmaxf(fabsf(o1.z), fabsf(o1.w)))));
+    if (has_v) {
+      const float4 g0 = cur.g0, g1 = cur.g1;
+      const float g = dv0;
+      const float4 w0 = *reinterpret_cast<const float4*>(s_vw + lane * 4);
+      const float4 w1 = *reinterpret_cast<const float4*>(s_vw + 128 + lane * 4);
+      float4 dg0 = make_float4(0.f, 0.f, 0.f, 0.f), dg1 = dg0;
+      dg0.x += g * w0.x; dg0.y += g * w0.y; dg0.z += g * w0.z; dg0.w += g * w0.w;
+      dg1.x += g * w1.x; dg1.y += g * w1.y; dg1.z += g * w1.z; dg1.w += g * w1.w;
+      rv[0] += g * g0.x; rv[1] += g * g0.y; rv[2] += g * g0.z; rv[3] += g * g0.w;
+      rv[4] += g * g1.x; rv[5] += g * g1.y; rv[6] += g * g1.z; rv[7] += g * g1.w;
+      float4 q0, q1;
+      q0.x = dg0.x * (1.f - g0.x * g0.x); q0.y = dg0.y * (1.f - g0.y * g0.y);
+      q0.z = dg0.z * (1.f - g0.z * g0.z); q0.w = dg0.w * (1.f - g0.w * g0.w);
+      q1.x = dg1.x * (1.f - g1.x * g1.x); q1.y = dg1.y * (1.f - g1.y * g1.y);
+      q1.z = dg1.z * (1.f - g1.z * g1.z); q1.w = dg1.w * (1.f - g1.w * g1.w);
+      *reinterpret_cast<float4*>(p.dy3 + row * kH + lane * 4) = q0;
+      *reinterpret_cast<float4*>(p.dy3 + row * kH + 128 + lane * 4) = q1;
+      cv[0] += q0.x; cv[1] += q0.y; cv[2] += q0.z; cv[3] += q0.w;
+      cv[4] += q1.x; cv[5] += q1.y; cv[6] += q1.z; cv[7] += q1.w;
+      my = fmaxf(my, fmaxf(fmaxf(fmaxf(fabsf(q0.x), fabsf(q0.y)), fmaxf(fabsf(q0.z), fabsf(q0.w))),
+                           fmaxf(fmaxf(fabsf(q1.x), fabsf(q1.y)), fmaxf(fabsf(q1.z), fabsf(q1.w)))));
+    }
+  }
+#pragma unroll
+  for (int o = 16; o > 0; o >>= 1) {
+    mz = fmaxf(mz, __shfl_xor_sync(0xffffffffu, mz, o));
+    my = fmaxf(my, __shfl_xor_sync(0xffffffffu, my, o));
+  }
+  if (lane == 0) {
+    if (mz > 0.f) atomicMax(reinterpret_cast<unsigned int*>(p.amax_dz3), __float_as_uint(mz));
+    if (has_v && my > 0.f) atomicMax(reinterpret_cast<unsigned int*>(p.amax_dy3), __float_as_uint(my));
+  }
+#pragma unroll
+  for (int j = 0; j < 4; ++j) {
+    atomicAdd(&a_b2[lane * 4 + j], cb[j]);
+    atomicAdd(&a_b2[128 + lane * 4 + j], cb[4 + j]);
+    if (has_v) {
+      atomicAdd(&a_vb2[lane * 4 + j], cv[j]);
+      atomicAdd(&a_vb2[128 + lane * 4 + j], cv[4 + j]);
+    }
+  }
+#pragma unroll
+  for (int a = 0; a < 8; ++a) {
+    if (a >= act) break;
+    float* am = a_mw + a * kH;
+#pragma unroll
+    for (int j = 0; j < 4; ++j) {
+      atomicAdd(&am[lane * 4 + j], rm[a][j]);
+      atomicAdd(&am[128 + lane * 4 + j], rm[a][4 + j]);
+    }
+  }
+  if (has_v) {
+#pragma unroll
+    for (int j = 0; j < 4; ++j) {
+      atomicAdd(&a_vw[lane * 4 + j], rv[j]);
+      atomicAdd(&a_vw[128 + lane * 4 + j], rv[4 + j]);
+    }
+  }
+  __syncthreads();
+  for (int i = threadIdx.x; i < acc_len; i += blockDim.x) {
+    float s = 0.f;
+    for (int w = 0; w < nwarp; ++w) s += acc0[w * acc_len + i];
+    p.part[(size_t)blockIdx.x * acc_len + i] = s;
+  }
+
+  double accd[S_NUM];
+#pragma unroll
+  for (int k = 0; k < S_NUM; ++k) accd[k] = (double)acc[k];
+  rb::block_sum<S_NUM>(accd, red);
+  if (threadIdx.x == 0) {
+#pragma unroll
+    for (int k = 1; k < S_NUM; ++k)
+      if (accd[k] != 0.0) atomicAdd(&q.sums[k], accd[k]);
+    __threadfence();
+    const unsigned long long prev = atomicAdd(reinterpret_cast<unsigned long long*>(q.sums + 31), 1ull);
+    if (prev == (unsigned long long)gridDim.x - 1ull) {
+      __threadfence();
+      double fin[S_NUM];
+#pragma unroll
+      for (int k = 0; k < S_NUM; ++k) fin[k] = __ldcg(&q.sums[k]);
+      finalize(q, fin);
+#pragma unroll
+      for (int k = 0; k < S_NUM; ++k) q.sums[k] = 0.0;
+      *reinterpret_cast<unsigned long long*>(q.sums + 31) = 0ull;
+    }
+  }
+}
+
+}
+
+extern "C" int rb200_mlp_ppo_train(const rb200_mlp_layout* L, const float* params, const float* wsplit,
+                                   const float* states, const float* action, int64_t n, const rb200_ppo_args* args,
+                                   const float* states_amax, float* acts, float* work, float* grads,
+                                   rb200_stream_t stream) {
+  if (!L || !args) return RB200_E_NULL;
+  if (!params || !wsplit || !states || !action || !acts || !work || !grads) return RB200_E_NULL;
+  const rb200_ppo_args& a = *args;
+  if (!a.old_logprobs || !a.advantages || !a.metrics || !a.workspace) return RB200_E_NULL;
+  if (a.with_critic && (!a.returns || !a.prev_values)) return RB200_E_NULL;
+  if (n <= 0 || a.bsz != n || a.A != L->act_dim) return RB200_E_SHAPE;
+  if (a.logprob_type < RB200_LOGPROB_TOKEN || a.logprob_type > RB200_LOGPROB_CHUNK) return RB200_E_ARG;
+  if (a.clip_ratio_c > 0.0 && !(a.clip_ratio_c > 1.0)) return RB200_E_ARG;
+  if (L->hidden != kH || L->act_dim <= 0 || L->act_dim > 8 || a.C != 1 || a.idx) return RB200_E_UNSUPPORTED;
+  if (a.with_critic && L->value_dim != 1) return RB200_E_UNSUPPORTED;
+  cudaStream_t st = rb::as_stream(stream);
+  const bool values = a.with_critic != 0;
+  int e;
+  if ((e = rb::mlp_train_forward(L, params, wsplit, states, n, values, acts, states_amax, st))) return e;
+
+  const int64_t PF = n * kH;
+  RowPassArgs q{};
+  HeadBwdArgs& p = q.p;
+  p.h3 = acts + 2 * PF; p.g3 = acts + 5 * PF; p.mw = params + L->mw; p.logstd = params + L->logstd;
+  p.vw3 = params + L->vw3; p.action = action;
+  p.dz3 = work; p.dy3 = work + 3 * PF;
+  float* amax = work + 6 * PF;
+  p.amax_dz3 = amax; p.amax_dy3 = amax + 3;
+  p.n = n; p.act = L->act_dim; p.vdim = L->value_dim;
+  q.mb = params + L->mb;
+  q.old_logprobs = a.old_logprobs; q.advantages = a.advantages; q.returns = a.returns; q.prev_values = a.prev_values;
+  q.loss_mask = a.loss_mask; q.loss_mask_sum = a.loss_mask_sum; q.mask_sum_row_mod = a.mask_sum_row_mod;
+  q.adv_stats = a.adv_stats;
+  Hyper& h = q.h;
+  h.clip_lo_bound = (float)(1.0 - a.clip_ratio_low);
+  h.clip_hi_bound = (float)(1.0 + a.clip_ratio_high);
+  h.dual_c = a.clip_ratio_c > 0.0 ? (float)a.clip_ratio_c : 0.0f;
+  h.has_lr_min = a.has_clip_log_ratio_min;
+  h.has_lr_max = a.has_clip_log_ratio_max;
+  h.lr_min = (float)a.clip_log_ratio_min;
+  h.lr_max = (float)a.clip_log_ratio_max;
+  h.value_clip = (float)a.value_clip;
+  h.huber_delta = (float)a.huber_delta;
+  h.half_huber_delta = (float)(0.5 * a.huber_delta);
+  h.max_episode_steps = a.max_episode_steps > 0 ? (float)a.max_episode_steps : 0.0f;
+  h.critic_warmup = a.critic_warmup;
+  h.entropy_bonus = (float)a.entropy_bonus;
+  h.loss_scale = (float)a.loss_scale;
+  h.adv_eps = a.adv_norm_eps;
+  q.critic = values;
+  q.token = a.logprob_type == RB200_LOGPROB_TOKEN;
+  q.entropy = a.entropy_bonus > 0.0;
+  q.sums = a.workspace; q.loss = a.loss; q.metrics = a.metrics;
+
+  {
+    cudaError_t ce = cudaMemsetAsync(amax, 0, 8 * sizeof(float), st);
+    if (ce != cudaSuccess) return (int)ce;
+  }
+  if (a.loss_mask) {
+    int64_t blocks = (n + 255) / 256;
+    const int64_t cap = (int64_t)rb::sm_count() * 3;
+    if (blocks > cap) blocks = cap;
+    mask_count_kernel<<<(int)blocks, 256, 0, st>>>(a.loss_mask, n, a.workspace);
+    rb::count_launch();
+  }
+  int nw = 0, acc_len = 0;
+  size_t smem = 0;
+  rb::head_bwd_shape(L, &nw, &smem, &acc_len);
+  const int grid = rb::heads::head_grid(n);
+  if (!(p.part = rb::partials_scratch((int64_t)grid * acc_len))) return RB200_E_UNSUPPORTED;
+  void (*kernel)(RowPassArgs);
+  {
+    const bool act8 = L->act_dim == 8;
+    if (q.token)
+      kernel = act8 ? (values ? heads_ppo_kernel<8, true, true> : heads_ppo_kernel<8, false, true>)
+                    : (values ? heads_ppo_kernel<0, true, true> : heads_ppo_kernel<0, false, true>);
+    else
+      kernel = act8 ? (values ? heads_ppo_kernel<8, true, false> : heads_ppo_kernel<8, false, false>)
+                    : (values ? heads_ppo_kernel<0, true, false> : heads_ppo_kernel<0, false, false>);
+    cudaError_t ce = cudaFuncSetAttribute(kernel, cudaFuncAttributeMaxDynamicSharedMemorySize, (int)smem);
+    if (ce != cudaSuccess) return (int)ce;
+  }
+  kernel<<<grid, 32 * nw, smem, st>>>(q);
+  rb::count_launch();
+  {
+    cudaError_t ce = cudaPeekAtLastError();
+    if (ce != cudaSuccess) return (int)ce;
+  }
+  return rb::head_bwd_finish(L, params, wsplit, states, nullptr, n, p.part, grid, values, acts, work, grads, st);
+}
diff --git a/rlinf_b200/csrc/mlp.cu b/rlinf_b200/csrc/mlp.cu
--- a/rlinf_b200/csrc/mlp.cu
+++ b/rlinf_b200/csrc/mlp.cu
@@ -1,6 +1,7 @@
 #include <curand_kernel.h>
 
 #include "common.cuh"
+#include "heads.cuh"
 #include "sgemm.cuh"
 #include "tc_gemm.cuh"
 
@@ -32,10 +33,10 @@
     if (s_col[c]) atomicMax(reinterpret_cast<unsigned int*>(out + 4 + c), s_col[c]);
 }
 
-constexpr int kH = 256;
-constexpr int kMaxAct = 32;
-constexpr int kMaxVal = 8;
-constexpr float kHalfLog2Pi = 0.91893853320467274178f;
+using rb::heads::kH;
+using rb::heads::kMaxAct;
+using rb::heads::kMaxVal;
+using rb::heads::HeadBwdArgs;
 
 struct HeadFwdArgs {
   const float* h3;
@@ -87,11 +88,7 @@
     fetch(row + row_stride);
     float my_mean = 0.f;
     for (int a = 0; a < p.act; ++a) {
-      const float4 w0 = *reinterpret_cast<const float4*>(s_mw + a * kH + lane * 4);
-      const float4 w1 = *reinterpret_cast<const float4*>(s_mw + a * kH + 128 + lane * 4);
-      float s = h0.x * w0.x + h0.y * w0.y + h0.z * w0.z + h0.w * w0.w + h1.x * w1.x + h1.y * w1.y + h1.z * w1.z +
-                h1.w * w1.w;
-      s = rb::warp_sum(s);
+      const float s = rb::heads::row_dot(h0, h1, s_mw + a * kH, lane);
       if (lane == a) my_mean = s + p.mb[a];
     }
     if (lane < p.act) {
@@ -116,52 +113,19 @@
         const int64_t src = p.idx ? p.idx[row] : row;
         x = p.action[src * p.act + lane];
       }
-      const float d = x - my_mean;
-      const float var = sd * sd;
-      if (p.logprobs) p.logprobs[row * p.act + lane] = -(d * d) / (2.0f * var) - logf(sd) - kHalfLog2Pi;
-      if (p.entropy) p.entropy[row * p.act + lane] = 0.5f + kHalfLog2Pi + logf(sd);
+      if (p.logprobs) p.logprobs[row * p.act + lane] = rb::heads::normal_logprob(x - my_mean, sd);
+      if (p.entropy) p.entropy[row * p.act + lane] = rb::heads::normal_entropy(sd);
       if (p.mean_out) p.mean_out[row * p.act + lane] = my_mean;
     }
     if (want_v) {
       const float4 g0 = pg0, g1 = pg1;
       for (int c = 0; c < p.vdim; ++c) {
-        const float4 w0 = *reinterpret_cast<const float4*>(s_vw + c * kH + lane * 4);
-        const float4 w1 = *reinterpret_cast<const float4*>(s_vw + c * kH + 128 + lane * 4);
-        float s = g0.x * w0.x + g0.y * w0.y + g0.z * w0.z + g0.w * w0.w + g1.x * w1.x + g1.y * w1.y + g1.z * w1.z +
-                  g1.w * w1.w;
-        s = rb::warp_sum(s);
+        const float s = rb::heads::row_dot(g0, g1, s_vw + c * kH, lane);
         if (lane == 0) p.values[row * p.vdim + c] = s;
       }
     }
   }
 }
-
-struct HeadBwdArgs {
-  const float* h3;
-  const float* g3;
-  const float* mean;
-  const float* mw;
-  const float* logstd;
-  const float* vw3;
-  const float* action;
-  const int64_t* idx;
-  const float* d_logprobs;
-  const float* d_entropy;
-  const float* d_values;
-  float* dz3;
-  float* dy3;
-  float* g_mw;
-  float* g_mb;
-  float* g_logstd;
-  float* g_vw3;
-  float* g_b2;
-  float* g_vb2;
-  float* amax_dz3;
-  float* amax_dy3;
-  float* part;
-  int64_t n;
-  int act, vdim;
-};
 
 template <bool REG>
 __global__ void __launch_bounds__(256) head_bwd_kernel(HeadBwdArgs p) {
@@ -361,12 +325,7 @@
   }
 }
 
-int head_grid(int64_t n) {
-  int64_t blocks = (n + 7) / 8;
-  const int64_t cap = (int64_t)rb::sm_count() * 4;
-  if (blocks > cap) blocks = cap;
-  return (int)(blocks < 1 ? 1 : blocks);
-}
+using rb::heads::head_grid;
 
 struct TowerW {
   const float *w0, *b0, *w1, *b1, *w2, *b2;
@@ -494,6 +453,13 @@
   return 0;
 }
 
+}
+
+int rb::heads::head_grid(int64_t n) {
+  int64_t blocks = (n + 7) / 8;
+  const int64_t cap = (int64_t)rb::sm_count() * 4;
+  if (blocks > cap) blocks = cap;
+  return (int)(blocks < 1 ? 1 : blocks);
 }
 
 extern "C" int rb200_mlp_layout_init(rb200_mlp_layout* L, int obs_dim, int act_dim, int value_dim, int hidden) {
@@ -631,6 +597,59 @@
   return head_forward(L, params, acts, n, values, h, st);
 }
 
+namespace rb {
+int mlp_train_forward(const rb200_mlp_layout* L, const float* params, const float* wsplit, const float* states, int64_t n,
+                      bool values, float* acts, const float* states_amax, cudaStream_t st) {
+  return forward_towers(L, params, wsplit, states, nullptr, n, true, values, acts, states_amax, st);
+}
+
+void head_bwd_shape(const rb200_mlp_layout* L, int* warps, size_t* smem, int* acc_len) {
+  *acc_len = (L->act_dim + L->value_dim) * kH + 64 + 2 * kH;
+  const int w_len = (L->act_dim + L->value_dim) * kH;
+  int nw = (232448 / 4 - w_len) / *acc_len;
+  *warps = nw > 8 ? 8 : nw;
+  *smem = sizeof(float) * ((size_t)w_len + (size_t)*warps * *acc_len);
+}
+
+int head_bwd_finish(const rb200_mlp_layout* L, const float* params, const float* wsplit, const float* states,
+                    const int64_t* idx, int64_t n, const float* part, int grid, bool values, const float* acts,
+                    float* work, float* grads, cudaStream_t st) {
+  int e;
+  const int64_t PF = act_floats(n);
+  float *dZ3 = work, *tA = dZ3 + PF, *tB = tA + PF, *dY3 = tB + PF, *uA = dY3 + PF, *uB = uA + PF;
+  float* amax = work + 6 * PF;
+  const float* P = params;
+  float* G = grads;
+  {
+    rb::tch::SlotSums ss{};
+    ss.nslab = grid;
+    const int A = L->act_dim, V = L->value_dim;
+    ss.stride = (A + V) * kH + 64 + 2 * kH;
+    auto seg = [&](int off, float* out, int len) {
+      ss.part[ss.count] = part + off; ss.out[ss.count] = out; ss.len[ss.count++] = len;
+    };
+    seg(0, G + L->mw, A * kH);
+    seg((A + V) * kH, G + L->mb, A);
+    seg((A + V) * kH + 32, G + L->logstd, A);
+    seg((A + V) * kH + 64, G + L->bb2, kH);
+    if (values) {
+      seg(A * kH, G + L->vw3, V * kH);
+      seg((A + V) * kH + 64 + kH, G + L->vb2, kH);
+    }
+    if ((e = rb::tch::sum_slots(ss, st))) return e;
+  }
+  float* act_buf = const_cast<float*>(acts);
+  TowerIO t[2] = {tower_io(L, P, wsplit, false, act_buf, n), tower_io(L, P, wsplit, true, act_buf + 3 * PF, n)};
+  t[0].dZ3 = dZ3; t[0].tA = tA; t[0].tB = tB; t[0].amax = amax;
+  t[0].g_w0 = G + L->bw0; t[0].g_b0 = G + L->bb0; t[0].g_w1 = G + L->bw1; t[0].g_b1 = G + L->bb1;
+  t[0].g_w2 = G + L->bw2; t[0].g_b2 = G + L->bb2;
+  t[1].dZ3 = dY3; t[1].tA = uA; t[1].tB = uB; t[1].amax = amax + 3;
+  t[1].g_w0 = G + L->vw0; t[1].g_b0 = G + L->vb0; t[1].g_w1 = G + L->vw1; t[1].g_b1 = G + L->vb1;
+  t[1].g_w2 = G + L->vw2; t[1].g_b2 = G + L->vb2;
+  return towers_backward_h(states, idx, n, L->obs_dim, t, values ? 2 : 1, x_amax_slot(L, act_buf, n), st);
+}
+}
+
 extern "C" int rb200_mlp_backward(const rb200_mlp_layout* L, const float* params, const float* wsplit,
                                   const float* states, const float* action, const int64_t* idx, int64_t n,
                                   const float* d_logprobs, const float* d_entropy, const float* d_values,
@@ -642,7 +661,7 @@
   cudaStream_t st = rb::as_stream(stream);
   const int64_t PF = act_floats(n);
   const float *H3 = acts + 2 * PF, *G3 = acts + 5 * PF, *mean = acts + 6 * PF;
-  float *dZ3 = work, *tA = dZ3 + PF, *tB = tA + PF, *dY3 = tB + PF, *uA = dY3 + PF, *uB = uA + PF;
+  float *dZ3 = work, *dY3 = work + 3 * PF;
   const float* P = params;
   float* G = grads;
   HeadBwdArgs h{};
@@ -659,10 +678,9 @@
   }
   h.amax_dz3 = amax;
   h.amax_dy3 = amax + 3;
-  const int acc_len = (L->act_dim + L->value_dim) * kH + 64 + 2 * kH, w_len = (L->act_dim + L->value_dim) * kH;
-  int nw = (232448 / 4 - w_len) / acc_len;
-  nw = nw > 8 ? 8 : nw;
-  const size_t smem = sizeof(float) * ((size_t)w_len + (size_t)nw * acc_len);
+  int nw = 0, acc_len = 0;
+  size_t smem = 0;
+  rb::head_bwd_shape(L, &nw, &smem, &acc_len);
   const bool reg = L->act_dim <= 8 && L->value_dim <= 2;
   const int grid = head_grid(n);
   if (!(h.part = rb::partials_scratch((int64_t)grid * acc_len))) return RB200_E_UNSUPPORTED;
@@ -681,33 +699,7 @@
     cudaError_t ce = cudaPeekAtLastError();
     if (ce != cudaSuccess) return (int)ce;
   }
-  {
-    rb::tch::SlotSums ss{};
-    ss.nslab = grid;
-    ss.stride = acc_len;
-    const int A = L->act_dim, V = L->value_dim;
-    auto seg = [&](int off, float* out, int len) {
-      ss.part[ss.count] = h.part + off; ss.out[ss.count] = out; ss.len[ss.count++] = len;
-    };
-    seg(0, h.g_mw, A * kH);
-    seg((A + V) * kH, h.g_mb, A);
-    seg((A + V) * kH + 32, h.g_logstd, A);
-    seg((A + V) * kH + 64, h.g_b2, kH);
-    if (d_values) {
-      seg(A * kH, h.g_vw3, V * kH);
-      seg((A + V) * kH + 64 + kH, h.g_vb2, kH);
-    }
-    if ((e = rb::tch::sum_slots(ss, st))) return e;
-  }
-  float* act_buf = const_cast<float*>(acts);
-  TowerIO t[2] = {tower_io(L, P, wsplit, false, act_buf, n), tower_io(L, P, wsplit, true, act_buf + 3 * PF, n)};
-  t[0].dZ3 = dZ3; t[0].tA = tA; t[0].tB = tB; t[0].amax = amax;
-  t[0].g_w0 = G + L->bw0; t[0].g_b0 = G + L->bb0; t[0].g_w1 = G + L->bw1; t[0].g_b1 = G + L->bb1;
-  t[0].g_w2 = G + L->bw2; t[0].g_b2 = G + L->bb2;
-  t[1].dZ3 = dY3; t[1].tA = uA; t[1].tB = uB; t[1].amax = amax + 3;
-  t[1].g_w0 = G + L->vw0; t[1].g_b0 = G + L->vb0; t[1].g_w1 = G + L->vw1; t[1].g_b1 = G + L->vb1;
-  t[1].g_w2 = G + L->vw2; t[1].g_b2 = G + L->vb2;
-  return towers_backward_h(states, idx, n, L->obs_dim, t, d_values ? 2 : 1, x_amax_slot(L, act_buf, n), st);
+  return rb::head_bwd_finish(L, params, wsplit, states, idx, n, h.part, grid, d_values != nullptr, acts, work, grads, st);
 }
 
 extern "C" int rb200_mlp_sample(const rb200_mlp_layout* L, const float* params, const float* wsplit,
diff --git a/rlinf_b200/csrc/tc_gemm_h.cu b/rlinf_b200/csrc/tc_gemm_h.cu
--- a/rlinf_b200/csrc/tc_gemm_h.cu
+++ b/rlinf_b200/csrc/tc_gemm_h.cu
@@ -566,6 +566,7 @@
   rb::tc::g_debug_flags = flags;
   return RB200_OK;
 }
+extern "C" int rb200_debug_get_flags(void) { return rb::tc::g_debug_flags; }
 
 extern "C" int rb200_tc_gemm_h(const float* A, const float* B, float* C, int64_t M, int K, int mode, const float* amax,
                                float* work, rb200_stream_t stream) {
diff --git a/rlinf_b200/ops.py b/rlinf_b200/ops.py
--- a/rlinf_b200/ops.py
+++ b/rlinf_b200/ops.py
@@ -92,22 +92,14 @@
     return out
 
 
-def ppo_loss(*, logprobs, old_logprobs, advantages, C_chunks, A_dim, logprob_type, values=None, returns=None,
-             prev_values=None, loss_mask=None, loss_mask_sum=None, mask_sum_row_mod=0, idx=None, entropy=None,
-             adv_stats=None, adv_norm_eps=1e-5, clip_ratio_low=0.2, clip_ratio_high=0.2, clip_ratio_c=None,
-             clip_log_ratio_min=None, clip_log_ratio_max=None, value_clip=0.0, huber_delta=0.0,
-             max_episode_steps=None, critic_warmup=False, entropy_bonus=0.0, loss_scale=1.0, want_grads=True,
-             _decoupled=None):
-    lib = L.load()
-    dev = logprobs.device
-    bsz = logprobs.shape[0]
-    with_critic = values is not None
-    lp = logprobs.contiguous()
+def _ppo_args(dev, bsz, C_chunks, A_dim, logprob_type, with_critic, keep, *, old_logprobs, advantages, returns,
+              prev_values, loss_mask, loss_mask_sum, mask_sum_row_mod, idx, adv_stats, adv_norm_eps, clip_ratio_low,
+              clip_ratio_high, clip_ratio_c, clip_log_ratio_min, clip_log_ratio_max, value_clip, huber_delta,
+              max_episode_steps, critic_warmup, entropy_bonus, loss_scale):
     a = L.PpoArgs()
     a.bsz, a.C, a.A = bsz, int(C_chunks), int(A_dim)
     a.logprob_type = L.LOGPROB_TYPES[logprob_type] if isinstance(logprob_type, str) else int(logprob_type)
     a.with_critic = 1 if with_critic else 0
-    keep = [lp]
 
     def P(t, dtype=None):
         if t is None:
@@ -116,9 +108,6 @@
         keep.append(t)
         return L.ptr(t)
 
-    a.logprobs = L.ptr(lp)
-    a.values = P(values, torch.float32)
-    a.entropy = P(entropy, torch.float32)
     a.idx = P(idx, torch.int64)
     a.old_logprobs = P(old_logprobs, torch.float32)
     a.advantages = P(advantages, torch.float32)
@@ -143,6 +132,30 @@
     a.critic_warmup = int(bool(critic_warmup))
     a.entropy_bonus = float(entropy_bonus)
     a.loss_scale = float(loss_scale)
+    return a, keep, P
+
+
+def ppo_loss(*, logprobs, old_logprobs, advantages, C_chunks, A_dim, logprob_type, values=None, returns=None,
+             prev_values=None, loss_mask=None, loss_mask_sum=None, mask_sum_row_mod=0, idx=None, entropy=None,
+             adv_stats=None, adv_norm_eps=1e-5, clip_ratio_low=0.2, clip_ratio_high=0.2, clip_ratio_c=None,
+             clip_log_ratio_min=None, clip_log_ratio_max=None, value_clip=0.0, huber_delta=0.0,
+             max_episode_steps=None, critic_warmup=False, entropy_bonus=0.0, loss_scale=1.0, want_grads=True,
+             _decoupled=None):
+    lib = L.load()
+    dev = logprobs.device
+    lp = logprobs.contiguous()
+    a, keep, P = _ppo_args(dev, logprobs.shape[0], C_chunks, A_dim, logprob_type, values is not None, [lp],
+                           old_logprobs=old_logprobs, advantages=advantages, returns=returns, prev_values=prev_values,
+                           loss_mask=loss_mask, loss_mask_sum=loss_mask_sum, mask_sum_row_mod=mask_sum_row_mod,
+                           idx=idx, adv_stats=adv_stats, adv_norm_eps=adv_norm_eps, clip_ratio_low=clip_ratio_low,
+                           clip_ratio_high=clip_ratio_high, clip_ratio_c=clip_ratio_c,
+                           clip_log_ratio_min=clip_log_ratio_min, clip_log_ratio_max=clip_log_ratio_max,
+                           value_clip=value_clip, huber_delta=huber_delta, max_episode_steps=max_episode_steps,
+                           critic_warmup=critic_warmup, entropy_bonus=entropy_bonus, loss_scale=loss_scale)
+    with_critic = values is not None
+    a.logprobs = L.ptr(lp)
+    a.values = P(values, torch.float32)
+    a.entropy = P(entropy, torch.float32)
     ws = _loss_workspace(dev)
     loss = torch.empty(1, dtype=torch.float32, device=dev)
     metrics = torch.empty(L.NUM_METRICS, dtype=torch.float32, device=dev)
@@ -174,6 +187,34 @@
         return loss, metrics, d_lp, d_v, d_e
     L.check(lib.rb200_ppo_loss(C.byref(a), L.stream_ptr()), "ppo_loss")
     return loss, metrics, d_lp, d_v, d_e
+
+
+HEADS_PPO_OFF = 8
+
+
+def heads_ppo_supported(cfg, layout) -> bool:
+    if cfg.actor.model.get("num_action_chunks", 1) != 1 or not 0 < int(layout.act_dim) <= 8:
+        return False
+    return cfg.algorithm.adv_type != "gae" or int(layout.value_dim) == 1
+
+
+def mlp_ppo_train(policy, states, action, *, states_amax=None, **loss_kw):
+    lib = L.load()
+    dev = policy.device
+    n = int(states.shape[0])
+    with_critic = loss_kw.pop("with_critic")
+    a, keep, _ = _ppo_args(dev, n, 1, policy.act_dim, loss_kw.pop("logprob_type"), with_critic, [], idx=None,
+                           mask_sum_row_mod=0, adv_stats=None, adv_norm_eps=1e-5, clip_ratio_c=None,
+                           clip_log_ratio_min=None, clip_log_ratio_max=None, **loss_kw)
+    loss = torch.empty(1, dtype=torch.float32, device=dev)
+    metrics = torch.empty(L.NUM_METRICS, dtype=torch.float32, device=dev)
+    a.workspace, a.loss, a.metrics = L.ptr(_loss_workspace(dev)), L.ptr(loss), L.ptr(metrics)
+    nscr = lib.rb200_mlp_fwd_scratch_floats(C.byref(policy.layout), n)
+    acts, work = policy._buf("acts", nscr), policy._buf("work", nscr)
+    L.check(lib.rb200_mlp_ppo_train(C.byref(policy.layout), L.ptr(policy.flat_params), policy._ws(), L.ptr(states),
+                                    L.ptr(action), n, C.byref(a), L.ptr(states_amax), L.ptr(acts), L.ptr(work),
+                                    L.ptr(policy.flat_grads), L.stream_ptr()), "mlp_ppo_train")
+    return loss, metrics
 
 
 def opd_loss(*, logprobs, advantages, loss_mask, loss_mask_sum, max_episode_steps=None, loss_scale=1.0, want_grads=True):
diff --git a/rlinf_b200/policy.py b/rlinf_b200/policy.py
--- a/rlinf_b200/policy.py
+++ b/rlinf_b200/policy.py
@@ -156,6 +156,11 @@
                                        L.ptr(acts), L.ptr(work), L.ptr(self.flat_grads), L.stream_ptr()),
                 "mlp_backward")
 
+    def ppo_train(self, states, action, **kw):
+        from . import ops
+
+        return ops.mlp_ppo_train(self, states, action, **kw)
+
     def sample(self, states, noise=None, seed=0, offset=0, calculate_values=True, counter=None, out=None):
         lib = L.load()
         n = states.shape[0]
```

Result: faster. 6.812 million (median of 6 runs) (+3.0%).
